# austintheriot/ray-tracer-webgl

Measured on AMD Instinct MI355X. Metric: Mray/s (ray segments/s) at 1920x1080, higher is better.
Workload: dtype f32

## Files before the change

### bindings/rust/ptrace_sys.rs

```rust
use std::os::raw::{c_char, c_int, c_void};

#[repr(C)] #[derive(Clone, Copy, Default)]
pub struct PtSphere {
    pub center: [f32; 3], pub radius: f32,
    pub type_: i32, pub albedo: [f32; 3],
    pub fuzz: f32, pub refraction_index: f32,
    pub uuid: i32, pub _pad: i32,
}

#[repr(C)] #[derive(Clone, Copy, Default)]
pub struct PtParams {
    pub width: u32, pub height: u32,
    pub time: f32, pub samples_per_pixel: i32, pub max_depth: i32,
    pub camera_origin: [f32; 3], pub horizontal: [f32; 3], pub vertical: [f32; 3],
    pub lower_left_corner: [f32; 3], pub u: [f32; 3], pub v: [f32; 3],
    pub lens_radius: f32,
    pub render_count: i32, pub should_average: i32, pub last_frame_weight: f32,
    pub background_mode: i32,
    pub band_rows: u32, pub band_index: u32, pub band_count: u32,
    pub time_step: f32, pub first_pass: u32,
}

#[repr(C)] #[derive(Clone, Copy, Default)]
pub struct PtErrorStats {
// ... 46 lines not shown

#[repr(C)] #[derive(Clone, Copy, Default)]
pub struct PtProbeSH {
    pub sh: [[f32; 3]; 9], pub samples: f32,
}

#[repr(C)] #[derive(Clone, Copy, Default)]
pub struct PtProbeLattice {
    pub origin: [f32; 3], pub nx: u32, pub step: [f32; 3], pub ny: u32, pub nz: u32, pub flags: u32, pub _pad: [u32; 2],
}

#[repr(C)] #[derive(Clone, Copy, Default)]
pub struct PtProbeShadeOptions {
    pub flags: u32, pub normal_bias: f32, pub _pad: [u32; 2],
}

#[repr(C)] #[derive(Clone, Copy)]
pub struct PtMeterOptions {
    pub key: f32, pub key_permille: u32, pub high_permille: u32, pub e_min: f32, pub e_max: f32, pub white_min: f32, pub rate: f32,
    pub x0: u32, pub y0: u32, pub w: u32, pub h: u32, pub _pad: u32,
}
impl Default for PtMeterOptions {
    fn default() -> Self {
        PtMeterOptions { key: 0.18, key_permille: 500, high_permille: 990, e_min: 0.00390625, e_max: 256.0, white_min: 1.0, rate: 1.0,
                         x0: 0, y0: 0, w: 0, h: 0, _pad: 0 }
    }
}

#[repr(C)] #[derive(Clone, Copy, Default)]
pub struct PtExposure {
    pub exposure: f32, pub white: f32, pub y_key: f32, pub y_high: f32, pub lit: u64, pub below: u32, pub meterings: u32,
}

#[repr(C)] #[derive(Clone, Copy, Default)]
pub struct PtToneOptions {
    pub curve: i32, pub gamma: i32, pub exposure: f32, pub white: f32,
}

pub const PT_GLARE_MAX_LEVELS: usize = 8;
#[repr(C)] #[derive(Clone, Copy)]
pub struct PtGlareOptions {
    pub strength: f32, pub threshold: f32, pub levels: u32, pub _pad: u32, pub weight: [f32; PT_GLARE_MAX_LEVELS],
}
impl Default for PtGlareOptions {
    fn default() -> Self {
        PtGlareOptions { strength: 0.15, threshold: 0.0, levels: 6, _pad: 0, weight: [0.35, 0.25, 0.18, 0.12, 0.06, 0.04, 0.0, 0.0] }
    }
}

#[repr(C)] pub struct PtCtx { _private: [u8; 0] }

#[link(name = "ptrace")]
extern "C" {
    pub fn pt_create(out: *mut *mut PtCtx, device: c_int, width: u32, height: u32) -> c_int;
    pub fn pt_create_on_stream(out: *mut *mut PtCtx, device: c_int, width: u32, height: u32, hip_stream: *mut c_void) -> c_int;
    pub fn pt_destroy(ctx: *mut PtCtx) -> c_int;
    pub fn pt_resize(ctx: *mut PtCtx, width: u32, height: u32) -> c_int;
    pub fn pt_set_spheres(ctx: *mut PtCtx, spheres: *const PtSphere, n: u32) -> c_int;
    pub fn pt_set_params(ctx: *mut PtCtx, params: *const PtParams) -> c_int;
    pub fn pt_render(ctx: *mut PtCtx) -> c_int;
    pub fn pt_render_passes(ctx: *mut PtCtx, n_passes: u32) -> c_int;
    pub fn pt_reserve_passes(ctx: *mut PtCtx, max_passes: u32) -> c_int;
    pub fn pt_reset_accum(ctx: *mut PtCtx) -> c_int;
    pub fn pt_synchronize(ctx: *mut PtCtx) -> c_int;
    pub fn pt_resolve(ctx: *mut PtCtx, rgba_out: *mut f32, gamma: c_int) -> c_int;
    pub fn pt_resolve_rgba8(ctx: *mut PtCtx, rgba_out: *mut u8, gamma: c_int) -> c_int;
    pub fn pt_blend_rgba8(ctx: *mut PtCtx, prev: *const u8, out: *mut u8) -> c_int;
    pub fn pt_accum_ptr(ctx: *mut PtCtx, dev_ptr: *mut *mut c_void, bytes: *mut usize) -> c_int;
    pub fn pt_bind_accum(ctx: *mut PtCtx, dev_ptr: *mut c_void, bytes: usize) -> c_int;
    pub fn pt_read_accum(ctx: *mut PtCtx, dst: *mut f32, bytes: usize) -> c_int;
    pub fn pt_load_accum(ctx: *mut PtCtx, src: *const f32, bytes: usize) -> c_int;
    pub fn pt_set_stream(ctx: *mut PtCtx, hip_stream: *mut c_void) -> c_int;
    pub fn pt_set_option(ctx: *mut PtCtx, key: c_int, value: c_int) -> c_int;
    pub fn pt_tune(ctx: *mut PtCtx, n_passes: u32) -> c_int;
    pub fn pt_set_debug_overlay(ctx: *mut PtCtx, enable: c_int, selected_object: i32, cursor_point: *const f32) -> c_int;
    pub fn pt_last_trace_build(ctx: *mut PtCtx) -> c_int;
    pub fn pt_error_ptr(ctx: *mut PtCtx, dev_ptr: *mut *mut c_void, bytes: *mut usize) -> c_int;
    pub fn pt_resolve_error(ctx: *mut PtCtx, rgba_out: *mut f32) -> c_int;
    pub fn pt_error_tiles(ctx: *mut PtCtx, tiles_out: *mut f32, tiles_x: *mut u32, tiles_y: *mut u32) -> c_int;
    pub fn pt_error_stats(ctx: *mut PtCtx, out: *mut PtErrorStats) -> c_int;
    pub fn pt_render_until(ctx: *mut PtCtx, target_rel_error: f32, passes_per_launch: u32, max_passes: u32, out: *mut PtErrorStats) -> c_int;
    pub fn pt_render_adaptive(ctx: *mut PtCtx, target_rel_error: f32, passes_per_round: u32, max_passes: u32, out: *mut PtErrorStats, adaptive_out: *mut PtAdaptiveStats) -> c_int;
    pub fn pt_adaptive_tiles(ctx: *mut PtCtx, base_out: *mut u32, order_out: *mut u32, n_tiles: *mut u32, n_active: *mut u32) -> c_int;
    pub fn pt_resolve_filtered(ctx: *mut PtCtx, rgba_out: *mut f32, radius: u32, kappa: f32, gamma: c_int) -> c_int;
    pub fn pt_resolve_filtered_patch(ctx: *mut PtCtx, rgba_out: *mut f32, radius: u32, patch: u32, kappa: f32, gamma: c_int) -> c_int;
    pub fn pt_render_features(ctx: *mut PtCtx) -> c_int;
    pub fn pt_features_ptr(ctx: *mut PtCtx, plane: c_int, dev_ptr: *mut *mut c_void, bytes: *mut usize) -> c_int;
    pub fn pt_read_features(ctx: *mut PtCtx, plane: c_int, out: *mut c_void) -> c_int;
    pub fn pt_keep_history(ctx: *mut PtCtx) -> c_int;
    pub fn pt_load_history(ctx: *mut PtCtx, prev: *const PtParams, ids: *const c_void, point: *const c_void) -> c_int;
    pub fn pt_reproject(ctx: *mut PtCtx, options: *const PtReprojectOptions) -> c_int;
    pub fn pt_reproject_stats(ctx: *mut PtCtx, out: *mut PtReprojectStats) -> c_int;
    pub fn pt_reproject_constants(prev: *const PtParams, tolerance_px: f32, out16: *mut f32) -> c_int;
    pub fn pt_reproject_estimate(ctx: *mut PtCtx, options: *const PtReprojectOptions) -> c_int;
    pub fn pt_query_rays(ctx: *mut PtCtx, rays: *const PtRay, n: u32, hits: *mut PtRayHit) -> c_int;
    pub fn pt_query_batch(ctx: *mut PtCtx) -> u32;
    pub fn pt_query_radiance(ctx: *mut PtCtx, rays: *const PtRay, n: u32, n_passes: u32, out: *mut PtRayRadiance) -> c_int;
    pub fn pt_gather_irradiance(ctx: *mut PtCtx, points: *const PtGatherPoint, n: u32, directions: u32, n_passes: u32, out: *mut PtIrradiance) -> c_int;
    pub fn pt_bake_probes(ctx: *mut PtCtx, probes: *const PtGatherPoint, n: u32, directions: u32, n_passes: u32, out: *mut PtProbeSH) -> c_int;
    pub fn pt_query_radiance_nee(ctx: *mut PtCtx, rays: *const PtRay, n: u32, n_passes: u32, out: *mut PtRayRadiance) -> c_int;
    pub fn pt_gather_irradiance_nee(ctx: *mut PtCtx, points: *const PtGatherPoint, n: u32, directions: u32, n_passes: u32, out: *mut PtIrradiance) -> c_int;
    pub fn pt_bake_probes_nee(ctx: *mut PtCtx, probes: *const PtGatherPoint, n: u32, directions: u32, n_passes: u32, out: *mut PtProbeSH) -> c_int;
    pub fn pt_bake_lattice(ctx: *mut PtCtx, lattice: *const PtProbeLattice, first: u32, count: u32, directions: u32, n_passes: u32, estimator: c_int, out: *mut PtProbeSH) -> c_int;
    pub fn pt_shade_probes(ctx: *mut PtCtx, lattice: *const PtProbeLattice, probes: *const PtProbeSH, options: *const PtProbeShadeOptions, rgba_out: *mut f32) -> c_int;
    pub fn pt_meter(ctx: *mut PtCtx, src: *const f32, options: *const PtMeterOptions) -> c_int;
    pub fn pt_meter_read(ctx: *mut PtCtx, out: *mut PtExposure, hist256: *mut u32) -> c_int;
    pub fn pt_meter_set(ctx: *mut PtCtx, record: *const PtExposure) -> c_int;
    pub fn pt_exposure_solve(hist256: *const u32, below: u32, options: *const PtMeterOptions, prev_or_null: *const PtExposure, out: *mut PtExposure) -> c_int;
    pub fn pt_resolve_toned(ctx: *mut PtCtx, src: *const f32, options: *const PtToneOptions, rgba_out: *mut f32) -> c_int;
    pub fn pt_resolve_toned_rgba8(ctx: *mut PtCtx, src: *const f32, options: *const PtToneOptions, rgba_out: *mut u8) -> c_int;
    pub fn pt_glare(ctx: *mut PtCtx, src: *const f32, options: *const PtGlareOptions, rgba_out: *mut f32) -> c_int;
    pub fn pt_grid_fit(ctx: *mut PtCtx) -> c_int;
    pub fn pt_refit_grid(ctx: *mut PtCtx, only_if_stale: c_int) -> c_int;
    pub fn pt_clear_textures(ctx: *mut PtCtx) -> c_int;
    pub fn pt_render_frame(ctx: *mut PtCtx, even_odd_count: u32) -> c_int;
    pub fn pt_render_frames(ctx: *mut PtCtx, even_odd_count: u32, max_render_count: u32, n_frames: u32) -> c_int;
    pub fn pt_read_canvas(ctx: *mut PtCtx, rgba_out: *mut u8) -> c_int;
    pub fn pt_read_texture(ctx: *mut PtCtx, index: c_int, rgba_out: *mut u8) -> c_int;
    pub fn pt_write_texture(ctx: *mut PtCtx, index: c_int, rgba_in: *const u8) -> c_int;
    pub fn pt_last_error(ctx: *mut PtCtx) -> *const c_char;
    pub fn pt_abi_version() -> c_int;
    pub fn pt_device_count() -> c_int;
    pub fn pt_local_rows(height: u32, band_rows: u32, band_index: u32, band_count: u32) -> u32;
    pub fn pt_band_row(band_rows: u32, band_index: u32, band_count: u32, local_row: u32) -> u32;
}

pub const PT_OPT_GEOMETRY_PATH: c_int = 1;
pub const PT_OPT_ERROR_ESTIMATE: c_int = 7;
pub const PT_OPT_FEATURES: c_int = 8;
pub const PT_OPT_REPROJECT: c_int = 9;
pub const PT_OPT_RAY_QUERIES: c_int = 10;
pub const PT_OPT_TONEMAP: c_int = 11;
pub const PT_OPT_GLARE: c_int = 12;
pub const PT_TONE_CLAMP: i32 = 0;
pub const PT_TONE_REINHARD: i32 = 1;
pub const PT_TONE_FILMIC: i32 = 2;
pub const PT_LATTICE_SKIP_BURIED: u32 = 1;
pub const PT_PROBE_HALFSPACE: u32 = 1;
pub const PT_RAY_INVALID: i32 = -2;
pub const PT_REPROJECT_TOLERANCE_DEFAULT: f32 = 2.0;
pub const PT_REPROJECT_CAP_DIFFUSE_DEFAULT: f32 = 32.0;
pub const PT_REPROJECT_CAP_OTHER_DEFAULT: f32 = 8.0;
pub const PT_FEAT_ALBEDO: c_int = 0;
pub const PT_FEAT_NORMAL: c_int = 1;
pub const PT_FEAT_POINT: c_int = 2;
pub const PT_FEAT_IDS: c_int = 3;
pub const PT_FEAT_PLANES: c_int = 4;
pub const PT_FILTER_MAX_RADIUS: u32 = 4;
pub const PT_FILTER_KAPPA_DEFAULT: f32 = 2.0;
pub const PT_FILTER_MAX_PATCH: u32 = 1;
pub const PT_FILTER_PATCH_KAPPA_DEFAULT: f32 = 1.5;
pub const PT_OPT_RUSSIAN_ROULETTE: c_int = 5;
pub const PT_OPT_NEXT_EVENT: c_int = 13;
pub const PT_BUILD_NEXT_EVENT: c_int = 16;


impl PtParams {
    pub fn from_state(s: &crate::state::State, now_ms: f64) -> Self {
        let spp = if s.is_paused { s.samples_per_pixel.max(25) } else { s.samples_per_pixel };
        PtParams {
            width: s.width, height: s.height, time: now_ms as f32,
            samples_per_pixel: spp as i32, max_depth: s.max_depth as i32,
            camera_origin: s.camera_origin.to_array(), horizontal: s.horizontal.to_array(),
            vertical: s.vertical.to_array(), lower_left_corner: s.lower_left_corner.to_array(),
            u: s.u.to_array(), v: s.v.to_array(), lens_radius: s.lens_radius as f32,
            render_count: s.render_count as i32, should_average: s.should_average as i32,
            last_frame_weight: s.last_frame_weight, background_mode: 0,
            band_rows: 8, band_index: 0, band_count: 1,
            time_step: 0.0, first_pass: 0,
        }
    }
}

impl From<&crate::glsl::Sphere> for PtSphere {
    fn from(s: &crate::glsl::Sphere) -> Self {
        PtSphere {
            center: s.center.to_array(), radius: s.radius as f32,
            type_: s.material.material_type.value(), albedo: s.material.albedo.to_array(),
            fuzz: s.material.fuzz, refraction_index: s.material.refraction_index,
            uuid: s.uuid, _pad: 0,
        }
    }
}
```

### include/ptrace.h

```cpp
#ifndef PTRACE_H
#define PTRACE_H

#include <stdint.h>
#include <stddef.h>

#ifdef __cplusplus
extern "C" {
#endif

#define PT_ABI_VERSION 5

enum {
  PT_OK = 0,
  PT_ERR_INVALID = -1,
  PT_ERR_NO_DEVICE = -2,
  PT_ERR_HIP = -3,
  PT_ERR_NOT_READY = -4,
  PT_ERR_CAPACITY = -5,
};

enum {
  PT_DIFFUSE = 0,
  PT_METAL = 1,
  PT_GLASS = 2,
  PT_EMISSIVE = 3,
};

enum {
  PT_GEOM_AUTO = 0,
  PT_GEOM_LDS = 1,
  PT_GEOM_SCALAR = 2,
  PT_GEOM_BVH = 3,
  PT_GEOM_GRID = 4,
  PT_GEOM_SMALL = 5,
};
enum {
  PT_OPT_GEOMETRY_PATH = 1,
  PT_OPT_COUNT_WORK = 2,
  PT_OPT_CARRY_LANES = 3,
  PT_OPT_REFILL_MIN = 4,
  PT_OPT_RUSSIAN_ROULETTE = 5,
  PT_OPT_GRID_FIT = 6,
  PT_OPT_ERROR_ESTIMATE = 7,
  PT_OPT_FEATURES = 8,
  PT_OPT_REPROJECT = 9,
  PT_OPT_RAY_QUERIES = 10,
  PT_OPT_TONEMAP = 11,
  PT_OPT_GLARE = 12,
  PT_OPT_NEXT_EVENT = 13,
};

enum {
  PT_BG_SKY = 0,
  PT_BG_BLACK = 1,
};

typedef struct PtSphere {
  float center[3];
  float radius;
  int32_t type;
  float albedo[3];
  float fuzz;
  float refraction_index;
  int32_t uuid;
  int32_t _pad;
} PtSphere;

typedef struct PtParams {
  uint32_t width;
  uint32_t height;
  float time;
  int32_t samples_per_pixel;
  int32_t max_depth;
  float camera_origin[3];
  float horizontal[3];
  float vertical[3];
  float lower_left_corner[3];
  float u[3];
  float v[3];
  float lens_radius;
  int32_t render_count;
  int32_t should_average;
  float last_frame_weight;
  int32_t background_mode;
  uint32_t band_rows;
  uint32_t band_index;
  uint32_t band_count;
  float time_step;
  uint32_t first_pass;
} PtParams;
#define PT_TIME_STEP_DECORRELATED 0.3618034f

typedef struct PtCameraIn {
  uint32_t width, height;
  double camera_origin[3];
  double yaw_degrees;
  double pitch_degrees;
  double vup[3];
  double fov_radians;
  double focus_distance;
  double aperture;
} PtCameraIn;

typedef struct PtLookAtIn {
  uint32_t width, height;
  double look_from[3], look_at[3], vup[3];
  double vfov_radians;
  double focus_distance;
  double aperture;
} PtLookAtIn;

typedef struct PtStats {
  uint64_t segments;
  uint64_t samples;
  uint64_t sphere_tests;
  double render_kernel_ms;
  uint32_t render_launches;
  uint32_t total_spp;
  uint32_t n_spheres;
  uint32_t local_rows;
  uint32_t geometry_path;
  uint32_t geometry_tuned;
  uint32_t bvh_nodes;
  uint32_t bvh_slots;
  uint32_t bvh_outliers;
  uint32_t bvh_depth;
  uint32_t grid_cells[3];
  uint32_t grid_entries;
  uint32_t grid_always;
  uint32_t grid_fit_stale;
  uint64_t work[8];
  float grid_near_factor;
  float grid_need_factor;
  uint64_t far_rays;
  uint32_t grid_kernel_build;
  uint32_t grid_walk_flat;
} PtStats;

typedef struct pt_ctx pt_ctx;

int pt_create(pt_ctx** out, int device, uint32_t width, uint32_t height);
int pt_create_on_stream(pt_ctx** out, int device, uint32_t width, uint32_t height, void* hip_stream);
int pt_destroy(pt_ctx* ctx);
int pt_resize(pt_ctx* ctx, uint32_t width, uint32_t height);

int pt_set_spheres(pt_ctx* ctx, const PtSphere* spheres, uint32_t n);
int pt_set_params(pt_ctx* ctx, const PtParams* params);

int pt_render(pt_ctx* ctx);
int pt_render_passes(pt_ctx* ctx, uint32_t n_passes);
int pt_reserve_passes(pt_ctx* ctx, uint32_t max_passes);
int pt_reset_accum(pt_ctx* ctx);
int pt_synchronize(pt_ctx* ctx);

int pt_resolve(pt_ctx* ctx, float* rgba_out, int gamma);
int pt_resolve_rgba8(pt_ctx* ctx, uint8_t* rgba_out, int gamma);
int pt_accum_ptr(pt_ctx* ctx, void** dev_ptr, size_t* bytes);
int pt_read_accum(pt_ctx* ctx, float* dst, size_t bytes);
int pt_load_accum(pt_ctx* ctx, const float* src, size_t bytes);
int pt_bind_accum(pt_ctx* ctx, void* dev_ptr, size_t bytes);
int pt_set_stream(pt_ctx* ctx, void* hip_stream);
#define PT_STREAM_LEGACY ((void*)1)

typedef struct PtErrorStats {
  double sum_e2;
  double sum_m2;
  double rel_error;
  double rms_error;
  uint64_t pixels;
  uint64_t pixels_counted;
  uint64_t pixels_short;
  uint64_t pixels_nonfinite;
  uint32_t passes_min, passes_max;
  uint32_t passes_rendered;
  uint32_t reached;
} PtErrorStats;
int pt_error_ptr(pt_ctx* ctx, void** dev_ptr, size_t* bytes);
int pt_resolve_error(pt_ctx* ctx, float* rgba_out);
int pt_error_tiles(pt_ctx* ctx, float* tiles_out, uint32_t* tiles_x, uint32_t* tiles_y);
int pt_error_stats(pt_ctx* ctx, PtErrorStats* out);
int pt_render_until(pt_ctx* ctx, float target_rel_error, uint32_t passes_per_launch, uint32_t max_passes, PtErrorStats* out);

typedef struct PtAdaptiveStats {
  uint32_t rounds;
  uint32_t partial_rounds;
  uint32_t tiles;
  uint32_t tiles_active;
  uint64_t tile_passes;
  uint64_t samples;
} PtAdaptiveStats;
int pt_render_adaptive(pt_ctx* ctx, float target_rel_error, uint32_t passes_per_round, uint32_t max_passes, PtErrorStats* out,
                       PtAdaptiveStats* adaptive_out );
int pt_adaptive_tiles(pt_ctx* ctx, uint32_t* base_out, uint32_t* order_out, uint32_t* n_tiles, uint32_t* n_active);

#define PT_FILTER_MAX_RADIUS 4
#define PT_FILTER_KAPPA_DEFAULT 2.0f
int pt_resolve_filtered(pt_ctx* ctx, float* rgba_out, uint32_t radius, float kappa, int gamma);

#define PT_FILTER_MAX_PATCH 1
#define PT_FILTER_PATCH_KAPPA_DEFAULT 1.5f
int pt_resolve_filtered_patch(pt_ctx* ctx, float* rgba_out, uint32_t radius, uint32_t patch, float kappa, int gamma);

// ... 239 lines not shown
```

### ray_tracer_webgl_amd/abi.py

```python
import ctypes as C

import numpy as np

PT_ABI_VERSION = 5

PT_OK = 0
PT_ERR_INVALID = -1
PT_ERR_NO_DEVICE = -2
PT_ERR_HIP = -3
PT_ERR_NOT_READY = -4
PT_ERR_CAPACITY = -5

PT_DIFFUSE = 0
PT_METAL = 1
PT_GLASS = 2
PT_EMISSIVE = 3

PT_BG_SKY = 0
PT_BG_BLACK = 1

PT_GEOM_AUTO, PT_GEOM_LDS, PT_GEOM_SCALAR, PT_GEOM_BVH, PT_GEOM_GRID, PT_GEOM_SMALL = 0, 1, 2, 3, 4, 5
PT_OPT_GEOMETRY_PATH, PT_OPT_COUNT_WORK, PT_OPT_CARRY_LANES, PT_OPT_REFILL_MIN, PT_OPT_RUSSIAN_ROULETTE, PT_OPT_GRID_FIT = 1, 2, 3, 4, 5, 6
PT_OPT_FEATURES = 8
PT_FEAT_ALBEDO, PT_FEAT_NORMAL, PT_FEAT_POINT, PT_FEAT_IDS, PT_FEAT_PLANES = 0, 1, 2, 3, 4
PT_OPT_ERROR_ESTIMATE = 7
PT_OPT_REPROJECT = 9
PT_OPT_RAY_QUERIES = 10
PT_OPT_TONEMAP = 11
PT_TONE_CLAMP, PT_TONE_REINHARD, PT_TONE_FILMIC = 0, 1, 2
PT_OPT_GLARE = 12
PT_GLARE_MAX_LEVELS = 8
PT_OPT_NEXT_EVENT = 13
PT_GLARE_STRENGTH_DEFAULT = 0.15
PT_GLARE_LEVELS_DEFAULT = 6
PT_GLARE_WEIGHTS_DEFAULT = (0.35, 0.25, 0.18, 0.12, 0.06, 0.04, 0.0, 0.0)
PT_METER_KEY_DEFAULT = 0.18
PT_METER_KEY_PERMILLE_DEFAULT = 500
PT_METER_HIGH_PERMILLE_DEFAULT = 990
PT_METER_E_MIN_DEFAULT = 2.0 ** -8
PT_METER_E_MAX_DEFAULT = 2.0 ** 8
PT_RAY_INVALID = -2
PT_REPROJECT_TOLERANCE_DEFAULT = 2.0
PT_REPROJECT_CAP_DIFFUSE_DEFAULT = 32.0
PT_REPROJECT_CAP_OTHER_DEFAULT = 8.0
PT_TIME_STEP_DECORRELATED = 0.3618034
PT_FILTER_MAX_RADIUS = 4
PT_FILTER_KAPPA_DEFAULT = 2.0
PT_FILTER_MAX_PATCH = 1
PT_FILTER_PATCH_KAPPA_DEFAULT = 1.5
NO_SELECTED_OBJECT_ID = 1000
BUILD_PLAIN, BUILD_ROULETTE, BUILD_TWIN, BUILD_DEBUG_OVERLAY, BUILD_FEATURES = 0, 1, 2, 3, 4
BUILD_NEXT_EVENT = 16
PT_STREAM_LEGACY = 1
GEOM_NAMES = {0: "auto", 1: "lds", 2: "scalar", 3: "bvh", 4: "grid", 5: "small"}

f3 = C.c_float * 3
d3 = C.c_double * 3


class PtSphere(C.Structure):
    _fields_ = [
        ("center", f3),
        ("radius", C.c_float),
        ("type", C.c_int32),
        ("albedo", f3),
        ("fuzz", C.c_float),
        ("refraction_index", C.c_float),
        ("uuid", C.c_int32),
        ("_pad", C.c_int32),
    ]


SPHERE_DTYPE = np.dtype(
    [
        ("center", "<f4", 3),
        ("radius", "<f4"),
        ("type", "<i4"),
        ("albedo", "<f4", 3),
        ("fuzz", "<f4"),
        ("refraction_index", "<f4"),
        ("uuid", "<i4"),
        ("_pad", "<i4"),
    ]
)
assert SPHERE_DTYPE.itemsize == C.sizeof(PtSphere) == 48


class PtParams(C.Structure):
    _fields_ = [
        ("width", C.c_uint32),
        ("height", C.c_uint32),
        ("time", C.c_float),
        ("samples_per_pixel", C.c_int32),
        ("max_depth", C.c_int32),
        ("camera_origin", f3),
        ("horizontal", f3),
        ("vertical", f3),
        ("lower_left_corner", f3),
        ("u", f3),
        ("v", f3),
        ("lens_radius", C.c_float),
        ("render_count", C.c_int32),
        ("should_average", C.c_int32),
        ("last_frame_weight", C.c_float),
        ("background_mode", C.c_int32),
        ("band_rows", C.c_uint32),
        ("band_index", C.c_uint32),
        ("band_count", C.c_uint32),
        ("time_step", C.c_float),
        ("first_pass", C.c_uint32),
    ]

    def copy(self):
        out = PtParams()
        C.memmove(C.byref(out), C.byref(self), C.sizeof(PtParams))
        return out


class PtCameraIn(C.Structure):
    _fields_ = [
        ("width", C.c_uint32),
        ("height", C.c_uint32),
        ("camera_origin", d3),
        ("yaw_degrees", C.c_double),
        ("pitch_degrees", C.c_double),
        ("vup", d3),
        ("fov_radians", C.c_double),
        ("focus_distance", C.c_double),
        ("aperture", C.c_double),
    ]


class PtLookAtIn(C.Structure):
    _fields_ = [
        ("width", C.c_uint32),
        ("height", C.c_uint32),
        ("look_from", d3),
        ("look_at", d3),
        ("vup", d3),
        ("vfov_radians", C.c_double),
        ("focus_distance", C.c_double),
        ("aperture", C.c_double),
    ]


class PtStats(C.Structure):
    _fields_ = [
        ("segments", C.c_uint64),
        ("samples", C.c_uint64),
        ("sphere_tests", C.c_uint64),
        ("render_kernel_ms", C.c_double),
        ("render_launches", C.c_uint32),
        ("total_spp", C.c_uint32),
        ("n_spheres", C.c_uint32),
        ("local_rows", C.c_uint32),
        ("geometry_path", C.c_uint32),
        ("geometry_tuned", C.c_uint32),
        ("bvh_nodes", C.c_uint32),
        ("bvh_slots", C.c_uint32),
        ("bvh_outliers", C.c_uint32),
        ("bvh_depth", C.c_uint32),
        ("grid_cells", C.c_uint32 * 3),
        ("grid_entries", C.c_uint32),
        ("grid_always", C.c_uint32),
        ("grid_fit_stale", C.c_uint32),
        ("work", C.c_uint64 * 8),
        ("grid_near_factor", C.c_float),
        ("grid_need_factor", C.c_float),
        ("far_rays", C.c_uint64),
        ("grid_kernel_build", C.c_uint32),
        ("grid_walk_flat", C.c_uint32),
    ]


class PtErrorStats(C.Structure):

    _fields_ = [
        ("sum_e2", C.c_double),
        ("sum_m2", C.c_double),
        ("rel_error", C.c_double),
        ("rms_error", C.c_double),
        ("pixels", C.c_uint64),
        ("pixels_counted", C.c_uint64),
        ("pixels_short", C.c_uint64),
        ("pixels_nonfinite", C.c_uint64),
# ... 326 lines not shown
```

### ray_tracer_webgl_amd/csrc/pt_api.hip

```cpp
#include <hip/hip_runtime.h>

#include <mutex>
#include <chrono>
#include <cmath>
#include <cstdarg>
#include <cstdio>
#include <cstdlib>
#include <cstring>
#include <new>
#include <string>
#include <thread>
#include <utility>
#include <vector>

#include "../../include/ptrace.h"
#include "../../include/ptrace_dev.h"
#include "pt_bvh.hpp"
#include "pt_grid.hpp"
#include "pt_grid_records.hpp"
#include "pt_scene_image.hpp"
#include "pt_extra.h"
#include "pt_kernel_args.h"
#include "pt_geom_plan.hpp"
#include "pt_launch_plan.hpp"
#include "pt_trace_table.hpp"
#include "pt_nee_table.hpp"
#include "pt_rad_nee_table.hpp"
#include "pt_nee.hpp"
#include "pt_tile_order.hpp"
#include "pt_error_plan.hpp"
#include "pt_reproject_plan.hpp"
#include "pt_reproject.hpp"
#include "pt_query.hpp"
#include "pt_radiance.hpp"
#include "pt_tone.hpp"
#include "pt_glare.hpp"
#include "pt_gather.hpp"
#include "pt_probe.hpp"
#include "pt_buffers.hpp"
#include "pt_ctx_state.hpp"

#define PT_API extern "C" __attribute__((visibility("default")))

#include "pt_kernels.hip"

static thread_local std::string g_create_error;

int ptbuf::dev_malloc(void** p, size_t bytes) {
  const hipError_t e = hipMalloc(p, bytes);
  if (e != hipSuccess) (void)hipGetLastError();
  return (int)e;
}
int ptbuf::dev_free(void* p) { return (int)hipFree(p); }
using ptbuf::DevBuf;

struct Launch {
  PtKernelArgs A;
  const void* kfn = nullptr;
  uint32_t grid = 1, block = 256;
  size_t lds = 0;
  int path = 0;
  int trial = -1;
};

struct FramePlan {
  Launch L;
  const uint32_t* ctr = nullptr;
  uint32_t even_odd0 = 0;
  int max_render_count = 0, render_count0 = 0, should_average = 0;
  float last_frame_weight = 0.f;
  hipStream_t stream = nullptr;
  float4* slab = nullptr;
  uint32_t* tex0 = nullptr; uint32_t* tex1 = nullptr; uint32_t* canvas = nullptr;
  uint32_t n_frames = 1;
};

struct SceneList {
  DevBuf<float> geom, r0;
  DevBuf<PtMatRec> mat;
  DevBuf<int32_t> uuid;
  uint32_t n = 0;
  ptscene::Split host;
};
struct SceneSlots {
  bool present = false;
  DevBuf<uint32_t> index;
  DevBuf<PtMatRec> mat;
  DevBuf<int32_t> uuid;
  size_t index_n = 0;
};
struct SceneBvh : SceneSlots { ptbvh::Bvh head; DevBuf<uint32_t> nodes; DevBuf<float> nodes32, slots; };
struct SceneGrid : SceneSlots { ptgrid::Grid head; DevBuf<uint32_t> cells, ring; DevBuf<float> entries; };

constexpr int kProbeFormDefault = 1;

struct pt_ctx {
  int device = 0;
  uint32_t width = 0, height = 0;
  hipStream_t own_stream = nullptr;
  hipStream_t stream = nullptr;
  SceneList list;
  SceneBvh bvh;
  SceneGrid grid;
  ptstate::Flags state;
  ptstate::AccumTally tally;
  PtParams params{};
  uint32_t local_rows = 0;
  ptbuf::FrameSet<float4> frame;
  ptbuf::EstimateSet<float4> est;
  ptbuf::FeatureSet<float4> feat;
  ptbuf::QuerySet<float4> query;
  ptbuf::HistorySet<float4> hist;
  ptbuf::ExposureSet expo;
  ptbuf::GlareSet<float4> glare;
  ptbuf::GatherSet gather;
  ptbuf::ProbeSet probe;
  int probe_form = kProbeFormDefault;
  uint32_t* probe_paths = nullptr;
  uint32_t reserved_passes = 1;
  PathTuner geom;
  hipEvent_t trial_ev[8] = {nullptr, nullptr, nullptr, nullptr, nullptr, nullptr, nullptr, nullptr};
  int grid_fit_mode = 0;
  int count_work = 0;
  DevBuf<uint32_t> d_cell_hist;
  size_t cell_hist_n = 0;
  DevBuf<unsigned long long> d_wave_log;
  size_t wave_log_n = 0;
  uint32_t carry_lanes = 12;
  uint32_t refill_min = 4;
  int rr_min_depth = 0;
  ptbuf::LightSet<ptnee::Light> lights;
  bool dbg_enable = false;
  int32_t dbg_selected = 0;
  float dbg_cursor[3] = {0.f, 0.f, 0.f};
  int last_build = 0;
  TileOrder order;
  DevBuf<uint32_t> d_adapt;
  std::vector<uint32_t> h_adapt_flags;
  uint32_t adapt_tiles = 0, adapt_active = 0;
  DevBuf<uint32_t> d_frame_ctr;
  hipGraphExec_t frame_exec[4] = {nullptr, nullptr, nullptr, nullptr};
  FramePlan frame_plan[4];
  DevBuf<float4> d_frame_slab;
  DevBuf<unsigned long long> d_counters;
  std::vector<std::pair<hipEvent_t, hipEvent_t>> events;
  size_t events_used = 0;
  double kernel_ms = 0.0;
  int num_cus = 256;
  double setup_ms[PT_SETUP_COUNT] = {0};
  std::string error;

  ~pt_ctx() {
    for (auto& ev : events) { (void)hipEventDestroy(ev.first); (void)hipEventDestroy(ev.second); }
    for (hipEvent_t e : trial_ev) if (e) (void)hipEventDestroy(e);
    for (hipGraphExec_t e : frame_exec) if (e) (void)hipGraphExecDestroy(e);
    if (own_stream) (void)hipStreamDestroy(own_stream);
  }
};

namespace {

inline size_t n_pixels(const pt_ctx* c) { return (size_t)c->local_rows * c->width; }
inline uint32_t tiles_x(const pt_ctx* c) { return (c->width + 7) / 8; }
inline uint32_t tiles_y(const pt_ctx* c) { return (c->local_rows + 7) / 8; }
inline uint32_t n_tiles(const pt_ctx* c) { return tiles_x(c) * tiles_y(c); }

inline uint32_t grid_for(uint32_t n, uint32_t block, uint32_t cap) {
  uint32_t g = (n + block - 1) / block;
  if (g < 1) g = 1;
  return g > cap ? cap : g;
}
inline uint32_t pixel_grid(uint32_t n_pix) { return grid_for(n_pix, 256, 2048); }
inline uint32_t tile_grid(uint32_t n) { return grid_for(n, 4, 4096); }

inline hipError_t zero_queue_heads(pt_ctx* c, uint32_t queue_static) {
  if (queue_static == 2u)
    return hipMemsetAsync(c->d_counters.get() + PT_CTR_GROUP_HEADS, 0, 8 * PT_QUEUE_GROUPS_MAX * sizeof(unsigned long long), c->stream);
  if (queue_static == 0u) return hipMemsetAsync(c->d_counters.get() + PT_CTR_HEAD, 0, sizeof(unsigned long long), c->stream);
  return hipSuccess;
}

inline double host_ms() {
  return std::chrono::duration<double, std::milli>(std::chrono::steady_clock::now().time_since_epoch()).count();
}

int fail(pt_ctx* c, int code, const char* fmt, ...) {
  char buf[512];
  va_list ap;
  va_start(ap, fmt);
  vsnprintf(buf, sizeof buf, fmt, ap);
  va_end(ap);
  if (c) c->error = buf; else g_create_error = buf;
  return code;
}

#define PT_HIP(c, call)                                                                     \
  do {                                                                                      \
    hipError_t e_ = static_cast<hipError_t>(call);  \
    if (e_ != hipSuccess)                                                                   \
      return fail((c), PT_ERR_HIP, "%s failed: %s (%s:%d)", #call, hipGetErrorString(e_),   \
                  __FILE__, __LINE__);                                                      \
  } while (0)

constexpr int kFrameLevels = 4;
#ifdef PT_DEV_KNOBS
static uint32_t kFrameGroups[kFrameLevels] = {64u, 16u, 4u, 1u};
struct FrameGroupKnob { FrameGroupKnob() { if (const char* e = getenv("PT_FRAME_GROUP")) { const uint32_t v = (uint32_t)atoi(e); if (v >= 16u && v <= 128u && v % 16u == 0u) kFrameGroups[0] = v; } } } g_frame_group_knob;
#else
constexpr uint32_t kFrameGroups[kFrameLevels] = {64u, 16u, 4u, 1u};
#endif
constexpr size_t kFrameSlabCap = (size_t)1 << 30;

uint32_t count_local_rows(uint32_t height, const PtParams& p) {
  return pt_local_rows(height, p.band_rows, p.band_index, p.band_count);
}

hipError_t fill_identity_order(DevBuf<uint32_t>& order, size_t tiles) {
  std::vector<uint32_t> ident(tiles);
  for (size_t i = 0; i < tiles; i++) ident[i] = (uint32_t)i;
  return hipMemcpy(order.get(), ident.data(), tiles * sizeof(uint32_t), hipMemcpyHostToDevice);
}

ptbuf::Extent extent_of(const pt_ctx* c) { return {n_pixels(c), n_tiles(c), c->reserved_passes}; }

int fit_refused(pt_ctx* c, const char* what, const ptbuf::Fit& f, const ptbuf::Extent& e) {
  if (f.capped) return fail(c, PT_ERR_CAPACITY, "%s: %zu local pixels exceed the kernels' 32-bit texel index", what, e.pix);
  return fail(c, PT_ERR_HIP, "%s: a device allocation for %zu local pixels failed: %s", what, e.pix, hipGetErrorString((hipError_t)f.err));
}

int ensure_buffers(pt_ctx* c) {
  const ptbuf::Extent e = extent_of(c);
  auto zero = [c](auto& buf, size_t n) { return hipMemsetAsync(buf.get(), 0, n * sizeof(*buf.get()), c->stream); };
  {
    auto& s = c->frame;
    const ptbuf::Fit f = s.fit(e);
    if (f.fresh & s.ACCUM) {
      PT_HIP(c, zero(s.own_accum, e.pix));
      c->tally.own_fresh();
    }
    if (f.fresh & s.COST) PT_HIP(c, zero(s.tile_cost, e.tiles));
    if (f.fresh & s.ORDER) {
      PT_HIP(c, fill_identity_order(s.tile_order, e.tiles));
      c->order.reseeded();
      changed(*c, ptstate::TILE_COUNT_CHANGED);
    }
    if (f.fresh & s.TEX0) PT_HIP(c, zero(s.tex[0], e.pix));
    if (f.fresh & s.TEX1) PT_HIP(c, zero(s.tex[1], e.pix));
    if (f.fresh & s.CANVAS) PT_HIP(c, zero(s.canvas, e.pix));
    if (!f.ok()) return fit_refused(c, "the context's buffers", f, e);
  }
  {
    const ptbuf::Fit f = c->est.fit(e, c->hist.on);
    if (f.fresh & c->est.STATE) PT_HIP(c, zero(c->est.state, 2 * e.pix));
    if (!f.ok()) return fit_refused(c, "error estimate", f, e);
  }
  if (const ptbuf::Fit f = c->feat.fit(e); !f.ok()) return fit_refused(c, "feature planes", f, e);
  {
    if (c->query.on && !c->query.fits(e)) PT_HIP(c, hipStreamSynchronize(c->stream));
    const ptbuf::Fit f = c->query.fit(e);
    if (f.fresh & c->query.ORDER) PT_HIP(c, fill_identity_order(c->query.order, e.tiles));
    if (!f.ok()) return fit_refused(c, "query planes", f, e);
  }
  if (const ptbuf::Fit f = c->hist.fit(e); !f.ok()) return fit_refused(c, "history planes", f, e);
  {
    const ptbuf::Fit f = c->expo.fit();
    if (f.fresh & c->expo.STATE) PT_HIP(c, zero(c->expo.state, c->expo.kWords));
    if (!f.ok()) return fit_refused(c, "exposure state", f, e);
  }
  if (const ptbuf::Fit f = c->glare.fit(c->width, c->local_rows); !f.ok()) return fit_refused(c, "glare pyramid", f, e);
  return PT_OK;
}

int frame_buffers_ready(pt_ctx* c, const char* who) {
  const ptbuf::Extent e = extent_of(c);
  if (c->frame.in_place(e) && (!c->est.on || c->est.in_place(e, c->hist.on))) return PT_OK;
  return fail(c, PT_ERR_CAPACITY, "%s: the context's buffers are not allocated for the rows in place (an earlier allocation failed)", who);
}

enum OptInSet { SET_ESTIMATE, SET_FEATURES, SET_QUERIES, SET_REPROJECT, SET_TONEMAP, SET_GLARE, SET_NEXT_EVENT };
int option_off(pt_ctx* c, const char* who, OptInSet set, int code = PT_ERR_NOT_READY) {
  static const char* const what[] = {"the error estimate is off (pt_set_option PT_OPT_ERROR_ESTIMATE)", "the feature planes are off (pt_set_option PT_OPT_FEATURES)",
                                     "ray queries are off (pt_set_option PT_OPT_RAY_QUERIES)", "reprojection is off (pt_set_option PT_OPT_REPROJECT)",
                                     "tone mapping is off (pt_set_option PT_OPT_TONEMAP)", "the glare is off (pt_set_option PT_OPT_GLARE)",
                                     "next-event estimation is off (pt_set_option PT_OPT_NEXT_EVENT)"};
// ... 591 lines not shown
  A.n_slots = g.n_entries;
  A.n_outliers = g.n_always;
  for (int k = 0; k < 3; k++) {
    A.bvh_c0[k] = g.c0[k];
    A.grid_n[k] = g.n[k];
    A.grid_lo[k] = g.lo[k]; A.grid_hi[k] = g.hi[k];
    A.grid_h[k] = g.h[k]; A.grid_inv_h[k] = g.inv_h[k];
    A.grid_lo_n[k] = g.lo_n[k]; A.grid_hi_n[k] = g.hi_n[k];
  }
  A.bvh_s0 = g.s0;
  A.grid_r2_near = g.r2_near;
  return grid_build(c);
}

static hipError_t resident_blocks(const void* kfn, uint32_t block, size_t lds, int built_for, int* out) {
  int n = 0;
  const hipError_t e = hipOccupancyMaxActiveBlocksPerMultiprocessor(&n, kfn, (int)block, lds);
  if (e != hipSuccess) return e;
  const int cap = built_for * 4 / (int)(block / 64u);
  *out = n < cap ? n : cap;
  return hipSuccess;
}

static uint32_t walk_block_threads(const void* kfn, int built_for, size_t scene, size_t lds_max, std::optional<uint32_t> knob) {
  uint32_t block = 0;
  int best_waves = -1;
  for (uint32_t b = 256; b <= 1024; b *= 2) {
    const size_t l = scene + (size_t)PT_PARK_STRIDE * 4 * b;
    if (l > lds_max) continue;
    int n = 0;
    if (resident_blocks(kfn, b, l, built_for, &n) != hipSuccess) {
      (void)hipGetLastError();
      continue;
    }
    const int waves = n * (int)(b / 64);
    if (waves > best_waves) { best_waves = waves; block = b; }
  }
  if (knob && *knob >= 64u && *knob <= 1024u && *knob % 64u == 0u) block = *knob;
  return block ? block : 1024u;
}

static LaunchKnobs read_launch_knobs() {
  LaunchKnobs k;
#ifdef PT_DEV_KNOBS
  auto knob = [](const char* name, auto& field) { if (const char* e = getenv(name)) field = atoi(e); };
  knob("PT_CARRY_LANES", k.carry_lanes), knob("PT_BVH_BLOCK", k.bvh_block), knob("PT_COOP_MAX", k.coop_max);
  knob("PT_PER_CU", k.per_cu), knob("PT_QUEUE_CHUNK", k.queue_chunk), knob("PT_GRID_PERCENT", k.grid_percent);
  knob("PT_QUEUE_STATIC", k.queue_static), knob("PT_COST_FEEDBACK", k.cost_feedback), knob("PT_QUEUE_GROUPED", k.queue_grouped);
  knob("PT_FEWER_X10_1", k.fewer_x10_1), knob("PT_FEWER_X10_2", k.fewer_x10_2);
#endif
  return k;
}

struct LaunchUse {
  bool allow_trials = false;
  enum Feedback { PLANNED, OFF, ON } feedback = PLANNED;
  uint32_t n_first_tiles = 0;
  const uint32_t* table = nullptr;
  Door door = DOOR_NONE;
  bool next_event = false;
  uint32_t query_rays = 0;
  uint32_t first_pass = 0;
  const char* who = "pt_render";
};

static int prepare_launch(pt_ctx* c, uint32_t n_passes, const LaunchUse& use, Launch* L) {
  PtKernelArgs& A = L->A;
  if (int rc = frame_buffers_ready(c, use.who); rc != PT_OK) return rc;
  {
    int rc = fill_uniforms(c, n_passes, A);
    if (rc != PT_OK) return rc;
  }
  if (use.n_first_tiles) {
    A.n_items = use.n_first_tiles * 64u * n_passes;
    A.tile_order = use.table;
  }
  const LaunchKnobs knobs = read_launch_knobs();
  if (knobs.carry_lanes) A.carry_lanes = *knobs.carry_lanes;
  const bool door = use.door != DOOR_NONE, query = use.door == DOOR_QUERY, rad = use.door == DOOR_RADIANCE;
  const bool feat = use.door == DOOR_FEATURES || query;
  if (c->geom.policy == PT_GEOM_AUTO && !door) try_finish_tuning(c);
  const bool rr = !door && c->rr_min_depth > 0, dbg = !door && c->dbg_enable;
  const bool nee = !door && c->lights.on;
  const bool rad_nee = rad && use.next_event;
  if ((nee || rad_nee) && !c->lights.in_place()) return fail(c, PT_ERR_CAPACITY, "%s: PT_OPT_NEXT_EVENT's light table is not in place (a failed allocation: install the scene or turn the option on again)", use.who);
  if (rr && c->count_work) return fail(c, PT_ERR_INVALID, "PT_OPT_COUNT_WORK and PT_OPT_RUSSIAN_ROULETTE exclude each other");
  if (dbg && c->count_work) return fail(c, PT_ERR_INVALID, "PT_OPT_COUNT_WORK and the debug overlay exclude each other");
  if (dbg && !c->state.uuid_valid) return fail(c, PT_ERR_NOT_READY, "debug overlay: the uuid arrays are not in place (pt_set_debug_overlay after a failed upload?)");
  if (feat && !c->state.uuid_valid) return fail(c, PT_ERR_NOT_READY, "%s: the uuid arrays are not in place (%s after a failed upload?)", query ? "ray queries" : "feature planes",
                                             query ? "PT_OPT_RAY_QUERIES" : "PT_OPT_FEATURES");
  const PathChoice choice = c->geom.choose(path_scene(c), use.allow_trials && !door, rr || dbg || door || nee);
  const int path = choice.path;
  if (!door) c->geom.last = path;

  const bool walk = path == PT_GEOM_BVH || path == PT_GEOM_GRID;
  size_t scene = 0;
  Staging st;
  if (walk) {
    st = path == PT_GEOM_BVH ? bind_hierarchy(c, A) : bind_grid(c, A);
    scene = st.bytes;
    A.lds_scene_bytes = (uint32_t)scene;
  } else {
    scene = c->list.n <= PT_MAX_SPHERES_LDS ? (size_t)PT_LDS_ENTRIES(c->list.n) * 16 : 0;
  }
  const int row = trace_row(path, c->list.n, st.kind, c->grid.head.n[1]);
  const int build = door ? door_build(use.door) : trace_build(false, dbg, rr, c->count_work);
  if (feat) {
    A.uuid = c->list.uuid.get();
    A.slot_uuid = path == PT_GEOM_BVH ? c->bvh.uuid.get() : (path == PT_GEOM_GRID ? c->grid.uuid.get() : nullptr);
    A.slab = reinterpret_cast<float*>(query ? c->query.planes.get() : c->feat.planes.get());
    A.spp = 1; A.max_depth = 1; A.rr_min_depth = 0;
    if (query) A.dbg_selected = (int32_t)use.query_rays;
  }
  if (rad) {
    A.uuid = reinterpret_cast<const int32_t*>(c->query.planes.get());
    A.slot_uuid = nullptr;
    A.dbg_selected = (int32_t)use.query_rays;
    A.first_pass = use.first_pass;
    A.rr_min_depth = 0;
  }
  const bool nee_cell = takes_nee_cell(nee, build);
  if (!nee_cell && reads_ring_layout(row, build)) {
    A.grid_cells = c->grid.ring.get();
    A.n_cells = (uint32_t)ptrec::ring_cells(c->grid.head.n[0], c->grid.head.n[2]);
  }
  if (nee_cell) {
    A.uuid = reinterpret_cast<const int32_t*>(c->lights.table.get());
    A.slot_uuid = nullptr;
    A.dbg_selected = (int32_t)c->lights.n;
    A.rr_min_depth = 0;
  }
  const bool rad_nee_cell = takes_rad_nee_cell(rad_nee, build);
  if (rad_nee_cell) {
    const uint32_t n_lights = c->lights.n;
    A.slot_uuid = reinterpret_cast<const int32_t*>(c->lights.table.get());
    memcpy(&A.dbg_cursor[0], &n_lights, sizeof n_lights);
  }
  const TraceCell& tk = rad_nee_cell ? kRadNeeKernels[row] : (nee_cell ? kNeeKernels[row] : kTraceKernels[row][build]);
  const void* kfn = cell_kernel(c->device, tk);
  if (!query && !rad) c->last_build = nee_cell ? (int)BUILD_NEXT_EVENT : build;
  const uint32_t block = walk ? walk_block_threads(kfn, tk.waves, scene, kWalkLdsMax, knobs.bvh_block) : list_block_threads(scene);
  const size_t lds = walk ? scene + (size_t)PT_PARK_STRIDE * 4 * block : scene;
  A.block_threads = block;
  int per_cu = 0;
  PT_HIP(c, resident_blocks(kfn, block, lds, tk.waves, &per_cu));

  const LaunchPlan P = plan_launch({A.n_items, feat ? 1 : c->params.samples_per_pixel, n_passes, block, per_cu, (uint32_t)c->num_cus, walk,
                                    c->list.n, knobs});
  A.queue_chunk = P.queue_chunk; A.queue_static = (uint32_t)P.deal; A.queue_groups = P.queue_groups;
  A.n_waves = P.n_waves; A.coop_max_live = P.coop_max_live; A.refill_ahead = P.refill_ahead;
  A.cost_feedback = use.feedback == LaunchUse::PLANNED ? P.cost_feedback : (use.feedback == LaunchUse::ON ? 1u : 0u);
  if (door) A.cost_feedback = 0u;
  L->kfn = kfn; L->grid = P.grid; L->block = block; L->lds = lds; L->path = path; L->trial = choice.trial;
  return PT_OK;
}

static int launch_trace(pt_ctx* c, const Launch& L) {
  void* kargs[] = {const_cast<PtKernelArgs*>(&L.A)};
  PT_HIP(c, hipLaunchKernel(L.kfn, dim3(L.grid), dim3(L.block), kargs, L.lds, c->stream));
  return PT_OK;
}

static int trace_once(pt_ctx* c, uint32_t n_passes, const LaunchUse& use, TimedSpan* span = nullptr) {
  Launch L;
  if (int rc = prepare_launch(c, n_passes, use, &L); rc != PT_OK) return rc;
  if (span)
    if (int rc = span->take(c); rc != PT_OK) return rc;
  PT_HIP(c, zero_queue_heads(c, L.A.queue_static));
  if (span)
    if (int rc = span->begin(c); rc != PT_OK) return rc;
  if (int rc = launch_trace(c, L); rc != PT_OK) return rc;
  return span ? span->end(c) : PT_OK;
}

PT_API int pt_render_passes(pt_ctx* c, uint32_t n_passes) {
  if (!c) return PT_ERR_INVALID;
  if (int rc = scene_and_uniforms(c, "pt_render"); rc != PT_OK) return rc;
  if (n_passes == 0) return fail(c, PT_ERR_INVALID, "pt_render_passes: n_passes == 0");
  if (n_passes > c->reserved_passes)
    return fail(c, PT_ERR_CAPACITY, "pt_render_passes: %u passes > %u reserved (pt_reserve_passes)",
                n_passes, c->reserved_passes);
  if (c->local_rows == 0) return PT_OK;
  const bool estimate = c->est.on && !c->est.paused;
  if (estimate && c->est.spp != 0 && c->est.spp != c->params.samples_per_pixel)
    return fail(c, PT_ERR_INVALID, "pt_render_passes: %d samples per pixel while the error estimate holds passes of %d: clear first "
                                   "(pt_reset_accum)", c->params.samples_per_pixel, c->est.spp);
  PT_HIP(c, hipSetDevice(c->device));

  Launch L;
  {
    LaunchUse use;
    use.allow_trials = true;
    use.who = "pt_render_passes";
    int rc = prepare_launch(c, n_passes, use, &L);
    if (rc != PT_OK) return rc;
  }
  PtKernelArgs& A = L.A;
  const PtParams& p = c->params;
  const uint32_t grid = L.grid, block = L.block;
  const int path = L.path;
  int trial = L.trial;

  const bool capturing = is_capturing(c);
  if (capturing && c->count_work)
    return fail(c, PT_ERR_INVALID, "pt_render_passes: PT_OPT_COUNT_WORK (measuring twin: allocates its wave log) cannot be captured into a hipGraph");
  if (c->count_work && (path == PT_GEOM_BVH || path == PT_GEOM_GRID || path == PT_GEOM_SMALL)) {
    const size_t n_waves = (size_t)grid * (block / 64);
    if (c->d_wave_log.capacity() < n_waves * PT_WAVE_LOG_WORDS) PT_HIP(c, c->d_wave_log.reserve(n_waves * PT_WAVE_LOG_WORDS));
    PT_HIP(c, hipMemsetAsync(c->d_wave_log.get(), 0, n_waves * PT_WAVE_LOG_WORDS * sizeof(unsigned long long), c->stream));
    c->wave_log_n = n_waves;
    A.wave_log = c->d_wave_log.get();
    if (path == PT_GEOM_GRID && c->count_work >= 2) {
      const size_t n_hist = (size_t)A.n_slots + PT_COH_BINS;
      if (c->d_cell_hist.capacity() < n_hist) PT_HIP(c, c->d_cell_hist.reserve(n_hist));
      PT_HIP(c, hipMemsetAsync(c->d_cell_hist.get(), 0, n_hist * sizeof(uint32_t), c->stream));
      c->cell_hist_n = n_hist;
      A.cell_hist = c->d_cell_hist.get();
    }
  }
  TimedSpan span;
  if (!capturing)
    if (int rc = span.take(c); rc != PT_OK) return rc;

  PT_HIP(c, zero_queue_heads(c, A.queue_static));
  if (c->order.uniform_wants_order_kernel(A.cost_feedback != 0u)) {
    int rc = launch_tile_order(c);
    if (rc != PT_OK) return rc;
    c->order.uniform_order_kernel_enqueued(capturing);
  }
  if (capturing) trial = -1;
  if (trial >= 0) {
    for (int k = 0; k < 2; k++)
      if (!c->trial_ev[2 * trial + k]) PT_HIP(c, hipEventCreate(&c->trial_ev[2 * trial + k]));
    PT_HIP(c, hipEventRecord(c->trial_ev[2 * trial], c->stream));
  }
  if (int rc = span.begin(c); rc != PT_OK) return rc;
  if (int rc = launch_trace(c, L); rc != PT_OK) return rc;
  c->order.uniform_traced(A.cost_feedback != 0u, capturing);
  if (int rc = span.end(c); rc != PT_OK) return rc;
  if (trial >= 0) {
    PT_HIP(c, hipEventRecord(c->trial_ev[2 * trial + 1], c->stream));
    c->geom.enqueued(trial, (double)n_pixels(c) * n_passes * (double)p.samples_per_pixel);
  }

  uint32_t n_pix = (uint32_t)n_pixels(c);
  if (estimate) {
    float4* accum = c->frame.accum;
    float4* est = c->est.state.get();
    const float4* slab = c->frame.slab.get();
    uint32_t passes = n_passes;
    void* kargs[] = {&accum, &est, &slab, &n_pix, &passes};
    PT_HIP(c, hipLaunchKernel(pt_error_kernel(PT_E_FOLD), dim3(pixel_grid(n_pix)), dim3(256), kargs, 0, c->stream));
    c->est.spp = p.samples_per_pixel;
  } else {
    hipLaunchKernelGGL(pt_accumulate_kernel, dim3(pixel_grid(n_pix)), dim3(256), 0, c->stream,
                       c->frame.accum, c->frame.slab.get(), n_pix, n_passes);
    PT_HIP(c, hipGetLastError());
  }

  c->tally.uniform_launch(capturing, n_pix, n_passes, (uint32_t)p.samples_per_pixel);
  return PT_OK;
}

PT_API int pt_render(pt_ctx* c) { return pt_render_passes(c, 1); }

namespace {

int plan_frame(pt_ctx* c, const uint32_t* ctr, uint32_t even_odd0, int max_render_count, uint32_t n_frames, float4* slab, FramePlan* F) {
  memset(static_cast<void*>(F), 0, sizeof *F);
  LaunchUse use;
  use.feedback = LaunchUse::OFF;
  int rc = prepare_launch(c, n_frames, use, &F->L);
  if (rc != PT_OK) return rc;
  F->L.A.frame_ctr = ctr;
  F->ctr = ctr; F->even_odd0 = even_odd0; F->max_render_count = max_render_count;
  F->render_count0 = c->params.render_count; F->should_average = c->params.should_average;
  F->last_frame_weight = c->params.last_frame_weight;
  F->L.A.slab = reinterpret_cast<float*>(slab);
  F->stream = c->stream; F->slab = slab;
  F->tex0 = c->frame.tex[0].get(); F->tex1 = c->frame.tex[1].get(); F->canvas = c->frame.canvas.get();
  F->n_frames = n_frames;
  return PT_OK;
}

int enqueue_frame(pt_ctx* c, FramePlan& F, bool advance) {
  if (int rc = launch_trace(c, F.L); rc != PT_OK) return rc;
  const uint32_t n_pix = (uint32_t)n_pixels(c);
  if (F.n_frames > 1u) {
    hipLaunchKernelGGL(pt_frames_blend_kernel, dim3(pixel_grid(n_pix)), dim3(256), 0, c->stream, F.slab, F.n_frames,
                       c->frame.tex[0].get(), c->frame.tex[1].get(), c->frame.canvas.get(), n_pix, F.ctr, F.render_count0, F.even_odd0, F.max_render_count,
                       F.should_average, F.last_frame_weight);
    PT_HIP(c, hipGetLastError());
  }
  for (uint32_t f = 0; f < (F.n_frames > 1u ? 0u : 1u); f++) {
    hipLaunchKernelGGL(pt_frame_blend_kernel, dim3(pixel_grid(n_pix)), dim3(256), 0, c->stream, F.slab + (size_t)f * n_pix,
                       c->frame.tex[0].get(), c->frame.tex[1].get(), c->frame.canvas.get(), n_pix, F.ctr, f, F.render_count0, F.even_odd0, F.max_render_count,
                       F.should_average, F.last_frame_weight);
    PT_HIP(c, hipGetLastError());
  }
  if (advance) {
    hipLaunchKernelGGL(pt_frame_advance_kernel, dim3(1), dim3(PT_QUEUE_GROUPS_MAX), 0, c->stream, c->d_frame_ctr.get(), c->d_counters.get(), F.n_frames);
    PT_HIP(c, hipGetLastError());
  }
  return PT_OK;
}

int ensure_cost_order(pt_ctx* c, uint32_t n_frames) {
  const TileOrder::FrameStep step = c->order.frames(c->params.samples_per_pixel, c->params, c->state.scene_gen, n_frames, [c] { return is_capturing(c); });
  if (step.zero_costs)
    PT_HIP(c, hipMemsetAsync(c->frame.tile_cost.get(), 0, c->frame.tile_cost.capacity() * sizeof(uint32_t), c->stream));
  if (step.order_kernel) {
    int rc = launch_tile_order(c);
    if (rc != PT_OK) return rc;
    c->order.order_kernel_ran();
  }
  if (!step.probe) return PT_OK;
  Launch L;
  LaunchUse use;
  use.feedback = LaunchUse::ON;
  int rc = prepare_launch(c, 1, use, &L);
  if (rc != PT_OK) return rc;
  L.A.slab = reinterpret_cast<float*>(c->frame.slab.get());
  unsigned long long* seg = c->d_counters.get() + PT_CTR_SEGMENTS;
  PT_HIP(c, hipMemcpyAsync(c->d_counters.get() + PT_CTR_SCRATCH, seg, sizeof *seg, hipMemcpyDeviceToDevice, c->stream));
  PT_HIP(c, zero_queue_heads(c, L.A.queue_static));
  rc = launch_trace(c, L);
  if (rc != PT_OK) return rc;
  rc = launch_tile_order(c);
  if (rc != PT_OK) return rc;
  PT_HIP(c, hipMemcpyAsync(seg, c->d_counters.get() + PT_CTR_SCRATCH, sizeof *seg, hipMemcpyDeviceToDevice, c->stream));
  c->order.probed_for(c->params, c->state.scene_gen);
  return PT_OK;
}

int frame_ready(pt_ctx* c, const char* who) {
  if (!c) return PT_ERR_INVALID;
  if (int rc = scene_and_uniforms(c, who); rc != PT_OK) return rc;
  if (c->count_work) return fail(c, PT_ERR_INVALID, "%s: not with PT_OPT_COUNT_WORK (the measuring twins are not frame kernels)", who);
  return frame_buffers_ready(c, who);
}

}

PT_API int pt_clear_textures(pt_ctx* c) {
  if (!c) return PT_ERR_INVALID;
  if (int rc = frame_buffers_ready(c, "pt_clear_textures"); rc != PT_OK) return rc;
  PT_HIP(c, hipSetDevice(c->device));
  const size_t bytes = n_pixels(c) * sizeof(uint32_t);
  if (bytes == 0) return PT_OK;
  for (int k = 0; k < 2; k++) PT_HIP(c, hipMemsetAsync(c->frame.tex[k].get(), 0, bytes, c->stream));
  PT_HIP(c, hipMemsetAsync(c->frame.canvas.get(), 0, bytes, c->stream));
  return PT_OK;
}

PT_API int pt_render_frame(pt_ctx* c, uint32_t even_odd_count) {
  int rc = frame_ready(c, "pt_render_frame");
  if (rc != PT_OK) return rc;
  if (c->local_rows == 0) return PT_OK;
  PT_HIP(c, hipSetDevice(c->device));
  FramePlan F;
  rc = plan_frame(c, c->d_frame_ctr.get() + 1, even_odd_count, 0x7fffffff, 1, c->frame.slab.get(), &F);
  if (rc != PT_OK) return rc;
  rc = ensure_cost_order(c, 1);
  if (rc != PT_OK) return rc;
  PT_HIP(c, zero_queue_heads(c, F.L.A.queue_static));
  rc = enqueue_frame(c, F, false);
  if (rc != PT_OK) return rc;
  c->tally.frames(1, n_pixels(c), (uint32_t)c->params.samples_per_pixel);
  return PT_OK;
}

PT_API int pt_render_frames(pt_ctx* c, uint32_t even_odd_count, uint32_t max_render_count, uint32_t n_frames) {
  int rc = frame_ready(c, "pt_render_frames");
  if (rc != PT_OK) return rc;
  if (n_frames == 0 || c->local_rows == 0) return PT_OK;
  if (max_render_count > 0x7fffffffu) max_render_count = 0x7fffffffu;
  PT_HIP(c, hipSetDevice(c->device));
// ... 455 lines not shown
  };
  int rc = look();
  while (rc == PT_OK && !out->reached && done < max_passes && n_active != 0) {
    const uint32_t k = passes_per_round < max_passes - done ? passes_per_round : max_passes - done;
    if (n_active == tiles) {
      rc = pt_render_passes(c, k);
    } else {
      rc = partial_round(c, k, tiles, n_active, pixels_active);
    }
    if (rc != PT_OK) break;
    ad.rounds++;
    ad.partial_rounds += n_active != tiles ? 1u : 0u;
    ad.tile_passes += (uint64_t)n_active * k;
    ad.samples += pixels_active * k * (uint64_t)c->params.samples_per_pixel;
    advance_first_pass(c, k);
    done += k;
    rc = look();
  }
  if (adaptive_out) *adaptive_out = ad;
  return rc;
}

PT_API int pt_adaptive_tiles(pt_ctx* c, uint32_t* base_out, uint32_t* order_out, uint32_t* n_tiles, uint32_t* n_active) {
  if (!c) return PT_ERR_INVALID;
  if (!c->state.adapt_valid) return fail(c, PT_ERR_NOT_READY, "pt_adaptive_tiles: no partial round yet (pt_render_adaptive)");
  if (n_tiles) *n_tiles = c->adapt_tiles;
  if (n_active) *n_active = c->adapt_active;
  if (!base_out && !order_out) return PT_OK;
  PT_HIP(c, hipSetDevice(c->device));
  const size_t bytes = (size_t)c->adapt_tiles * sizeof(uint32_t);
  const uint32_t* part = c->d_adapt.get() + c->adapt_tiles;
  if (order_out) PT_HIP(c, hipMemcpyAsync(order_out, part, bytes, hipMemcpyDeviceToHost, c->stream));
  if (base_out) PT_HIP(c, hipMemcpyAsync(base_out, part + c->adapt_tiles, bytes, hipMemcpyDeviceToHost, c->stream));
  PT_HIP(c, hipStreamSynchronize(c->stream));
  return PT_OK;
}

PT_API int pt_get_stats(pt_ctx* c, PtStats* out) {
  if (!c || !out) return PT_ERR_INVALID;
  PT_HIP(c, hipSetDevice(c->device));
  PT_HIP(c, hipStreamSynchronize(c->stream));
  int rc = fold_events(c);
  if (rc != PT_OK) return rc;
  unsigned long long ctr[PT_CTR_COUNT];
  PT_HIP(c, hipMemcpy(ctr, c->d_counters.get(), sizeof ctr, hipMemcpyDeviceToHost));
  memset(out, 0, sizeof *out);
  out->segments = ctr[PT_CTR_SEGMENTS];
  out->samples = c->tally.samples;
  out->sphere_tests = ctr[PT_CTR_SEGMENTS] * (uint64_t)c->list.n;
  out->render_kernel_ms = c->kernel_ms;
  out->render_launches = c->tally.launches;
  out->total_spp = c->tally.total_spp;
  if (c->frame.accum && c->local_rows) {
    float4 px0;
    PT_HIP(c, hipMemcpy(&px0, c->frame.accum, sizeof px0, hipMemcpyDeviceToHost));
    if (px0.w >= 0.0f && px0.w < 4294967040.0f) out->total_spp = (uint32_t)px0.w;
  }
  out->n_spheres = c->list.n;
  try_finish_tuning(c);
  out->local_rows = c->local_rows;
  out->geometry_path = (uint32_t)c->geom.last;
  out->geometry_tuned = c->geom.tuned ? 1u : 0u;
  for (int k = 0; k < 8; k++) out->work[k] = ctr[PT_CTR_WORK + k];
  out->far_rays = ctr[PT_CTR_FAR_RAYS];
  if (c->grid.present) {
    for (int k = 0; k < 3; k++) out->grid_cells[k] = c->grid.head.n[k];
    out->grid_entries = c->grid.head.n_entries;
    out->grid_always = c->grid.head.n_always;
    out->grid_near_factor = c->grid.head.near_factor;
    out->grid_need_factor = (float)need_factor(c);
    out->grid_fit_stale = (uint32_t)fit_state(c);
    out->grid_kernel_build = (uint32_t)grid_build(c).kind;
    out->grid_walk_flat = grid_walk_flat((int)out->grid_kernel_build, c->grid.head.n[1]) ? 1u : 0u;
  }
  if (c->bvh.present) {
    out->bvh_nodes = c->bvh.head.n_nodes;
    out->bvh_slots = c->bvh.head.n_slots;
    out->bvh_outliers = c->bvh.head.n_outliers;
    out->bvh_depth = c->bvh.head.depth;
  }
  return PT_OK;
}

template <class Set, class Off, class Extra>
static int set_buffer_option(pt_ctx* c, int value, const char* name, Set& set, Off off, const void* kernel, Extra extra) {
  if (value != 0 && value != 1) return fail(c, PT_ERR_INVALID, "pt_set_option: %s %d", name, value);
  PT_HIP(c, hipSetDevice(c->device));
  PT_HIP(c, hipStreamSynchronize(c->stream));
  if (!value) { off(); return PT_OK; }
  if (set.on) return PT_OK;
  hipFuncAttributes attr;
  PT_HIP(c, hipFuncGetAttributes(&attr, kernel));
  set.on = true;
  int rc = ensure_buffers(c);
  if (rc == PT_OK) rc = extra();
  if (rc != PT_OK) off();
  return rc;
}

PT_API int pt_set_option(pt_ctx* c, int key, int value) {
  if (!c) return PT_ERR_INVALID;
  if (key == PT_OPT_GEOMETRY_PATH) {
    if (value != PT_GEOM_AUTO && value != PT_GEOM_LDS && value != PT_GEOM_SCALAR && value != PT_GEOM_BVH &&
        value != PT_GEOM_GRID && value != PT_GEOM_SMALL)
      return fail(c, PT_ERR_INVALID, "pt_set_option: bad geometry path %d", value);
    c->geom.policy = value;
    return PT_OK;
  }
  if (key == PT_OPT_COUNT_WORK) {
    if (value > 0 && c->lights.on)
      return fail(c, PT_ERR_INVALID, "pt_set_option: PT_OPT_COUNT_WORK and PT_OPT_NEXT_EVENT exclude each other (turn next-event estimation off first: "
                                     "pt_set_option(ctx, PT_OPT_NEXT_EVENT, 0))");
    c->count_work = value < 0 ? 0 : (value > 2 ? 2 : value);
    return PT_OK;
  }
  if (key == PT_OPT_REFILL_MIN) {
    if (value < 1 || value > 64) return fail(c, PT_ERR_INVALID, "pt_set_option: refill min %d", value);
    c->refill_min = (uint32_t)value;
    return PT_OK;
  }
  if (key == PT_OPT_RUSSIAN_ROULETTE) {
    if (value < 0 || value > 1000000) return fail(c, PT_ERR_INVALID, "pt_set_option: roulette depth %d", value);
    if (value > 0 && c->dbg_enable)
      return fail(c, PT_ERR_INVALID, "pt_set_option: PT_OPT_RUSSIAN_ROULETTE and the debug overlay exclude each other (turn the overlay off first: "
                                     "pt_set_debug_overlay(ctx, 0, ...))");
    if (value > 0 && c->lights.on)
      return fail(c, PT_ERR_INVALID, "pt_set_option: PT_OPT_RUSSIAN_ROULETTE and PT_OPT_NEXT_EVENT exclude each other (turn next-event estimation off first: "
                                     "pt_set_option(ctx, PT_OPT_NEXT_EVENT, 0))");
    c->rr_min_depth = value;
    return PT_OK;
  }
  if (key == PT_OPT_NEXT_EVENT) {
    if (value != 0 && value != 1) return fail(c, PT_ERR_INVALID, "pt_set_option: next-event estimation %d", value);
    if (value && c->rr_min_depth > 0)
      return fail(c, PT_ERR_INVALID, "pt_set_option: PT_OPT_NEXT_EVENT and PT_OPT_RUSSIAN_ROULETTE exclude each other (turn roulette off first: "
                                     "pt_set_option(ctx, PT_OPT_RUSSIAN_ROULETTE, 0))");
    if (value && c->dbg_enable)
      return fail(c, PT_ERR_INVALID, "pt_set_option: PT_OPT_NEXT_EVENT and the debug overlay exclude each other (turn the overlay off first: "
                                     "pt_set_debug_overlay(ctx, 0, ...))");
    if (value && c->count_work)
      return fail(c, PT_ERR_INVALID, "pt_set_option: PT_OPT_NEXT_EVENT and PT_OPT_COUNT_WORK exclude each other (turn the measuring twins off first: "
                                     "pt_set_option(ctx, PT_OPT_COUNT_WORK, 0))");
    PT_HIP(c, hipSetDevice(c->device));
    PT_HIP(c, hipStreamSynchronize(c->stream));
    if (!value) { c->lights.release(); return PT_OK; }
    if (c->lights.on) return PT_OK;
    hipFuncAttributes attr;
    PT_HIP(c, hipFuncGetAttributes(&attr, pt_nee_kernel(PT_VARIANT_ID(pt_trace_kernel_scalar))));
    c->lights.on = true;
    if (c->state.have_spheres) {
      int rc = upload_lights(c, c->list.host, c->list.n);
      if (rc != PT_OK) { c->lights.release(); return rc; }
    }
    return PT_OK;
  }
  if (key == PT_OPT_CARRY_LANES) {
    if (value < 0 || value > 64) return fail(c, PT_ERR_INVALID, "pt_set_option: carry lanes %d", value);
    c->carry_lanes = (uint32_t)value;
    return PT_OK;
  }
  if (key == PT_OPT_GRID_FIT) {
    if (value != 0 && value != 1) return fail(c, PT_ERR_INVALID, "pt_set_option: grid fit mode %d", value);
    c->grid_fit_mode = value;
    return PT_OK;
  }
  auto reproject_off = [c] { c->hist.release(); c->est.stage.release(); };
  auto uuids = [c] { return !c->state.uuid_valid && c->state.have_spheres ? upload_uuids(c, c->list.host.uuid) : PT_OK; };
  if (key == PT_OPT_ERROR_ESTIMATE)
    return set_buffer_option(c, value, "error estimate", c->est, [c] { c->est.release(); }, pt_error_kernel(PT_E_FOLD), [c] { return clear_error(c); });
  if (key == PT_OPT_FEATURES)
    return set_buffer_option(c, value, "feature planes", c->feat, [&] { c->feat.release(); c->probe.release_stage(); reproject_off(); },
                             pt_feature_kernel(PT_VARIANT_ID(pt_trace_kernel_scalar)), uuids);
  if (key == PT_OPT_RAY_QUERIES)
    return set_buffer_option(c, value, "ray queries", c->query, [c] { c->query.release(); c->gather.release(); c->probe.release_points(); }, pt_query_kernel(PT_VARIANT_ID(pt_trace_kernel_scalar)), uuids);
  if (key == PT_OPT_REPROJECT) {
    if (value == 1 && !c->feat.on) return fail(c, PT_ERR_INVALID, "pt_set_option: PT_OPT_REPROJECT needs PT_OPT_FEATURES on (it reads the feature planes)");
    return set_buffer_option(c, value, "reprojection", c->hist, reproject_off, pt_reproject_kernel_handle(), [] { return PT_OK; });
  }
  if (key == PT_OPT_TONEMAP)
    return set_buffer_option(c, value, "tone mapping", c->expo, [c] { c->expo.release(); }, pt_display_kernel(PT_D_METER), [] { return PT_OK; });
  if (key == PT_OPT_GLARE)
    return set_buffer_option(c, value, "glare", c->glare, [c] { c->glare.release(); }, pt_glare_kernel(PT_G_DOWN), [] { return PT_OK; });
  return fail(c, PT_ERR_INVALID, "pt_set_option: unknown key %d", key);
}

PT_API int pt_set_debug_overlay(pt_ctx* c, int enable, int32_t selected_object, const float cursor_point[3]) {
  if (!c) return PT_ERR_INVALID;
  if (enable && !cursor_point) return fail(c, PT_ERR_INVALID, "pt_set_debug_overlay: cursor_point is NULL");
  if (enable && c->rr_min_depth > 0)
    return fail(c, PT_ERR_INVALID, "pt_set_debug_overlay: the debug overlay and PT_OPT_RUSSIAN_ROULETTE exclude each other (turn roulette off first: "
                                   "pt_set_option(ctx, PT_OPT_RUSSIAN_ROULETTE, 0))");
  if (enable && c->lights.on)
    return fail(c, PT_ERR_INVALID, "pt_set_debug_overlay: the debug overlay and PT_OPT_NEXT_EVENT exclude each other (turn next-event estimation off first: "
                                   "pt_set_option(ctx, PT_OPT_NEXT_EVENT, 0))");
  if (!enable) {
    c->dbg_enable = false;
    return PT_OK;
  }
  if (!c->state.uuid_valid && c->state.have_spheres) {
    int rc = upload_uuids(c, c->list.host.uuid);
    if (rc != PT_OK) return rc;
  }
  c->dbg_enable = true;
  c->dbg_selected = selected_object;
  for (int k = 0; k < 3; k++) c->dbg_cursor[k] = cursor_point[k];
  return PT_OK;
}

PT_API int pt_last_trace_build(pt_ctx* c) {
  if (!c) return PT_ERR_INVALID;
  return c->last_build;
}

PT_API int pt_render_features(pt_ctx* c) {
  if (!c) return PT_ERR_INVALID;
  if (c->count_work) return fail(c, PT_ERR_INVALID, "pt_render_features: not with PT_OPT_COUNT_WORK (the measuring twins have no feature build)");
  PT_TRY(scene_and_uniforms(c, "pt_render_features"));
  if (!c->feat.on) return option_off(c, "pt_render_features", SET_FEATURES);
  PT_HIP(c, hipSetDevice(c->device));
  if (is_capturing(c)) return fail(c, PT_ERR_INVALID, "pt_render_features: not inside a stream capture");
  if (!c->feat.in_place(extent_of(c))) return fail(c, PT_ERR_CAPACITY, "pt_render_features: the planes are not allocated for the rows in place (an earlier allocation failed)");
  if (c->local_rows == 0) { c->feat.valid = true; return PT_OK; }
  LaunchUse use;
  use.door = DOOR_FEATURES;
  use.who = "pt_render_features";
  if (int rc = trace_once(c, 1, use); rc != PT_OK) return rc;
  c->feat.valid = true;
  return PT_OK;
}

PT_API int pt_features_ptr(pt_ctx* c, int plane, void** dev_ptr, size_t* bytes) {
  if (!c || !dev_ptr) return fail(c, PT_ERR_INVALID, "pt_features_ptr: NULL argument");
  if (plane < 0 || plane >= PT_FEAT_PLANES) return fail(c, PT_ERR_INVALID, "pt_features_ptr: plane %d out of range", plane);
  if (!c->feat.on) return option_off(c, "pt_features_ptr", SET_FEATURES);
  if (!c->feat.in_place(extent_of(c))) return fail(c, PT_ERR_CAPACITY, "pt_features_ptr: the planes are not allocated for the rows in place (an earlier allocation failed)");
  *dev_ptr = c->feat.planes.get() + (size_t)plane * n_pixels(c);
  if (bytes) *bytes = n_pixels(c) * sizeof(float4);
  return PT_OK;
}

PT_API int pt_read_features(pt_ctx* c, int plane, void* out) {
  if (!c || !out) return fail(c, PT_ERR_INVALID, "pt_read_features: NULL argument");
  if (plane < 0 || plane >= PT_FEAT_PLANES) return fail(c, PT_ERR_INVALID, "pt_read_features: plane %d out of range", plane);
  if (c->count_work) return fail(c, PT_ERR_INVALID, "pt_read_features: not with PT_OPT_COUNT_WORK");
  if (!c->feat.on) return option_off(c, "pt_read_features", SET_FEATURES);
  if (!c->feat.valid)
    return fail(c, PT_ERR_NOT_READY, "pt_read_features: no pt_render_features since the scene, the uniforms or the size last changed");
  PT_HIP(c, hipSetDevice(c->device));
  if (is_capturing(c)) return fail(c, PT_ERR_INVALID, "pt_read_features: not inside a stream capture (a read-out synchronises)");
  const size_t need = n_pixels(c) * sizeof(float4);
  if (need) PT_HIP(c, hipMemcpyAsync(out, c->feat.planes.get() + (size_t)plane * n_pixels(c), need, hipMemcpyDefault, c->stream));
  PT_HIP(c, hipStreamSynchronize(c->stream));
  return PT_OK;
}

static bool device_pointer(const void* p) {
  hipPointerAttribute_t attr;
  if (hipPointerGetAttributes(&attr, p) != hipSuccess) {
    (void)hipGetLastError();
    return false;
  }
  return attr.type == hipMemoryTypeDevice || attr.type == hipMemoryTypeManaged;
}

PT_API uint32_t pt_query_batch(pt_ctx* c) {
  if (!c || !c->query.on || !c->state.have_spheres || !c->state.have_params || c->local_rows == 0 || !c->query.in_place(extent_of(c))) return 0u;
  return (uint32_t)n_pixels(c);
}

static int query_ready(pt_ctx* c, const char* who, const char* build, const void* rays, const void* out) {
  if (!rays || !out) return fail(c, PT_ERR_INVALID, "%s: NULL argument", who);
  if (c->count_work) return fail(c, PT_ERR_INVALID, "%s: not with PT_OPT_COUNT_WORK (the measuring twins have no %s build)", who, build);
  if (!c->query.on) return option_off(c, who, SET_QUERIES);
  PT_TRY(scene_and_uniforms(c, who));
  PT_HIP(c, hipSetDevice(c->device));
  PT_TRY(not_capturing(c, who));
  if (c->local_rows == 0) return fail(c, PT_ERR_NOT_READY, "%s: this band owns no rows, so it has no work items to decode rays against", who);
  if (!c->query.in_place(extent_of(c))) return fail(c, PT_ERR_CAPACITY, "%s: the planes are not allocated for the rows in place (an earlier allocation failed)", who);
  return frame_buffers_ready(c, who);
}

static int stage_rays(pt_ctx* c, const PtRay* rays, bool on_device, uint32_t m, std::vector<ptq::F4>& h_in) {
  ptq::F4* planes = reinterpret_cast<ptq::F4*>(c->query.planes.get());
  uint32_t plane = (uint32_t)n_pixels(c);
  if (on_device) {
    void* kargs[] = {&rays, &m, &planes, &plane};
    PT_HIP(c, hipLaunchKernel(pt_query_pack_kernel_handle(), dim3((m + 255u) / 256u), dim3(256), kargs, 0, c->stream));
    return PT_OK;
  }
  h_in.resize(2 * (size_t)m);
  for (uint32_t i = 0; i < m; i++) ptq::pack_ray(rays[i], &h_in[i], &h_in[(size_t)m + i]);
  PT_HIP(c, hipMemcpyAsync(planes + (size_t)PT_FEAT_POINT * plane, h_in.data(), (size_t)m * sizeof(ptq::F4), hipMemcpyHostToDevice, c->stream));
  PT_HIP(c, hipMemcpyAsync(planes + (size_t)PT_FEAT_NORMAL * plane, h_in.data() + m, (size_t)m * sizeof(ptq::F4), hipMemcpyHostToDevice, c->stream));
  return PT_OK;
}

static int estimator_ready(pt_ctx* c, const char* who, bool next_event) {
  if (!next_event) return PT_OK;
  if (!c->lights.on) return option_off(c, who, SET_NEXT_EVENT);
  if (!c->lights.in_place()) return fail(c, PT_ERR_CAPACITY, "%s: PT_OPT_NEXT_EVENT's light table is not in place (a failed allocation: install the scene or turn the option on again)", who);
  return PT_OK;
}

static LaunchUse batch_use(const pt_ctx* c, Door door, uint32_t m) {
  LaunchUse use;
  use.door = door;
// ... 704 lines not shown
```

### ray_tracer_webgl_amd/csrc/pt_buffers.hpp

```cpp
#pragma once
#include <cstddef>
#include <cstdint>
#include <utility>

#include "../../include/ptrace.h"
#include "pt_gather.hpp"
#include "pt_glare.hpp"

namespace ptbuf {

int dev_malloc(void** p, size_t bytes);
int dev_free(void* p);

template <class T>
struct DevBuf {
  DevBuf() = default;
  DevBuf(const DevBuf&) = delete;
  DevBuf& operator=(const DevBuf&) = delete;
  DevBuf(DevBuf&& o) noexcept : p_(o.p_), cap_(o.cap_) { o.p_ = nullptr; o.cap_ = 0; }
  DevBuf& operator=(DevBuf&& o) noexcept { std::swap(p_, o.p_); std::swap(cap_, o.cap_); return *this; }
  ~DevBuf() { if (p_) (void)dev_free(p_); }
  int reserve(size_t n) {
    int e = 0;
    if (p_) e = dev_free(p_);
// ... 138 lines not shown

  bool fits(const Extent& e) const { return planes.capacity() == plane_texels(e.pix) && order.capacity() == e.tiles; }
  Fit fit(const Extent& e) {
    Fit f;
    if (!on || fits(e)) return f;
    if (!planes_indexable(e.pix)) { f.capped = true; return f; }
    planes.release();
    if (refit(f, order, e.tiles, ORDER)) refit(f, planes, plane_texels(e.pix), PLANES);
    return f;
  }
  bool in_place(const Extent& e) const { return on && planes.holds(plane_texels(e.pix)) && order.holds(e.tiles); }
  void release() {
    on = false;
    planes.release(); order.release();
  }
};

template <class Texel>
struct HistorySet {
  enum : uint32_t { PLANES = 1, TALLY = 2 };
  bool on = false;
  bool valid = false;
  bool ran = false;
  PtParams params{};
  DevBuf<Texel> planes;
  DevBuf<unsigned long long> tally;

  Fit fit(const Extent& e) {
    Fit f;
    if (!on) return f;
    if (planes.capacity() != 2 * e.pix) {
      valid = false;
      if (!refit(f, planes, 2 * e.pix, PLANES)) return f;
    }
    if (tally.capacity() < 3) refit(f, tally, 3, TALLY);
    return f;
  }
  bool in_place(const Extent& e) const { return on && planes.holds(2 * e.pix) && tally.holds_at_least(3); }
  void release() {
    on = valid = ran = false;
    planes.release(); tally.release();
  }
};

struct ExposureSet {
  enum : uint32_t { STATE = 1 };
  static constexpr size_t kTallies = 258, kWords = kTallies + sizeof(PtExposure) / sizeof(uint32_t);
  bool on = false;
  bool valid = false;
  DevBuf<uint32_t> state;

  Fit fit() {
    Fit f;
    if (!on || state.holds(kWords)) return f;
    valid = false;
    refit(f, state, kWords, STATE);
    return f;
  }
  bool in_place() const { return on && state.holds(kWords); }
  void release() {
    on = valid = false;
    state.release();
  }
};

template <class Texel>
struct GlareSet {
  enum : uint32_t { PYRAMID = 1 };
  bool on = false;
  DevBuf<Texel> pyramid;

  static size_t texels(uint32_t width, uint32_t rows) {
    const size_t n = ptglare::pyramid_texels(width, rows, PT_GLARE_MAX_LEVELS);
    return n ? n : 1;
  }
  Fit fit(uint32_t width, uint32_t rows) {
    Fit f;
    if (!on || pyramid.holds(texels(width, rows))) return f;
    refit(f, pyramid, texels(width, rows), PYRAMID);
    return f;
  }
  bool in_place(uint32_t width, uint32_t rows) const { return on && pyramid.holds(texels(width, rows)); }
  void release() {
    on = false;
    pyramid.release();
  }
};

struct GatherSet {
  enum : uint32_t { WORK = 1 };
  static constexpr size_t kSlot = (size_t)ptgather::kLanes * ptgather::kMaxAcc, kCarry = 2 * kSlot, kPoint = 8, kRecord = 28;
  DevBuf<float> work;

  static size_t items(const Extent& e) { return e.pix / ptgather::kMinDirections + 2; }
  static size_t floats(const Extent& e) { return kCarry + (kPoint + kRecord) * items(e); }
  Fit fit(const Extent& e) {
    Fit f;
    if (work.holds_at_least(floats(e))) return f;
    refit(f, work, floats(e), WORK);
    return f;
  }
  bool in_place(const Extent& e) const { return work.holds_at_least(floats(e)); }
  float* carry(uint32_t slot) const { return work.get() + (slot & 1u) * kSlot; }
  float* points() const { return work.get() + kCarry; }
  float* records(const Extent& e) const { return work.get() + kCarry + kPoint * items(e); }
  void release() { work.release(); }
};

struct ProbeSet {
  enum : uint32_t { POINTS = 1, STAGE = 2 };
  static constexpr size_t kPoint = 8, kRecord = 28;
  DevBuf<float> points, stage;

  Fit fit_points(size_t nodes) {
    Fit f;
    if (!points.holds_at_least(kPoint * (nodes ? nodes : 1))) refit(f, points, kPoint * (nodes ? nodes : 1), POINTS);
    return f;
  }
  Fit fit_stage(size_t nodes) {
    Fit f;
    if (!stage.holds_at_least(kRecord * (nodes ? nodes : 1))) refit(f, stage, kRecord * (nodes ? nodes : 1), STAGE);
    return f;
  }
  bool points_in_place(size_t nodes) const { return points.holds_at_least(kPoint * (nodes ? nodes : 1)); }
  bool stage_in_place(size_t nodes) const { return stage.holds_at_least(kRecord * (nodes ? nodes : 1)); }
  void release_points() { points.release(); }
  void release_stage() { stage.release(); }
};

template <class Record>
struct LightSet {
  enum : uint32_t { TABLE = 1 };
  bool on = false;
  uint32_t n = 0;
  DevBuf<Record> table;

  Fit fit(uint32_t n_lights) {
    Fit f;
    n = 0;
    if (!on) return f;
    const size_t want = n_lights ? n_lights : 1u;
    if (table.capacity() < want && !refit(f, table, want, TABLE)) return f;
    n = n_lights;
    return f;
  }
  bool in_place() const { return on && table.holds_at_least(n ? n : 1u); }
  void release() {
    on = false;
    n = 0;
    table.release();
  }
};

}
```

### ray_tracer_webgl_amd/csrc/pt_kernel_args.h

```cpp
#pragma once
#include <stdint.h>

struct PtMatRec {
  float albedo[3];
  float fuzz;
  float refraction_index;
  int32_t type;
  float radius;
  float inv_ri;
};
static_assert(sizeof(PtMatRec) == 32, "PtMatRec must be 32 bytes");
struct PtDiv {
  uint32_t m, s1, s2;
};
static inline PtDiv pt_div_make(uint32_t d) {
  PtDiv r;
  uint32_t l = 0;
  while (l < 32 && (1ull << l) < (unsigned long long)d) l++;
  r.m = (uint32_t)(((1ull << 32) * ((1ull << l) - d)) / d + 1ull);
  r.s1 = l < 1 ? l : 1;
  r.s2 = l > 0 ? l - 1 : 0;
  return r;
}

struct PtKernelArgs {
  float origin[3], horizontal[3], vertical[3], llc[3], cam_u[3], cam_v[3];
  float lens_radius;
  float time0, time_step;
  uint32_t first_pass;
  int32_t spp;
  int32_t max_depth;
  int32_t background_mode;
  uint32_t width, height;
  uint32_t local_rows;
  uint32_t band_rows, band_index, band_count;
  uint32_t n_passes;
  uint32_t n_spheres;
  uint32_t scene_regular;
  uint32_t tiles_x, tiles_y;
  uint32_t n_items;
  const float* geom;
  const PtMatRec* mat;
  float* slab;
  unsigned long long* counters;
  const uint32_t* tile_order;
  uint32_t* tile_cost;
  const uint32_t* bvh_nodes;
  const float* bvh_nodes32;
  const float* bvh_slots;
  const uint32_t* bvh_slot_index;
  const PtMatRec* slot_mat;
  uint32_t n_nodes, n_tree_slots, n_slots, n_outliers;
  float bvh_c0[3], bvh_s0;
  const uint32_t* grid_cells;
  uint32_t n_cells;
  uint32_t grid_n[3];
  float grid_lo[3], grid_hi[3], grid_h[3], grid_inv_h[3];
  float grid_r2_near;
  float grid_lo_n[3], grid_hi_n[3];
  uint32_t lds_scene_bytes;
  unsigned long long* wave_log;
  uint32_t refill_min;
  uint32_t carry_lanes;
  float bvh_kinv;
  uint32_t block_threads;
  uint32_t queue_chunk;
  float fw, fh;
  PtDiv div_per_tile, div_tiles_x, div_band_rows;
  uint32_t coop_max_live;
  int32_t rr_min_depth;
  uint32_t lens_off;
  uint32_t queue_groups;
  uint32_t queue_static;
  uint32_t n_waves;
  uint32_t cost_feedback;
  uint32_t* cell_hist;
  const uint32_t* frame_ctr;
  const float* mat_r0;
  const int32_t* uuid;
  const int32_t* slot_uuid;
  float dbg_cursor[3];
  int32_t dbg_selected;
  uint32_t refill_ahead;
};

#ifndef PT_WAVES_WALK
#define PT_WAVES_WALK 6
#endif
#ifndef PT_WAVES_LIST
#define PT_WAVES_LIST 7
#endif
#define PT_WAVES_LIST_LDS 6
#ifndef PT_WAVES_SMALL
#define PT_WAVES_SMALL 7
#endif
#define PT_WAVES_TWIN_CELLS 4
#define PT_BUILT_FOR(n) __attribute__((amdgpu_waves_per_eu(n, n)))
#ifndef PT_LEAF_GROUP_GMEM
#define PT_LEAF_GROUP_GMEM 4
#endif

enum { PT_WAVE_LOG_WORDS = 4 };
enum { PT_COH_BINS = 66, PT_HIST_WAVE_STRIDE = 8 };
enum { PT_REG_REFILL_DECODE = 0, PT_REG_REFILL_RESERVE, PT_REG_CAMERA_RAY, PT_REG_SHADE_HIT_RECORD, PT_REG_SHADE_SKY, PT_REG_SHADE_DIFFUSE,
       PT_REG_SHADE_METAL, PT_REG_SHADE_GLASS, PT_REG_SHADE_GLASS_REFRACT, PT_REG_SHADE_CONTINUES, PT_REG_SHADE_FINISHED, PT_REG_SHADE_ITEM_STORE,
       PT_REG_WALK_ENTRY, PT_REG_WALK_ENTER_CELL, PT_REG_WALK_FAR_RAY, PT_REG_SHADE_ANY,
       PT_REG_REFILL_PROMOTE , PT_N_REGIONS };
enum { PT_CTR_HEAD = 0, PT_CTR_SEGMENTS = 1, PT_CTR_SAMPLES = 2, PT_CTR_FAR_RAYS = 3 , PT_CTR_REGIONS_MORE = 4 , PT_CTR_SCRATCH = 7 , PT_CTR_WORK = 8, PT_CTR_LITERAL = 16, PT_CTR_PHASES = 24, PT_N_PHASES = 8, PT_CTR_REGIONS = 32, PT_CTR_TIMEBINS = 64, PT_CTR_COUNT = 128,
       PT_QUEUE_GROUPS_MAX = 256, PT_CTR_GROUP_HEADS = 128 ,
       PT_CTR_ALLOC = PT_CTR_GROUP_HEADS + 8 * PT_QUEUE_GROUPS_MAX };

#define PT_LDS_ENTRIES(n) ((((n) + 7u) & ~7u) + 4u)
#define PT_MAX_SPHERES_SMALL 16u
#define PT_MAX_SPHERES_LDS 10232u
#define PT_PARK_DWORDS 14u
#ifndef PT_PARK_STRIDE
#define PT_PARK_STRIDE 15u
#endif
#define PT_BVH_LDS_BYTES32(n_nodes, n_slots) ((((size_t)(n_nodes) + 1u) * 2u + (size_t)(n_slots)) * 16u)
#define PT_BVH_LDS_BYTES16(n_nodes) (((size_t)(n_nodes) + 1u) * 16u)
#define PT_GRID_LDS_CELLS(n_cells) ((((size_t)(n_cells) + 3u) / 4u) * 16u)
#define PT_MAX_SPHERES 65528u

enum {
  PT_PROBE_HASH = 0,
  PT_PROBE_SINCOS = 1,
  PT_PROBE_CBRT = 2,
  PT_PROBE_UNIT_SPHERE = 3,
  PT_PROBE_DIVSQRT = 4,
  PT_PROBE_BASE_HASH = 5,
  PT_PROBE_FAST_ARITH = 6,
};
```

### ray_tracer_webgl_amd/csrc/pt_kernels.hip

```cpp
#include "pt_trace_body.hpp"

PT_MAIN_KERNELS(PT_TRACE_KERNEL)

extern "C" const void* pt_main_kernel(int id) {
  switch (id) {
    PT_MAIN_KERNELS(PT_TRACE_KERNEL_CASE)
    default: return nullptr;
  }
}

extern "C" __global__ __launch_bounds__(1024) void pt_tile_order_kernel(uint32_t* cost, uint32_t* order,
                                                                        uint32_t n_tiles) {
  __shared__ uint32_t s_hist[1024];
  __shared__ uint32_t s_scan[1024];
  __shared__ uint32_t s_max;
  const uint32_t t = threadIdx.x;
  if (t == 0) s_max = 0;
  s_hist[t] = 0;
  __syncthreads();
  uint32_t m = 0;
  for (uint32_t i = t; i < n_tiles; i += 1024) m = cost[i] > m ? cost[i] : m;
  atomicMax(&s_max, m);
  __syncthreads();
  const uint32_t mx = s_max;
  if (mx == 0) {
    for (uint32_t i = t; i < n_tiles; i += 1024) order[i] = i;
    return;
  }
  const float scale = 1023.0f / (float)mx;
  for (uint32_t i = t; i < n_tiles; i += 1024) {
    uint32_t b = 1023u - (uint32_t)((float)cost[i] * scale);
    atomicAdd(&s_hist[b > 1023u ? 0u : b], 1u);
  }
  __syncthreads();
  s_scan[t] = s_hist[t];
  __syncthreads();
  for (uint32_t off = 1; off < 1024; off <<= 1) {
    uint32_t v = t >= off ? s_scan[t - off] : 0u;
    __syncthreads();
    s_scan[t] += v;
    __syncthreads();
  }
  s_hist[t] = s_scan[t] - s_hist[t];
  __syncthreads();
  for (uint32_t i = t; i < n_tiles; i += 1024) {
    uint32_t b = 1023u - (uint32_t)((float)cost[i] * scale);
    uint32_t pos = atomicAdd(&s_hist[b > 1023u ? 0u : b], 1u);
    order[pos] = i;
  }
  __syncthreads();
  for (uint32_t i = t; i < n_tiles; i += 1024) cost[i] = 0;
}

extern "C" __global__ __launch_bounds__(256) void pt_accumulate_kernel(float4* accum,
                                                                       const float4* slab,
                                                                       uint32_t n_pix,
                                                                       uint32_t n_passes) {
  uint32_t stride = gridDim.x * blockDim.x;
  for (uint32_t i = blockIdx.x * blockDim.x + threadIdx.x; i < n_pix; i += stride) {
    float4 acc = accum[i];
    for (uint32_t p = 0; p < n_passes; p++) {
      float4 s = slab[(size_t)p * n_pix + i];
      acc.x += s.x; acc.y += s.y; acc.z += s.z; acc.w += s.w;
    }
    accum[i] = acc;
  }
}

__device__ __forceinline__ uint32_t unorm8(float v) {
  if (!(v > 0.0f)) return 0u;
  if (v >= 1.0f) return 255u;
  return (uint32_t)(v * 255.0f + 0.5f);
}

__device__ __forceinline__ float pixel_scale(float w) { return w > 0.0f ? 1.0f / w : 0.0f; }

struct BlendRule {
  float rc, lfw, total, y_total, y255;
  bool averaging;
  bool total_ok;
};
__device__ __forceinline__ BlendRule blend_rule(int render_count, int should_average, float last_frame_weight) {
  BlendRule B;
  B.rc = (float)render_count;
  B.lfw = last_frame_weight;
  B.total = B.rc + last_frame_weight;
  B.total_ok = ptk::div_den_ok(B.total);
  B.y_total = ptk::rcp_newton(B.total_ok ? B.total : 1.0f);
  B.y255 = ptk::rcp_newton(255.0f);
  B.averaging = should_average && render_count > 1;
  return B;
}
__device__ __forceinline__ uint32_t blend_texel(const float4 v, const uint32_t pv, const BlendRule& B) {
  using namespace ptk;
  const float scale = pixel_scale(v.w);
  const float x0 = v.x * scale, x1 = v.y * scale, x2 = v.z * scale;
  float px[3] = {sqrt_core(x0), sqrt_core(x1), sqrt_core(x2)};
  const uint32_t lo = f2u(0x1p-96f), span = 0x7f800000u - f2u(0x1p-96f);
  bool odd = (f2u(x0) != 0u && f2u(x0) - lo > span) || (f2u(x1) != 0u && f2u(x1) - lo > span) || (f2u(x2) != 0u && f2u(x2) - lo > span);
  uint32_t o = 255u << 24;
  const bool merge = B.averaging && (pv >> 24) != 0u;
  float m[3] = {px[0], px[1], px[2]};
  if (B.averaging) {
    const float n_lo = 0x1p-103f;
#pragma unroll
    for (int c = 0; c < 3; c++) {
      const float pr = div_core((float)((pv >> (8 * c)) & 255u), 255.0f, B.y255);
      const float num = fma_(px[c], B.lfw, pr * B.rc);
      const float q = div_core(num, B.total, B.y_total);
      odd = odd || (merge && !(B.total_ok && (f2u(num) == 0u || f2u(num) - f2u(n_lo) < f2u(0x1p76f) - f2u(n_lo))));
      m[c] = merge ? q : px[c];
    }
  }
  if (__builtin_expect(pt_ballot(odd) != 0ull, 0)) {
    if (odd) {
      m[0] = px[0] = __builtin_sqrtf(x0); m[1] = px[1] = __builtin_sqrtf(x1); m[2] = px[2] = __builtin_sqrtf(x2);
      if (merge) {
#pragma unroll
        for (int c = 0; c < 3; c++) {
          const float pr = (float)((pv >> (8 * c)) & 255u) / 255.0f;
          m[c] = fma_(px[c], B.lfw, pr * B.rc) / B.total;
        }
      }
    }
  }
  o |= unorm8(m[0]) | (unorm8(m[1]) << 8) | (unorm8(m[2]) << 16);
  return o;
}

extern "C" __global__ __launch_bounds__(256) void pt_resolve_kernel(const float4* accum, float4* out,
                                                                    uint32_t n_pix, int gamma) {
  uint32_t stride = gridDim.x * blockDim.x;
  for (uint32_t i = blockIdx.x * blockDim.x + threadIdx.x; i < n_pix; i += stride) {
    float4 v = accum[i];
    const float scale = pixel_scale(v.w);
    float r = v.x * scale, g = v.y * scale, b = v.z * scale;
    if (gamma) { r = __builtin_sqrtf(r); g = __builtin_sqrtf(g); b = __builtin_sqrtf(b); }
    out[i] = make_float4(r, g, b, 1.0f);
  }
}

extern "C" __global__ __launch_bounds__(256) void pt_resolve_rgba8_kernel(const float4* accum,
                                                                          uint32_t* out, uint32_t n_pix,
                                                                          int gamma) {
  uint32_t stride = gridDim.x * blockDim.x;
  for (uint32_t i = blockIdx.x * blockDim.x + threadIdx.x; i < n_pix; i += stride) {
    float4 v = accum[i];
    const float scale = pixel_scale(v.w);
    float r = v.x * scale, g = v.y * scale, b = v.z * scale;
    if (gamma) { r = __builtin_sqrtf(r); g = __builtin_sqrtf(g); b = __builtin_sqrtf(b); }
    out[i] = unorm8(r) | (unorm8(g) << 8) | (unorm8(b) << 16) | (255u << 24);
  }
}

extern "C" __global__ __launch_bounds__(256) void pt_blend_rgba8_kernel(
    const float4* accum, const uint32_t* prev, uint32_t* out, uint32_t n_pix,
    int render_count, int should_average, float last_frame_weight) {
  uint32_t stride = gridDim.x * blockDim.x;
  const BlendRule B = blend_rule(render_count, should_average, last_frame_weight);
  for (uint32_t i = blockIdx.x * blockDim.x + threadIdx.x; i < n_pix; i += stride) {
    const uint32_t o = blend_texel(accum[i], prev[i], B);
    out[i] = o;
  }
}

extern "C" __global__ __launch_bounds__(256) void pt_frame_blend_kernel(
    const float4* slab, uint32_t* tex0, uint32_t* tex1, uint32_t* canvas, uint32_t n_pix, const uint32_t* ctr, uint32_t k_off,
    int render_count0, uint32_t even_odd0, int max_render_count, int should_average, float last_frame_weight) {
  const uint32_t k = ctr[0] + k_off;
  const long long rc_ll = (long long)render_count0 + (long long)k;
  const int render_count = rc_ll < (long long)max_render_count ? (int)rc_ll : max_render_count;
  const uint32_t even_odd = even_odd0 + k;
  const uint32_t* prev = ((even_odd + 1u) & 1u) ? tex1 : tex0;
  uint32_t* out_tex = (even_odd & 1u) ? tex1 : tex0;
  uint32_t stride = gridDim.x * blockDim.x;
  const BlendRule B = blend_rule(render_count, should_average, last_frame_weight);
  for (uint32_t i = blockIdx.x * blockDim.x + threadIdx.x; i < n_pix; i += stride) {
    const uint32_t o = blend_texel(slab[i], prev[i], B);
    canvas[i] = o;
    if (should_average) out_tex[i] = o;
  }
}

extern "C" __global__ __launch_bounds__(256) void pt_frames_blend_kernel(
    const float4* slab, uint32_t n_frames, uint32_t* tex0, uint32_t* tex1, uint32_t* canvas, uint32_t n_pix, const uint32_t* ctr,
    int render_count0, uint32_t even_odd0, int max_render_count, int should_average, float last_frame_weight) {
  const uint32_t k0 = ctr[0];
  uint32_t stride = gridDim.x * blockDim.x;
  for (uint32_t i = blockIdx.x * blockDim.x + threadIdx.x; i < n_pix; i += stride) {
    uint32_t pv = 0u, o = 0u;
    auto frame = [&](uint32_t f, const float4 v) {
      const uint32_t k = k0 + f;
      const long long rc_ll = (long long)render_count0 + (long long)k;
      const int render_count = rc_ll < (long long)max_render_count ? (int)rc_ll : max_render_count;
      const BlendRule B = blend_rule(render_count, should_average, last_frame_weight);
      const uint32_t even_odd = even_odd0 + k;
      if (f == 0u || !should_average) pv = (((even_odd + 1u) & 1u) ? tex1 : tex0)[i];
      else pv = o;
      o = blend_texel(v, pv, B);
      if (should_average && f + 2u >= n_frames) ((even_odd & 1u) ? tex1 : tex0)[i] = o;
    };
    uint32_t f = 0;
    for (; f + 8u <= n_frames; f += 8u) {
      float4 v[8];
// ... 82 lines not shown
```

### ray_tracer_webgl_amd/csrc/pt_refill.hpp

```cpp
#pragma once
#include "pt_scene.hpp"
#include "pt_query.hpp"

namespace ptk {

struct PixelDiv {
  bool wh_ok;
  float y_fw, y_fh;
};
__device__ __forceinline__ PixelDiv pixel_div() {
  karg_t& K = *kargs();
  PixelDiv pd;
  pd.wh_ok = div_den_ok(K.fw) && div_den_ok(K.fh);
  pd.y_fw = u2f((uint32_t)__builtin_amdgcn_readfirstlane((int)f2u(rcp_newton(K.fw))));
  pd.y_fh = u2f((uint32_t)__builtin_amdgcn_readfirstlane((int)f2u(rcp_newton(K.fh))));
  return pd;
}

template <bool FEAT = false, bool QRY = false, bool RAD = false>
__device__ __forceinline__ void start_sample(Path& p, const PixelDiv& pd) {
  karg_t& K = *kargs();
  if constexpr (RAD) {
    const uint32_t j = f2u(p.st_s), plane = K.local_rows * K.width;
    const float4* rays = reinterpret_cast<const float4*>(K.uuid);
    const float4 qo = rays[2u * plane + j], qd = rays[plane + j];
    const V3 o = mk(qo.x, qo.y, qo.z), d = mk(qd.x, qd.y, qd.z);
    p.o = o; p.d = d; p.a = dot3(d, d); p.col = mk(1.0f, 1.0f, 1.0f); p.depth = 0;
    return;
  }
  if constexpr (QRY) {
    const uint32_t i = p.slab_index, plane = K.local_rows * K.width;
    const float4* planes = reinterpret_cast<const float4*>(K.slab);
    const float4 qo = planes[2u * plane + i], qd = planes[plane + i];
    const V3 o = mk(qo.x, qo.y, qo.z), d = mk(qd.x, qd.y, qd.z);
    p.o = o; p.d = d; p.a = dot3(d, d); p.col = mk(1.0f, 1.0f, 1.0f); p.depth = 0;
    return;
  }
  if constexpr (FEAT) {
    const float s = p.st_s, t = p.st_t;
    const V3 dd = mk(fma_(t, K.vertical[0], fma_(s, K.horizontal[0], K.llc[0])),
                     fma_(t, K.vertical[1], fma_(s, K.horizontal[1], K.llc[1])),
                     fma_(t, K.vertical[2], fma_(s, K.horizontal[2], K.llc[2])));
    const V3 cam_o = mk(K.origin[0], K.origin[1], K.origin[2]);
    const V3 d = mk(dd.x - cam_o.x, dd.y - cam_o.y, dd.z - cam_o.z);
    p.o = cam_o; p.d = d; p.a = dot3(d, d); p.col = mk(1.0f, 1.0f, 1.0f); p.depth = 0;
    return;
  }
  float seed = p.seed;
  const float st_s = p.st_s, st_t = p.st_t;
  const bool wh_ok = pd.wh_ok;
  const float y_fw = pd.y_fw, y_fh = pd.y_fh;
  V3 o, d; float a; V3 col; int depth;
  float r0, r1;
  hash2(seed, r0, r1);
  float jx, jy;
  if (wh_ok) { jx = div_core(r0, K.fw, y_fw); jy = div_core(r1, K.fh, y_fh); }
  else { jx = r0 / K.fw; jy = r1 / K.fh; }
  float s = st_s + jx;
  float t = st_t + jy;
  V3 dd = mk(fma_(t, K.vertical[0], fma_(s, K.horizontal[0], K.llc[0])),
             fma_(t, K.vertical[1], fma_(s, K.horizontal[1], K.llc[1])),
             fma_(t, K.vertical[2], fma_(s, K.horizontal[2], K.llc[2])));
  const V3 cam_o = mk(K.origin[0], K.origin[1], K.origin[2]);
  const V3 tt = mk(dd.x - cam_o.x, dd.y - cam_o.y, dd.z - cam_o.z);
  float seed_l = seed;
  seed = (seed + 0.1f) + 0.1f;
  seed = (seed + 0.1f) + 0.1f;
  bool lens = K.lens_off == 0u;
  if (!lens) {
    const uint32_t nz = 0x80000000u;
    lens = pt_ballot(f2u(tt.x) == nz || f2u(tt.y) == nz || f2u(tt.z) == nz) != 0ull;
  }
  if (lens) {
    float ua = hash1(seed_l);
    float sa, ca;
    sincos2pi(ua, sa, ca);
    float rr = sqrt_rn(hash1(seed_l));
    float rdx = K.lens_radius * (rr * ca);
    float rdy = K.lens_radius * (rr * sa);
    V3 off = mk(fma_(K.cam_v[0], rdy, K.cam_u[0] * rdx), fma_(K.cam_v[1], rdy, K.cam_u[1] * rdx),
                fma_(K.cam_v[2], rdy, K.cam_u[2] * rdx));
    d = mk(tt.x - off.x, tt.y - off.y, tt.z - off.z);
    o = mk(cam_o.x + off.x, cam_o.y + off.y, cam_o.z + off.z);
  } else {
    d = tt;
    o = cam_o;
  }
  a = dot3(d, d);
  col = mk(1.0f, 1.0f, 1.0f);
  depth = 0;
  p.seed = seed; p.o = o; p.d = d; p.a = a; p.col = col; p.depth = depth;
}

__device__ __forceinline__ bool query_admit(uint32_t i) {
  karg_t& K = *kargs();
  if (i >= (uint32_t)K.dbg_selected) return false;
  const uint32_t plane = K.local_rows * K.width;
  float4* planes = reinterpret_cast<float4*>(K.slab);
  const float4 qo = planes[2u * plane + i], qd = planes[plane + i];
  if (ptq::ray_valid(qo.x, qo.y, qo.z, qd.x, qd.y, qd.z)) return true;
  ptq::F4 t_alb, t_n, t_hp; ptq::I4 t_ids;
  ptq::invalid_texels(&t_alb, &t_n, &t_hp, &t_ids);
  planes[i] = make_float4(t_alb.x, t_alb.y, t_alb.z, t_alb.w);
  planes[plane + i] = make_float4(t_n.x, t_n.y, t_n.z, t_n.w);
  planes[2u * plane + i] = make_float4(t_hp.x, t_hp.y, t_hp.z, t_hp.w);
  reinterpret_cast<int4*>(planes)[3u * plane + i] = make_int4(t_ids.x, t_ids.y, t_ids.z, t_ids.w);
  return false;
}

__device__ __forceinline__ bool radiance_admit(uint32_t j) {
  karg_t& K = *kargs();
  if (j >= (uint32_t)K.dbg_selected) return false;
  const uint32_t plane = K.local_rows * K.width;
  const float4* rays = reinterpret_cast<const float4*>(K.uuid);
  const float4 qo = rays[2u * plane + j], qd = rays[plane + j];
  return ptq::ray_valid(qo.x, qo.y, qo.z, qd.x, qd.y, qd.z);
}

template <bool COUNT, bool QRY = false, bool RAD = false>
__device__ __forceinline__ void refill(const PtKernelArgs& A, Path& p, Queue& q, const PixelDiv& pd, Tally<COUNT>& tally) {
  karg_t& K = *kargs();
  const bool alive = p.alive;
  bool dry = q.dry;
  uint32_t nx_slab = p.nx_slab, nx_tile = p.nx_tile;
  float nx_seed = p.nx_seed, nx_s = p.nx_s, nx_t = p.nx_t;
  uint32_t pool_next = q.pool_next, pool_end = q.pool_end;
  uint32_t pool_tp0 = q.pool_tp0, pool_split = q.pool_split, pool_tile0 = q.pool_tile0, pool_tile1 = q.pool_tile1;
  uint32_t q_round = q.round;
  const bool wh_ok = pd.wh_ok;
  const float y_fw = pd.y_fw, y_fh = pd.y_fh;
  for (;;) {
    const bool slot_empty = nx_slab == ptdeal::kSlotEmpty;
    if (pt_ballot(ptdeal::starving(alive, slot_empty, dry)) == 0ull) break;
    bool need = ptdeal::wants_item(alive, slot_empty, dry, K.refill_ahead != 0u);
    const unsigned long long mask = pt_ballot(need);
    if (ptdeal::pool_used_up(pool_next, pool_end)) {
      tally.flag(PT_REG_REFILL_RESERVE);
      unsigned long long base = 0;
      if (K.queue_static == 2u) {
        const uint32_t wave = blockIdx.x * (blockDim.x >> 6) + (threadIdx.x >> 6);
        const uint32_t group = ptdeal::group_of(wave, K.queue_groups);
        unsigned long long r = 0;
        if (lane_id() == 0u) r = atomicAdd(&A.counters[PT_CTR_GROUP_HEADS + 8u * group], 1ull);
        const uint32_t r_lo = (uint32_t)__builtin_amdgcn_readfirstlane((int)(uint32_t)r);
        base = ptdeal::grouped_base(r_lo, K.queue_groups, group, A.queue_chunk);
      } else if (K.queue_static != 0u) {
        const uint32_t wave = blockIdx.x * (blockDim.x >> 6) + (threadIdx.x >> 6);
        base = ptdeal::static_base(q_round, K.n_waves, wave, A.queue_chunk);
        q_round++;
      } else {
        if (lane_id() == 0u) base = atomicAdd(&A.counters[PT_CTR_HEAD], (unsigned long long)A.queue_chunk);
      }
      base = ((unsigned long long)(uint32_t)__builtin_amdgcn_readfirstlane((int)(uint32_t)(base >> 32)) << 32) |
             (unsigned long long)(uint32_t)__builtin_amdgcn_readfirstlane((int)(uint32_t)base);
      if (ptdeal::reservation_dry(base, A.n_items)) {
        tally.queue_dry();
        dry = true;
        need = false;
      } else {
        pool_next = (uint32_t)base;
        pool_end = ptdeal::reservation_end(base, A.queue_chunk, A.n_items);
        pool_tp0 = div_by(pool_next, K.div_per_tile.m, K.div_per_tile.s1, K.div_per_tile.s2);
        pool_split = (pool_tp0 + 1u) * (64u * K.n_passes);
        const uint32_t n_tiles_w = K.tiles_x * K.tiles_y;
        pool_tile0 = (uint32_t)__builtin_amdgcn_readfirstlane((int)K.tile_order[pool_tp0]);
        pool_tile1 = (uint32_t)__builtin_amdgcn_readfirstlane((int)K.tile_order[pool_tp0 + 1u < n_tiles_w ? pool_tp0 + 1u : pool_tp0]);
      }
    }
    const uint32_t avail = pool_end - pool_next;
    const uint32_t rank = ptdeal::rank_of(mask, lane_id());
    const uint32_t pool_base = pool_next;
    pool_next += ptdeal::taken(mask, avail);
    if (ptdeal::gets_item(need, rank, avail)) {
      tally.flag(PT_REG_REFILL_DECODE);
      uint32_t item = ptdeal::item_of(pool_base, rank);
      uint32_t per_tile = 64u * K.n_passes;
      uint32_t tile_pos, tile;
      if (K.queue_chunk <= per_tile) {
        const bool second = item >= pool_split;
        tile_pos = pool_tp0 + (second ? 1u : 0u);
        const uint32_t t0 = pool_tile0, t1 = pool_tile1;
        tile = second ? t1 : t0;
      } else {
        tile_pos = div_by(item, K.div_per_tile.m, K.div_per_tile.s1, K.div_per_tile.s2);
        tile = K.tile_order[tile_pos];
      }
      uint32_t rem_i = item - tile_pos * per_tile;
      uint32_t pass = rem_i >> 6, l = rem_i & 63u;
      uint32_t ty = div_by(tile, K.div_tiles_x.m, K.div_tiles_x.s1, K.div_tiles_x.s2), tx = tile - ty * K.tiles_x;
      uint32_t px = tx * 8u + (l & 7u), ly = ty * 8u + (l >> 3);
      bool inside = px < K.width && ly < K.local_rows;
      if constexpr (QRY) { if (inside) inside = query_admit((pass * K.local_rows + ly) * K.width + px); }
      if constexpr (RAD) { if (inside) inside = radiance_admit(ly * K.width + px); }
      if (inside) {
        uint32_t y = ly;
        if (K.band_count > 1u) {
          uint32_t b = div_by(ly, K.div_band_rows.m, K.div_band_rows.s1, K.div_band_rows.s2), r = ly - b * K.band_rows;
          y = (b * K.band_count + K.band_index) * K.band_rows + r;
        }
        const float fx2 = (float)(2u * px + 1u), fy2 = (float)(2u * y + 1u);
        float vx, vy;
        if (wh_ok) { vx = div_core(fx2, K.fw, y_fw) - 1.0f; vy = div_core(fy2, K.fh, y_fh) - 1.0f; }
        else { vx = fx2 / K.fw - 1.0f; vy = fy2 / K.fh - 1.0f; }
        const uint32_t frame_k = *(const uint32_t __attribute__((address_space(4)))*)K.frame_ctr;
        float u_time = K.time0 + (float)(K.first_pass + pass + frame_k) * K.time_step;
        nx_seed = (float)base_hash(f2u(vx), f2u(vy)) * (1.0f / 4294967296.0f) + u_time;
        nx_s = (vx + 1.0f) * 0.5f;
        nx_t = (vy + 1.0f) * 0.5f;
        if constexpr (RAD) nx_s = u2f(ly * K.width + px);
        nx_slab = (pass * K.local_rows + ly) * K.width + px;
        nx_tile = (pass == 0u && K.cost_feedback != 0u) ? tile : 0xffffffffu;
      }
    }
  }
  p.nx_slab = nx_slab; p.nx_tile = nx_tile; p.nx_seed = nx_seed; p.nx_s = nx_s; p.nx_t = nx_t;
  q.pool_next = pool_next; q.pool_end = pool_end;
  q.pool_tp0 = pool_tp0; q.pool_split = pool_split; q.pool_tile0 = pool_tile0; q.pool_tile1 = pool_tile1;
  q.round = q_round; q.dry = dry;
}

template <bool COUNT>
__device__ __forceinline__ void promote(Path& p, Tally<COUNT>& tally) {
  if (ptdeal::promotes(p.alive, p.nx_slab == ptdeal::kSlotEmpty)) {
    tally.flag(PT_REG_REFILL_PROMOTE);
    p.seed = p.nx_seed; p.st_s = p.nx_s; p.st_t = p.nx_t;
    p.slab_index = p.nx_slab; p.item_tile = p.nx_tile; p.item_segs = 0;
    p.sum = mk(0.f, 0.f, 0.f);
    p.sample = 0;
    p.new_path = true;
    p.alive = true;
    p.nx_slab = ptdeal::kSlotEmpty;
  }
}

}
```

### ray_tracer_webgl_amd/csrc/pt_scene.hpp

```cpp
#pragma once
#include "pt_arith.hpp"
#include "pt_deal.hpp"
#include "pt_kernel_args.h"

namespace ptk {
using namespace ptd;

extern __shared__ float4 pt_lds[];

typedef float f4v __attribute__((ext_vector_type(4)));
typedef const f4v __attribute__((address_space(4))) const_f4v;
typedef const PtKernelArgs __attribute__((address_space(4))) karg_t;

__device__ __forceinline__ karg_t* kargs() { return (karg_t*)__builtin_amdgcn_kernarg_segment_ptr(); }

__device__ __forceinline__ uint32_t lane_id() { return threadIdx.x & 63u; }

__device__ __forceinline__ uint32_t div_by(uint32_t n, uint32_t m, uint32_t s1, uint32_t s2) {
  const uint32_t t = __umulhi(m, n);
  return (t + ((n - t) >> s1)) >> s2;
}

struct Path {
  bool alive = false;
  bool new_path = false;
  uint32_t slab_index = 0;
  uint32_t item_tile = 0xffffffffu, item_segs = 0;
  int sample = 0, depth = 0;
  float seed = 0.f, st_s = 0.f, st_t = 0.f;
  V3 o = mk(0, 0, 0), d = mk(0, 0, 0);
  float a = 0.f;
  V3 col = mk(1, 1, 1), sum = mk(0, 0, 0);
  uint32_t nx_slab = ptdeal::kSlotEmpty, nx_tile = 0xffffffffu;
  float nx_seed = 0.f, nx_s = 0.f, nx_t = 0.f;
};

template <bool NEE>
struct NeeState {};
template <>
struct NeeState<true> {
  uint32_t bits = 0u;
  float wgt = 0.f;
  V3 nd = mk(0, 0, 0);
  __device__ __forceinline__ bool pending() const { return (bits & 1u) != 0u; }
  __device__ __forceinline__ bool sampled() const { return (bits & 2u) != 0u; }
  __device__ __forceinline__ int light() const { return (int)(bits >> 2); }
  __device__ __forceinline__ void set_sampled(bool on) { bits = on ? 2u : 0u; }
  __device__ __forceinline__ void set_pending(int k) { bits = 3u | ((uint32_t)k << 2); }
  __device__ __forceinline__ void clear_pending() { bits = 2u; }
};

template <bool NEE> struct NeeArgOf { typedef NeeState<false> type; };
template <> struct NeeArgOf<true> { typedef NeeState<true>& type; };

template <bool RAD>
__device__ __forceinline__ const float4* nee_light_table(karg_t* K) {
  if constexpr (RAD) return reinterpret_cast<const float4*>(K->slot_uuid);
  else return reinterpret_cast<const float4*>(K->uuid);
}
template <bool RAD>
__device__ __forceinline__ int nee_light_count(karg_t* K) {
  if constexpr (RAD) return __float_as_int(K->dbg_cursor[0]);
  else return K->dbg_selected;
}

struct Queue {
  uint32_t pool_next = 0, pool_end = 0;
  uint32_t pool_tp0 = 0, pool_split = 0, pool_tile0 = 0, pool_tile1 = 0;
  uint32_t round = 0;
  bool dry = false;
};

struct Hit {
  float closest = PT_MAX_T;
  int hit = -1;
  uint32_t lit_from = 0xffffffffu;
};

struct Carry {
  bool carried = false;
  float closest_w = PT_MAX_T;
  uint32_t hit_pos = 0xffffffffu;
};
struct BvhWalk {
  uint32_t cur = 0, l0 = 0, l1 = 0, l2 = 0, l3 = 0, l_cnt = 0;
  uint32_t q0 = 0, q1 = 0, q2 = 0, q3 = 0, q_cnt = 0;
};
struct GridWalk {
  float tmx = 0.f, tmy = 0.f, tmz = 0.f, t_exit = 0.f;
  uint32_t cell = 0, rem = 0, pend = 0;
};

template <bool SCAN_LDS_, bool HAVE_LDS_, int WALK_, int TAIL_ = -1, bool FLAT_Y_ = false>
struct Scene {
  static constexpr bool SCAN_LDS = SCAN_LDS_, HAVE_LDS = HAVE_LDS_;
  static constexpr int WALK = WALK_;
  static constexpr bool BVH = WALK >= 1 && WALK <= 3;
  static constexpr bool GRID = WALK >= 4 && WALK <= 6;
  static constexpr bool FLAT_Y = FLAT_Y_;
  static_assert(!FLAT_Y_ || WALK_ == 4, "the one-layer walk exists for the LDS-staged grid build");
  static constexpr bool SMALL = WALK == 7;
  static constexpr int SMALL_TAIL = TAIL_;
  static_assert(TAIL_ >= -1 && TAIL_ <= 3 && (TAIL_ < 0 || WALK_ == 7), "a list remainder belongs to the small-list kernel");
  static constexpr bool TREE = BVH || GRID;
  static constexpr int BVH_MODE = BVH ? WALK : 0;
  static constexpr bool NODES_LDS = WALK == 1 || WALK == 2;
  static constexpr bool CELLS_LDS = WALK == 4 || WALK == 5;
  static_assert(HAVE_LDS || !SCAN_LDS, "an LDS scan needs the LDS copy");
  static_assert(!TREE || (!SCAN_LDS && !HAVE_LDS), "the walk kernels read list-order data from global memory");

  static __device__ __forceinline__ void stage(const PtKernelArgs& A) {
    const float4* __restrict__ g_geom = reinterpret_cast<const float4*>(A.geom);
    const uint4* __restrict__ g_nodes = reinterpret_cast<const uint4*>(A.bvh_nodes);
    const float4* __restrict__ g_nodes32 = reinterpret_cast<const float4*>(A.bvh_nodes32);
    const float4* __restrict__ g_slots = reinterpret_cast<const float4*>(A.bvh_slots);
    if constexpr (HAVE_LDS && !TREE) {
      const uint32_t n_padded = PT_LDS_ENTRIES(A.n_spheres);
      for (uint32_t i = threadIdx.x; i < n_padded; i += blockDim.x) pt_lds[i] = g_geom[i];
      __syncthreads();
    }
    if constexpr (WALK == 1) {
      const uint32_t n_a = 2u * (A.n_nodes + 1u);
      typedef float4 __attribute__((address_space(3))) lds_f4s;
      const uint32_t lds_base = (uint32_t)(uintptr_t)(lds_f4s*)pt_lds;
      for (uint32_t i = threadIdx.x; i < n_a; i += blockDim.x) {
        float4 v = g_nodes32[i];
        if ((i & 1u) == 0u) v.w = u2f(f2u(v.w) + lds_base);
        pt_lds[i] = v;
      }
      for (uint32_t i = threadIdx.x; i < A.n_slots; i += blockDim.x) pt_lds[n_a + i] = g_slots[i];
      __syncthreads();
    }
    if constexpr (WALK == 2) {
      const uint32_t n_a = A.n_nodes + 1u;
      uint4* s_nodes = reinterpret_cast<uint4*>(pt_lds);
      for (uint32_t i = threadIdx.x; i < n_a; i += blockDim.x) s_nodes[i] = g_nodes[i];
      __syncthreads();
    }
    if constexpr (CELLS_LDS) {
      const uint32_t n_c4 = (A.n_cells + 3u) >> 2;
      const uint4* g_c4 = reinterpret_cast<const uint4*>(A.grid_cells);
      uint4* s_c4 = reinterpret_cast<uint4*>(pt_lds);
      for (uint32_t i = threadIdx.x; i < n_c4; i += blockDim.x) s_c4[i] = g_c4[i];
      if constexpr (WALK == 4)
        for (uint32_t i = threadIdx.x; i < A.n_slots; i += blockDim.x) pt_lds[n_c4 + i] = g_slots[i];
      __syncthreads();
    }
  }

  static __device__ __forceinline__ float4 geom_scan(const PtKernelArgs& A, uint32_t i) {
    if constexpr (SCAN_LDS) {
      return pt_lds[i];
    } else {
      const f4v v = ((const_f4v*)A.geom)[i];
      return make_float4(v.x, v.y, v.z, v.w);
    }
  }
  static __device__ __forceinline__ float4 geom_at(const PtKernelArgs& A, uint32_t i) {
    if constexpr (HAVE_LDS && !TREE) {
      return pt_lds[i];
    } else {
      return reinterpret_cast<const float4*>(A.geom)[i];
    }
  }
  static __device__ __forceinline__ uint4 node_at(const PtKernelArgs& A, uint32_t i) {
    if constexpr (NODES_LDS) return reinterpret_cast<const uint4*>(pt_lds)[i];
    else return reinterpret_cast<const uint4*>(A.bvh_nodes)[i];
  }
  static __device__ __forceinline__ float4 slot_at(const PtKernelArgs& A, uint32_t i) {
    if constexpr (WALK == 1) return pt_lds[2u * (A.n_nodes + 1u) + i];
    else if constexpr (WALK == 4) return pt_lds[((A.n_cells + 3u) >> 2) + i];
    else return reinterpret_cast<const float4*>(A.bvh_slots)[i];
  }
  static __device__ __forceinline__ uint32_t cell_at(const PtKernelArgs& A, uint32_t i) {
    if constexpr (CELLS_LDS) return reinterpret_cast<const uint32_t*>(pt_lds)[i];
    else return A.grid_cells[i];
  }
  static __device__ __forceinline__ const_f4v* c_slots(const PtKernelArgs& A) { return (const_f4v*)A.bvh_slots; }
};

typedef volatile uint32_t __attribute__((address_space(3))) lds_u32;
__device__ __forceinline__ lds_u32* park_of(const PtKernelArgs& A) {
  return (lds_u32*)reinterpret_cast<uint32_t*>(pt_lds) + (A.lds_scene_bytes >> 2) + PT_PARK_STRIDE * threadIdx.x;
}
__device__ __forceinline__ void park_store(const PtKernelArgs& A, const Path& p) {
  lds_u32* ps = park_of(A);
  ps[0] = f2u(p.sum.x); ps[1] = f2u(p.sum.y); ps[2] = f2u(p.sum.z);
  ps[3] = f2u(p.col.x); ps[4] = f2u(p.col.y); ps[5] = f2u(p.col.z);
  ps[6] = f2u(p.seed);
  ps[7] = f2u(p.st_s); ps[8] = f2u(p.st_t);
  ps[12] = (uint32_t)p.sample; ps[13] = (uint32_t)p.depth;
  ps[9] = p.slab_index; ps[10] = p.item_tile; ps[11] = p.item_segs;
}
__device__ __forceinline__ void park_load(const PtKernelArgs& A, Path& p) {
  lds_u32* ps = park_of(A);
  p.sum = mk(u2f(ps[0]), u2f(ps[1]), u2f(ps[2]));
  p.col = mk(u2f(ps[3]), u2f(ps[4]), u2f(ps[5]));
  p.seed = u2f(ps[6]);
  p.st_s = u2f(ps[7]); p.st_t = u2f(ps[8]);
  p.sample = (int)ps[12]; p.depth = (int)ps[13];
  p.slab_index = ps[9]; p.item_tile = ps[10]; p.item_segs = ps[11];
}

static_assert(PT_PARK_STRIDE > PT_PARK_DWORDS, "the parking area has a spare dword per lane");
__device__ __forceinline__ void park_store(const PtKernelArgs& A, const NeeState<true>& ne) { park_of(A)[PT_PARK_DWORDS] = f2u(ne.wgt); }
__device__ __forceinline__ void park_load(const PtKernelArgs& A, NeeState<true>& ne) { ne.wgt = u2f(park_of(A)[PT_PARK_DWORDS]); }

template <bool COUNT>
struct Tally {
  unsigned long long t_wave_start = 0, t_wave_dry = 0;
  uint32_t lane_flags = 0, reg_acc = 0;
  uint32_t hw_id = 0, xcc_id = 0;
  uint32_t tb_bin = 0xffffffffu, tb_acc = 0;
  uint32_t n_walk_it = 0, n_walk_ln = 0, n_leaf_it = 0, n_leaf_ln = 0, n_exact_it = 0, n_exact_ln = 0, n_steps = 0,
           n_carried = 0;
  uint32_t n_walk_first = 0;
  uint32_t n_exact_always_it = 0, n_exact_always_ln = 0;
  bool in_always = false;
  unsigned long long ph_t[PT_N_PHASES] = {0, 0, 0, 0, 0, 0, 0, 0}, ph_mark = 0;

  __device__ __forceinline__ void start() {
    if constexpr (COUNT) {
      t_wave_start = __builtin_amdgcn_s_memrealtime();
// ... 124 lines not shown
```

### ray_tracer_webgl_amd/csrc/pt_shade.hpp

```cpp
#pragma once
#include "pt_nee.hpp"
#include "pt_scene.hpp"

namespace ptk {

template <typename S, bool RR, bool COUNT, bool DBG = false, bool FEAT = false, bool QRY = false, bool NEE = false, bool RAD = false>
__device__ __forceinline__ void shade_segment(const PtKernelArgs& A, Path& p, const Hit& h, const Carry& cw, Tally<COUNT>& tally, typename NeeArgOf<NEE>::type ne) {
  static_assert(!NEE || (!RR && !DBG && !FEAT && !COUNT), "next-event estimation excludes roulette, the overlay, the doors and the twins");
  tally.flag(PT_REG_SHADE_ANY);
  bool alive = p.alive, new_path = p.new_path;
  const uint32_t slab_index = p.slab_index; const uint32_t item_tile = p.item_tile; uint32_t item_segs = p.item_segs;
  int sample = p.sample, depth = p.depth; float seed = p.seed;
  V3 o = p.o, d = p.d; float a = p.a; V3 col = p.col, sum = p.sum;
  const float closest = h.closest; const int hit = h.hit; const uint32_t hit_pos = cw.hit_pos;
  (void)hit_pos;
  item_segs++;
  if constexpr (NEE) {
    if (ne.pending()) {
      int index = hit;
      if constexpr (S::TREE) {
        if (hit >= 0 && hit_pos != 0xffffffffu) index = (int)A.bvh_slot_index[hit_pos];
      }
      karg_t* K = kargs();
      const float4 l1 = nee_light_table<RAD>(K)[2 * ne.light() + 1];
      if (hit >= 0 && index == __float_as_int(l1.w)) {
        float s3[3] = {sum.x, sum.y, sum.z};
        const float t3[3] = {col.x, col.y, col.z}, a3[3] = {l1.x, l1.y, l1.z};
        ptnee::add(s3, t3, a3, ne.wgt);
        p.sum = mk(s3[0], s3[1], s3[2]);
      }
      ne.clear_pending();
      p.d = ne.nd; p.a = dot3(ne.nd, ne.nd);
      p.item_segs = item_segs;
      return;
    }
  }
  bool finished = false;
  bool nee_skip = false;
  (void)nee_skip;
  int mtype = -1;
  V3 hp = mk(0.f, 0.f, 0.f), n = hp, alb = hp; bool front = false; float fuzz = 0.f, ri = 1.f, inv_ri = 1.f;
  if (hit >= 0) {
    tally.flag(PT_REG_SHADE_HIT_RECORD);
    float4 g;
    if constexpr (S::TREE) {
      if (hit_pos != 0xffffffffu) g = S::slot_at(A, hit_pos);
      else g = S::geom_at(A, (uint32_t)hit);
    } else {
      g = S::geom_at(A, (uint32_t)hit);
    }
    const float4* mp = reinterpret_cast<const float4*>(A.mat + hit);
    if constexpr (S::TREE) {
      if (hit_pos != 0xffffffffu) mp = reinterpret_cast<const float4*>(A.slot_mat + hit_pos);
    }
    float4 m0 = mp[0];
    float4 m1 = mp[1];
    mtype = __float_as_int(m1.y);
    float radius = m1.z;
    fuzz = m0.w; ri = m1.x; inv_ri = m1.w;
    hp = mk(fma_(d.x, closest, o.x), fma_(d.y, closest, o.y), fma_(d.z, closest, o.z));
    const float nx = hp.x - g.x, ny = hp.y - g.y, nz = hp.z - g.z;
    V3 on;
    const float n_lo = __builtin_fminf(__builtin_fminf(__builtin_fabsf(nx), __builtin_fabsf(ny)), __builtin_fabsf(nz));
    const float n_hi = __builtin_fmaxf(__builtin_fmaxf(__builtin_fabsf(nx), __builtin_fabsf(ny)), __builtin_fabsf(nz));
    const uint32_t r_guard = div_den_ok(radius) ? f2u(0x1p76f) - f2u(0x1p-103f) : 0u;
    const bool n_odd = f2u(n_lo) - f2u(0x1p-103f) >= r_guard || f2u(n_hi) - f2u(0x1p-103f) >= r_guard;
    const float yr = rcp_newton(radius);
    on = mk(div_core(nx, radius, yr), div_core(ny, radius, yr), div_core(nz, radius, yr));
    if (__builtin_expect(pt_ballot(n_odd) != 0ull, 0)) {
      if (n_odd) on = mk(nx / radius, ny / radius, nz / radius);
    }
    front = dot3(d, on) < 0.0f;
    n = front ? on : mk(-on.x, -on.y, -on.z);
    alb = mk(m0.x, m0.y, m0.z);
    if constexpr (NEE) {
      if (ne.sampled() && mtype == 3) {
        const float x3[3] = {o.x, o.y, o.z}, c3[3] = {g.x, g.y, g.z};
        float w3[3], d2;
        const bool reached = ptnee::reach(x3, c3, g.w, w3, d2);
        nee_skip = reached && radius != 0.0f && ptnee::is_finite(m0.x) && ptnee::is_finite(m0.y) && ptnee::is_finite(m0.z);
      }
    }
    if constexpr (DBG) {
      karg_t* K = kargs();
      const V3 v = mk(hp.x - K->dbg_cursor[0], hp.y - K->dbg_cursor[1], hp.z - K->dbg_cursor[2]);
      const bool on_cursor = sqrt_rn(dot3(v, v)) < 0.1f;
      const int32_t* up = K->uuid + hit;
      if constexpr (S::TREE) {
        if (hit_pos != 0xffffffffu) up = K->slot_uuid + hit_pos;
      }
      const bool on_outline = *up == K->dbg_selected && dot3(n, d) > -0.05f;
      if (on_cursor || on_outline) {
        sum.x += on_cursor ? 0.0f : 1.0f; sum.y += 0.0f; sum.z += on_cursor ? 1.0f : 0.0f;
        mtype = 4;
      }
    }
  }
  if constexpr (FEAT) {
    karg_t* K = kargs();
    float4* planes = reinterpret_cast<float4*>(A.slab);
    const uint32_t plane = K->local_rows * K->width;
    float4 t_alb = make_float4(0.f, 0.f, 0.f, 0.f), t_n = t_alb, t_hp = t_alb;
    int4 t_ids = make_int4(-1, -1, -1, 0);
    if (hit >= 0) {
      int index = hit;
      const int32_t* up = K->uuid + hit;
      if constexpr (S::TREE) {
        if (hit_pos != 0xffffffffu) { index = (int)A.bvh_slot_index[hit_pos]; up = K->slot_uuid + hit_pos; }
      }
      t_alb = make_float4(alb.x, alb.y, alb.z, closest);
      t_n = make_float4(n.x, n.y, n.z, 0.f);
      t_hp = make_float4(hp.x, hp.y, hp.z, 0.f);
      t_ids = make_int4(index, *up, mtype, front ? 1 : 0);
    } else if (A.background_mode == 0) {
      const float uy = d.y * inv_sqrt_rn(a);
      const float t = 0.5f * (uy + 1.0f);
      const float omt = 1.0f - t;
      t_alb = make_float4(0.0f + col.x * fma_(0.5f, t, omt), 0.0f + col.y * fma_(0.7f, t, omt), 0.0f + col.z * fma_(1.0f, t, omt), 0.f);
    }
    planes[slab_index] = t_alb;
    planes[plane + slab_index] = t_n;
    planes[2u * plane + slab_index] = t_hp;
    reinterpret_cast<int4*>(planes)[3u * plane + slab_index] = t_ids;
    p.alive = false; p.new_path = false; p.item_segs = item_segs;
    return;
  }
  const bool sky = hit < 0 && A.background_mode == 0;
  const float inv = inv_sqrt_rn(a);
  float seed_drawn = seed;
  const uint32_t draw = seed_step_hash(seed_drawn);
  seed = (uint32_t)mtype <= 2u ? seed_drawn : seed;
  if (hit < 0) {
    if (sky) {
      tally.flag(PT_REG_SHADE_SKY);
      float uy = d.y * inv;
      float t = 0.5f * (uy + 1.0f);
      float omt = 1.0f - t;
      sum.x += col.x * fma_(0.5f, t, omt);
      sum.y += col.y * fma_(0.7f, t, omt);
      sum.z += col.z * fma_(1.0f, t, omt);
    }
    finished = true;
  } else {
    const V3 p = hp;
    if (mtype == 0 || mtype == 1) {
      V3 rs = random_in_unit_sphere_from(draw);
      V3 nd;
      bool ok = true;
      if (mtype == 0) {
        tally.flag(PT_REG_SHADE_DIFFUSE);
        V3 ruv = normalize3(rs);
        nd = mk(n.x + ruv.x, n.y + ruv.y, n.z + ruv.z);
      } else {
        tally.flag(PT_REG_SHADE_METAL);
        V3 refl = reflect3(d, n);
        nd = mk(fma_(fuzz, rs.x, refl.x), fma_(fuzz, rs.y, refl.y), fma_(fuzz, rs.z, refl.z));
        ok = dot3(n, nd) > 0.0f;
      }
      if (ok) {
        o = p; d = nd;
        col.x *= alb.x; col.y *= alb.y; col.z *= alb.z;
      } else {
        finished = true;
      }
    } else if (mtype == 2) {
      tally.flag(PT_REG_SHADE_GLASS);
      float ratio = front ? inv_ri : ri;
      V3 ud = mk(d.x * inv, d.y * inv, d.z * inv);
      float cdot = dot3(mk(-ud.x, -ud.y, -ud.z), n);
      float cos_theta = (1.0f < cdot) ? 1.0f : cdot;
      float sin_theta = sqrt_rn(fma_(-cos_theta, cos_theta, 1.0f));
      bool cannot_refract = ratio * sin_theta > 1.0f;
      float refl_amount;
      if constexpr (S::SMALL) {
        const float r0 = A.mat_r0[2u * (uint32_t)hit + (front ? 0u : 1u)];
        const float x = 1.0f - cos_theta, x2 = x * x, x5 = (x2 * x2) * x;
        refl_amount = fma_(1.0f - r0, x5, r0);
      } else {
        refl_amount = reflectance(cos_theta, ratio);
      }
      float rnd = (float)draw * (1.0f / 4294967296.0f);
      V3 nd;
      if (cannot_refract || refl_amount > rnd) {
        nd = reflect3(ud, n);
      } else {
        tally.flag(PT_REG_SHADE_GLASS_REFRACT);
        float dni = dot3(n, ud);
        float k = fma_(-(ratio * ratio), fma_(-dni, dni, 1.0f), 1.0f);
        if (k < 0.0f) {
          nd = mk(0.f, 0.f, 0.f);
        } else {
          float t = fma_(ratio, dni, sqrt_rn(k));
          nd = mk(fma_(-t, n.x, ratio * ud.x), fma_(-t, n.y, ratio * ud.y),
                  fma_(-t, n.z, ratio * ud.z));
        }
      }
      o = p; d = nd;
      col.x *= alb.x; col.y *= alb.y; col.z *= alb.z;
    } else if (mtype == 3) {
      if constexpr (NEE) {
        if (!nee_skip) { sum.x += col.x * alb.x; sum.y += col.y * alb.y; sum.z += col.z * alb.z; }
      } else {
        sum.x += col.x * alb.x; sum.y += col.y * alb.y; sum.z += col.z * alb.z;
      }
      finished = true;
    } else {
      finished = true;
    }
    if (!finished) {
      tally.flag(PT_REG_SHADE_CONTINUES);
      a = dot3(d, d);
      depth++;
      if (depth >= A.max_depth) {
        sum.x += col.x; sum.y += col.y; sum.z += col.z;
        finished = true;
      }
      if constexpr (RR) if (!finished && depth >= A.rr_min_depth) {
        const float q = __builtin_fminf(__builtin_fmaxf(__builtin_fmaxf(col.x, col.y), col.z), 1.0f);
        const float xi = hash1(seed);
        if (!(xi < q)) {
          finished = true;
        } else {
          const float inv = 1.0f / q;
          col.x *= inv; col.y *= inv; col.z *= inv;
        }
      }
      if constexpr (NEE) {
        karg_t* K = kargs();
        const int n_lights = nee_light_count<RAD>(K);
        const bool smp = !finished && mtype == 0 && n_lights > 0;
        ne.set_sampled(smp);
        if (smp) {
          float u0, u1, u2;
          hash3(seed, u0, u1, u2);
          const int k = ptnee::choose(u0, n_lights);
          const float4 l0 = nee_light_table<RAD>(K)[2 * k];
          const float x3[3] = {o.x, o.y, o.z}, c3[3] = {l0.x, l0.y, l0.z};
          float w3[3], d2;
          if (ptnee::reach(x3, c3, l0.w, w3, d2)) {
            float sp, cp, om3[3], om;
            sincos2pi(u2, sp, cp);
            ptnee::sample(w3, d2, l0.w, u1, sp, cp, om3, om);
            const float n3[3] = {n.x, n.y, n.z};
            const float cos_s = ptnee::cos_at(n3, om3);
            if (cos_s > 0.0f) {
              ne.set_pending(k); ne.wgt = ptnee::weight(n_lights, om, cos_s);
              ne.nd = d;
              d = mk(om3[0], om3[1], om3[2]);
              a = dot3(d, d);
            }
          }
        }
      }
    }
  }
  if constexpr (NEE) { if (finished) ne.set_sampled(false); }

  if (finished) {
    tally.flag(PT_REG_SHADE_FINISHED);
    sample++;
    if (sample >= A.spp) {
      tally.flag(PT_REG_SHADE_ITEM_STORE);
      float4 outv = make_float4(sum.x, sum.y, sum.z, (float)A.spp);
      reinterpret_cast<float4*>(A.slab)[slab_index] = outv;
      if (item_tile != 0xffffffffu) atomicMax(&A.tile_cost[item_tile], item_segs);
      alive = false;
    } else {
      new_path = true;
    }
  }
  p.alive = alive; p.new_path = new_path; p.item_segs = item_segs;
  p.sample = sample; p.depth = depth; p.seed = seed;
  p.o = o; p.d = d; p.a = a; p.col = col; p.sum = sum;
}

}
```

### ray_tracer_webgl_amd/csrc/pt_trace_body.hpp

```cpp
#pragma once
#include <hip/hip_runtime.h>
#include <stdint.h>

#include "pt_kernel_args.h"
#include "pt_extra.h"
#include "pt_arith.hpp"
#include "pt_scene.hpp"
#include "pt_refill.hpp"
#include "pt_list.hpp"
#include "pt_bvh_walk.hpp"
#include "pt_grid_walk.hpp"
#include "pt_shade.hpp"

using namespace ptd;

namespace ptb {
struct Defaults {
  static constexpr bool SCAN_LDS = false, HAVE_LDS = false, COUNT = false, RR = false, FLAT_Y = false, DBG = false, FEAT = false, QRY = false, RAD = false, NEE = false;
  static constexpr int WALK = 0, TAIL = -1;
};
struct ListLds : Defaults { static constexpr bool SCAN_LDS = true, HAVE_LDS = true; };
struct Scalar : Defaults { static constexpr bool HAVE_LDS = true; };
struct ScalarNolds : Defaults {};
template <int T> struct Small : Defaults { static constexpr bool HAVE_LDS = true; static constexpr int WALK = 7, TAIL = T; };
struct Bvh : Defaults { static constexpr int WALK = 1; };
struct BvhNodes : Defaults { static constexpr int WALK = 2; };
struct BvhGmem : Defaults { static constexpr int WALK = 3; };
struct GridLayers : Defaults { static constexpr int WALK = 4; };
struct Grid : GridLayers { static constexpr bool FLAT_Y = true; };
struct GridCells : Defaults { static constexpr int WALK = 5; };
struct GridGmem : Defaults { static constexpr int WALK = 6; };
template <class Row> struct Count : Row { static constexpr bool COUNT = true; };
template <class Row> struct Rr : Row { static constexpr bool RR = true; };
template <class Row> struct Dbg : Row { static constexpr bool DBG = true; };
template <class Row> struct Feat : Row { static constexpr bool FEAT = true; };
template <class Row> struct Qry : Row { static constexpr bool FEAT = true, QRY = true; };
template <class Row> struct Rad : Row { static constexpr bool RAD = true; };
template <class Row> struct Nee : Row { static constexpr bool NEE = true; };
template <class Row> using RadNee = Nee<Rad<Row>>;
}

#define PT_TRACE_KERNEL(sym, waves, Build) \
  extern "C" __global__ __launch_bounds__(1024) PT_BUILT_FOR(waves) void sym(const PtKernelArgs A) { using namespace ptb; pt_trace_body<Build>(A); }
#define PT_TRACE_KERNEL_CASE(sym, waves, Build) case PT_KERNEL_ID(sym): return reinterpret_cast<const void*>(sym);
#define PT_TRACE_VARIANT(stem, waves, Row, suffix, Adaptor) PT_TRACE_KERNEL(stem##suffix, waves, Adaptor<Row>)
#define PT_TRACE_VARIANT_CASE(stem, waves, Row, suffix, Adaptor) case PT_VARIANT_ID(stem): return reinterpret_cast<const void*>(stem##suffix);
#define PT_VARIANT_ACCESSOR(name, suffix, Adaptor)             \
  extern "C" const void* name(int id) {                        \
    switch (id) {                                              \
      PT_VARIANT_ROWS(PT_TRACE_VARIANT_CASE, suffix, Adaptor)  \
      default: return nullptr;                                 \
    }                                                          \
  }

template <class B>
__device__ __forceinline__ void pt_trace_body(const PtKernelArgs& A) {
  using namespace ptk;
  constexpr bool SCAN_LDS = B::SCAN_LDS, HAVE_LDS = B::HAVE_LDS, COUNT = B::COUNT, RR = B::RR, FLAT_Y = B::FLAT_Y, DBG = B::DBG, FEAT = B::FEAT, QRY = B::QRY, RAD = B::RAD, NEE = B::NEE;
  constexpr int WALK = B::WALK, TAIL = B::TAIL;
  using S = Scene<SCAN_LDS, HAVE_LDS, WALK, TAIL, FLAT_Y>;
  S::stage(A);

  Path p;
  Queue q;
  Carry cw;
  BvhWalk bw;
  GridWalk gw;
  Tally<COUNT> tally;
  const PixelDiv pd = pixel_div();
  uint32_t seg_count = 0;
  tally.start();
  NeeState<NEE> ne;

  for (;;) {
    refill<COUNT, QRY, RAD>(A, p, q, pd, tally);
    promote<COUNT>(p, tally);
    tally.phase(0);
    if (p.alive && p.new_path) {
      tally.flag(PT_REG_CAMERA_RAY);
      start_sample<FEAT, QRY, RAD>(p, pd);
      p.new_path = false;
    }
    tally.phase(1);
    const unsigned long long live = pt_ballot(p.alive);
    if (live == 0ull) break;
    tally.step();

    Hit h;
    if constexpr (S::TREE) h.closest = cw.carried ? cw.closest_w : PT_MAX_T;
    if (!cw.carried) cw.hit_pos = 0xffffffffu;
    const bool fast = regular_ray(A, p);
    const int n_live = (int)__popcll(live);
    if constexpr (S::TREE) park_store(A, p);
    if constexpr (S::TREE && NEE) park_store(A, ne);
    constexpr bool kTail = !S::TREE && !S::SMALL;
    const bool coop = kTail && (n_live <= (int)A.coop_max_live) && (pt_ballot(p.alive && !fast) == 0ull) &&
                      (pt_ballot(cw.carried) == 0ull);
    if (coop) {
      tail_mode<S>(A, p, live, h);
    } else {
      h.lit_from = fast ? 0xffffffffu : 0u;
      const bool scan_lane = p.alive && fast;
      if constexpr (S::BVH) bvh_walk<S, COUNT>(A, p, scan_lane, n_live, cw, bw, h, tally);
      else if constexpr (S::GRID) grid_walk<S, COUNT>(A, p, scan_lane, n_live, cw, gw, h, tally);
      else if constexpr (S::SMALL) small_scan<S>(A, p, scan_lane, h);
      else list_scan<S>(A, p, scan_lane, h);
      tally.literal(A, p.alive && !fast, scan_lane && h.lit_from < A.n_spheres, p.slab_index);
      if constexpr (S::GRID && S::WALK != 4) {
        const bool handed_over = scan_lane && h.lit_from == 0u;
        const unsigned long long m_h = pt_ballot(handed_over);
        if (m_h != 0ull) {
          tail_mode<S>(A, p, m_h, h);
          if (handed_over) h.lit_from = 0xffffffffu;
        }
      }
      literal_loop<S>(A, p, h);
    }
    if constexpr (S::TREE) {
      if (coop) cw.carried = false;
      cw.closest_w = h.closest;
      park_load(A, p);
      if constexpr (NEE) park_load(A, ne);
    }
    tally.phase(6);

    const bool shade = p.alive && !cw.carried;
    seg_count += (uint32_t)__popcll(pt_ballot(shade));
    tally.timebin(A, shade);
    if (shade) shade_segment<S, RR, COUNT, DBG, FEAT, QRY, NEE, RAD>(A, p, h, cw, tally, ne);
    tally.collect();
    tally.phase(7);
  }

  if (lane_id() == 0) atomicAdd(&A.counters[PT_CTR_SEGMENTS], (unsigned long long)seg_count);
  tally.flush(A);
}
```

### ray_tracer_webgl_amd/tracer.py

```python
import ctypes as C

import numpy as np

from . import abi
from ._lib import load


class PtError(RuntimeError):
    def __init__(self, code, message):
        super().__init__("libptrace error %d: %s" % (code, message))
        self.code = code


class PathTracer:
    def __init__(self, width, height, device=0, use_torch=False):
        self.lib = load()
        self.width, self.height = int(width), int(height)
        self.device = int(device)
        self._ctx = C.c_void_p()
        self.use_torch = bool(use_torch)
        stream_handle = None
        if self.use_torch:
            import torch

            self._torch = torch
            try:
                stream = torch.cuda.current_stream(self.device)
            except RuntimeError as e:
                raise PtError(abi.PT_ERR_NO_DEVICE, "PyTorch cannot see the GPU libptrace is using (%s): two HIP runtimes in one "
                              "process?  `import torch` before anything of ray_tracer_webgl_amd" % e) from e
            stream_handle = C.c_void_p(stream.cuda_stream or abi.PT_STREAM_LEGACY)
            rc = self.lib.pt_create_on_stream(C.byref(self._ctx), self.device, self.width, self.height, stream_handle)
        else:
            rc = self.lib.pt_create(C.byref(self._ctx), self.device, self.width, self.height)
        if rc != abi.PT_OK:
            msg = self.lib.pt_last_error(None)
            self._ctx = C.c_void_p()
            raise PtError(rc, msg.decode() if msg else "pt_create failed")
        self.params = None
        self.local_rows = self.height
        self.accum_tensor = None
        self._keep = None

    def _check(self, rc):
        if rc != abi.PT_OK:
            msg = self.lib.pt_last_error(self._ctx)
            raise PtError(rc, msg.decode() if msg else "")
        return rc

    def close(self):
        if self._ctx:
            self.lib.pt_destroy(self._ctx)
            self._ctx = C.c_void_p()

    def __del__(self):
        try:
            self.close()
        except Exception:
            pass

    def __enter__(self):
        return self

    def __exit__(self, *exc):
        self.close()

    def set_spheres(self, spheres):
        ptr, n, keep = abi.spheres_as_ctypes(spheres)
        self._check(self.lib.pt_set_spheres(self._ctx, ptr, n))
        self.n_spheres = n

    def set_params(self, params):
        self.params = params.copy()
        rows = abi.local_rows(self.height, params.band_rows, params.band_index, params.band_count)
        if self.use_torch and self.accum_tensor is not None and self.accum_tensor.shape[0] != max(rows, 1):
            self._check(self.lib.pt_bind_accum(self._ctx, None, 0))
            self.accum_tensor = None
        self._check(self.lib.pt_set_params(self._ctx, C.byref(self.params)))
        self.local_rows = rows
        if self.use_torch:
            self._bind_torch_accum()

    def _bind_torch_accum(self):
        torch = self._torch
        shape = (max(self.local_rows, 1), self.width, 4)
        if self.accum_tensor is None or tuple(self.accum_tensor.shape) != shape:
            self.accum_tensor = torch.zeros(shape, dtype=torch.float32, device="cuda:%d" % self.device)
            nbytes = self.accum_tensor.numel() * 4
            self._check(self.lib.pt_bind_accum(self._ctx, C.c_void_p(self.accum_tensor.data_ptr()), nbytes))

    def set_geometry_path(self, path):
        self._check(self.lib.pt_set_option(self._ctx, abi.PT_OPT_GEOMETRY_PATH, int(path)))

    def set_count_work(self, on=True):
        self._check(self.lib.pt_set_option(self._ctx, abi.PT_OPT_COUNT_WORK, int(on)))

    def set_carry_lanes(self, n):
        self._check(self.lib.pt_set_option(self._ctx, abi.PT_OPT_CARRY_LANES, int(n)))

    def set_refill_min(self, n):
        self._check(self.lib.pt_set_option(self._ctx, abi.PT_OPT_REFILL_MIN, int(n)))

    def set_russian_roulette(self, min_depth):
        self._check(self.lib.pt_set_option(self._ctx, abi.PT_OPT_RUSSIAN_ROULETTE, int(min_depth)))

    def next_event(self, on=True):
        self._check(self.lib.pt_set_option(self._ctx, abi.PT_OPT_NEXT_EVENT, 1 if on else 0))

    def set_debug_overlay(self, enable, selected_object=abi.NO_SELECTED_OBJECT_ID, cursor_point=(0.0, 0.0, 0.0)):
        cur = (C.c_float * 3)(*[float(x) for x in cursor_point])
        self._check(self.lib.pt_set_debug_overlay(self._ctx, 1 if enable else 0, int(selected_object), cur))

    def last_trace_build(self):
        rc = self.lib.pt_last_trace_build(self._ctx)
        if rc < 0:
            raise PtError(rc, "pt_last_trace_build failed")
        return rc

    def set_grid_fit(self, unmeasured):
        self._check(self.lib.pt_set_option(self._ctx, abi.PT_OPT_GRID_FIT, 1 if unmeasured else 0))

    def tune(self, n_passes):
        self._check(self.lib.pt_tune(self._ctx, int(n_passes)))
        if self.accum_tensor is not None:
            self.accum_tensor.zero_()

    def refit_grid(self, only_if_stale=False):
        self._check(self.lib.pt_refit_grid(self._ctx, 1 if only_if_stale else 0))

    def grid_fit(self):
        rc = self.lib.pt_grid_fit(self._ctx)
        if rc < 0:
            raise PtError(rc, "pt_grid_fit failed")
        return rc

    def reserve_passes(self, n):
        self._check(self.lib.pt_reserve_passes(self._ctx, int(n)))

    def render(self):
        self._check(self.lib.pt_render(self._ctx))

    def render_passes(self, n):
        self._check(self.lib.pt_render_passes(self._ctx, int(n)))

    def reset(self):
        self._check(self.lib.pt_reset_accum(self._ctx))
        if self.accum_tensor is not None:
            self.accum_tensor.zero_()

    def synchronize(self):
        self._check(self.lib.pt_synchronize(self._ctx))

    def wait(self, timeout_s):
        fn = self.lib.pt_debug_wait
        fn.restype, fn.argtypes = C.c_int, [C.c_void_p, C.c_uint]
        rc = fn(self._ctx, int(timeout_s * 1000))
        if rc < 0:
            raise PtError(rc, "pt_debug_wait failed")
        return rc == 0

    def clear_textures(self):
        self._check(self.lib.pt_clear_textures(self._ctx))

    def render_frame(self, even_odd_count):
        self._check(self.lib.pt_render_frame(self._ctx, int(even_odd_count) & 0xFFFFFFFF))

    def render_frames(self, even_odd_count, max_render_count, n_frames):
        self._check(self.lib.pt_render_frames(self._ctx, int(even_odd_count) & 0xFFFFFFFF, int(max_render_count), int(n_frames)))

    def read_canvas(self):
        out = np.empty((self.local_rows, self.width, 4), dtype=np.uint8)
        if out.size:
            self._check(self.lib.pt_read_canvas(self._ctx, out.ctypes.data_as(C.c_void_p)))
        return out

    def read_texture(self, index):
        out = np.empty((self.local_rows, self.width, 4), dtype=np.uint8)
        if out.size:
            self._check(self.lib.pt_read_texture(self._ctx, int(index), out.ctypes.data_as(C.c_void_p)))
        return out

    def write_texture(self, index, rgba8):
        a = np.ascontiguousarray(rgba8, dtype=np.uint8)
        if a.shape != (self.local_rows, self.width, 4):
            raise ValueError("texture is %s, this context holds %s" % (a.shape, (self.local_rows, self.width, 4)))
        self._check(self.lib.pt_write_texture(self._ctx, int(index), a.ctypes.data_as(C.c_void_p)))

    def resolve(self, gamma=True):
        out = np.empty((self.local_rows, self.width, 4), dtype=np.float32)
        if out.size:
            self._check(self.lib.pt_resolve(self._ctx, out.ctypes.data_as(C.c_void_p), 1 if gamma else 0))
        return out

    def resolve_rgba8(self, gamma=True):
        out = np.empty((self.local_rows, self.width, 4), dtype=np.uint8)
        if out.size:
            self._check(self.lib.pt_resolve_rgba8(self._ctx, out.ctypes.data_as(C.c_void_p), 1 if gamma else 0))
        return out

    def blend_rgba8(self, prev):
        prev = np.ascontiguousarray(prev, dtype=np.uint8)
        out = np.empty_like(prev)
        self._check(self.lib.pt_blend_rgba8(self._ctx, prev.ctypes.data_as(C.c_void_p), out.ctypes.data_as(C.c_void_p)))
        return out

    def accum(self):
        self.synchronize()
        if self.accum_tensor is not None:
            self._torch.cuda.current_stream(self.device).synchronize()
            return self.accum_tensor[: self.local_rows].cpu().numpy()
        out = np.empty((self.local_rows, self.width, 4), dtype=np.float32)
        if out.size:
            self._check(self.lib.pt_read_accum(self._ctx, out.ctypes.data_as(C.c_void_p), out.nbytes))
        return out

    def load_accum(self, accum):
        a = np.ascontiguousarray(accum, dtype=np.float32)
        if a.shape != (self.local_rows, self.width, 4):
            raise ValueError("accumulation checkpoint is %s, this context holds %s"
                             % (a.shape, (self.local_rows, self.width, 4)))
        self._check(self.lib.pt_load_accum(self._ctx, a.ctypes.data_as(C.c_void_p), a.nbytes))

    def error_estimate(self, on=True):
        self._check(self.lib.pt_set_option(self._ctx, abi.PT_OPT_ERROR_ESTIMATE, 1 if on else 0))

    def error_state(self):
        ptr, nbytes = C.c_void_p(), C.c_size_t()
        self._check(self.lib.pt_error_ptr(self._ctx, C.byref(ptr), C.byref(nbytes)))
        self.synchronize()
        out = np.empty((self.local_rows, self.width, 2, 4), dtype=np.float32)
        assert out.nbytes == nbytes.value
        if out.size:
            _memcpy(out.ctypes.data_as(C.c_void_p), ptr, out.nbytes, _D2H)
        return out

    def load_error_state(self, state):
        a = np.ascontiguousarray(state, dtype=np.float32)
        if a.shape != (self.local_rows, self.width, 2, 4):
            raise ValueError("error state is %s, this context holds %s" % (a.shape, (self.local_rows, self.width, 2, 4)))
        ptr, nbytes = C.c_void_p(), C.c_size_t()
        self._check(self.lib.pt_error_ptr(self._ctx, C.byref(ptr), C.byref(nbytes)))
        self.synchronize()
        if a.size:
            _memcpy(ptr, a.ctypes.data_as(C.c_void_p), a.nbytes, _H2D)

    def error_image(self):
        out = np.empty((self.local_rows, self.width, 4), dtype=np.float32)
        if out.size:
            self._check(self.lib.pt_resolve_error(self._ctx, out.ctypes.data_as(C.c_void_p)))
        return out

    def filtered_image(self, radius=2, kappa=abi.PT_FILTER_KAPPA_DEFAULT, gamma=True):
        out = np.empty((self.local_rows, self.width, 4), dtype=np.float32)
        if out.size:
            self._check(self.lib.pt_resolve_filtered(self._ctx, out.ctypes.data_as(C.c_void_p), int(radius), float(kappa), 1 if gamma else 0))
        return out

    def patch_filtered_image(self, radius=2, patch=abi.PT_FILTER_MAX_PATCH, kappa=abi.PT_FILTER_PATCH_KAPPA_DEFAULT, gamma=True):
        out = np.empty((self.local_rows, self.width, 4), dtype=np.float32)
        if out.size:
# ... 398 lines not shown
```

Before: 61390.

## Skip intersection for waves whose tiles provably miss all spheres

Adds a tile classification kernel that conservatively proves, in double precision, that every primary ray of an 8x8 tile (including lens and pixel jitter) misses all spheres. It stores the result as a bitmask that is cached and keyed on the scene and camera. The refill path tags work items from empty tiles, and when every live lane of a wave is in such a tile, the geometry walk is skipped and the rays go straight to sky shading. This removes traversal cost for background regions, at the price of an extra launch whenever the camera or scene changes, more bit-packing in the tile IDs, and new template variants.

```diff
diff --git a/bindings/rust/ptrace_sys.rs b/bindings/rust/ptrace_sys.rs
--- a/bindings/rust/ptrace_sys.rs
+++ b/bindings/rust/ptrace_sys.rs
@@ -222,6 +222,7 @@
 pub const PT_FILTER_PATCH_KAPPA_DEFAULT: f32 = 1.5;
 pub const PT_OPT_RUSSIAN_ROULETTE: c_int = 5;
 pub const PT_OPT_NEXT_EVENT: c_int = 13;
+pub const PT_OPT_TILE_BYPASS: c_int = 0;
 pub const PT_BUILD_NEXT_EVENT: c_int = 16;
 
 
diff --git a/include/ptrace.h b/include/ptrace.h
--- a/include/ptrace.h
+++ b/include/ptrace.h
@@ -48,6 +48,7 @@
   PT_OPT_TONEMAP = 11,
   PT_OPT_GLARE = 12,
   PT_OPT_NEXT_EVENT = 13,
+  PT_OPT_TILE_BYPASS = 0,
 };
 
 enum {
diff --git a/ray_tracer_webgl_amd/abi.py b/ray_tracer_webgl_amd/abi.py
--- a/ray_tracer_webgl_amd/abi.py
+++ b/ray_tracer_webgl_amd/abi.py
@@ -31,6 +31,7 @@
 PT_OPT_GLARE = 12
 PT_GLARE_MAX_LEVELS = 8
 PT_OPT_NEXT_EVENT = 13
+PT_OPT_TILE_BYPASS = 0
 PT_GLARE_STRENGTH_DEFAULT = 0.15
 PT_GLARE_LEVELS_DEFAULT = 6
 PT_GLARE_WEIGHTS_DEFAULT = (0.35, 0.25, 0.18, 0.12, 0.06, 0.04, 0.0, 0.0)
diff --git a/ray_tracer_webgl_amd/csrc/pt_api.hip b/ray_tracer_webgl_amd/csrc/pt_api.hip
--- a/ray_tracer_webgl_amd/csrc/pt_api.hip
+++ b/ray_tracer_webgl_amd/csrc/pt_api.hip
@@ -61,6 +61,15 @@
   size_t lds = 0;
   int path = 0;
   int trial = -1;
+  bool bypass = false;
+};
+
+struct TileMaskKey {
+  uint64_t scene_gen;
+  const float* geom;
+  uint32_t n_spheres, scene_regular;
+  float camera[19];
+  uint32_t width, height, local_rows, band_rows, band_index, band_count, tiles_x, tiles_y;
 };
 
 struct FramePlan {
@@ -130,6 +139,7 @@
   uint32_t refill_min = 4;
   int rr_min_depth = 0;
   ptbuf::LightSet<ptnee::Light> lights;
+  ptbuf::TileClassSet<TileMaskKey> tile_class;
   bool dbg_enable = false;
   int32_t dbg_selected = 0;
   float dbg_cursor[3] = {0.f, 0.f, 0.f};
@@ -1027,6 +1037,43 @@
   A.cost_feedback = use.feedback == LaunchUse::PLANNED ? P.cost_feedback : (use.feedback == LaunchUse::ON ? 1u : 0u);
   if (door) A.cost_feedback = 0u;
   L->kfn = kfn; L->grid = P.grid; L->block = block; L->lds = lds; L->path = path; L->trial = choice.trial;
+  const bool reads_tile_mask = (build == BUILD_PLAIN || build == BUILD_TWIN) && path != PT_GEOM_SMALL &&
+                               !(path == PT_GEOM_GRID && st.kind != 1);
+  L->bypass = !door && !nee_cell && use.n_first_tiles == 0u && reads_tile_mask;
+  return PT_OK;
+}
+
+static TileMaskKey tile_mask_key(const pt_ctx* c, const PtKernelArgs& A) {
+  TileMaskKey k;
+  memset(static_cast<void*>(&k), 0, sizeof k);
+  k.scene_gen = c->state.scene_gen;
+  k.geom = A.geom; k.n_spheres = A.n_spheres; k.scene_regular = A.scene_regular;
+  const float* parts[6] = {A.origin, A.llc, A.horizontal, A.vertical, A.cam_u, A.cam_v};
+  for (int i = 0; i < 6; i++) memcpy(&k.camera[3 * i], parts[i], 3 * sizeof(float));
+  k.camera[18] = A.lens_radius;
+  k.width = A.width; k.height = A.height; k.local_rows = A.local_rows;
+  k.band_rows = A.band_rows; k.band_index = A.band_index; k.band_count = A.band_count;
+  k.tiles_x = A.tiles_x; k.tiles_y = A.tiles_y;
+  return k;
+}
+
+static int tile_mask_for(pt_ctx* c, Launch& L, bool capturing) {
+  auto& s = c->tile_class;
+  if (!L.bypass || !s.on || capturing) return PT_OK;
+  const ptbuf::Extent e = extent_of(c);
+  if (!s.in_place(e)) (void)s.fit(e);
+  if (!s.in_place(e)) return PT_OK;
+  const TileMaskKey key = tile_mask_key(c, L.A);
+  if (!s.valid || memcmp(&key, &s.key, sizeof key) != 0) {
+    s.valid = false;
+    const uint32_t tiles = L.A.tiles_x * L.A.tiles_y;
+    hipLaunchKernelGGL(pt_tile_class_kernel, dim3(grid_for(tiles, 256, 0xffffffffu)), dim3(256), 0, c->stream, L.A, s.mask.get(),
+                       (uint32_t)s.mask.capacity());
+    PT_HIP(c, hipGetLastError());
+    s.key = key;
+    s.valid = true;
+  }
+  L.A.tile_empty = s.mask.get();
   return PT_OK;
 }
 
@@ -1098,6 +1145,7 @@
     if (int rc = span.take(c); rc != PT_OK) return rc;
 
   PT_HIP(c, zero_queue_heads(c, A.queue_static));
+  if (int rc = tile_mask_for(c, L, capturing); rc != PT_OK) return rc;
   if (c->order.uniform_wants_order_kernel(A.cost_feedback != 0u)) {
     int rc = launch_tile_order(c);
     if (rc != PT_OK) return rc;
@@ -1859,6 +1907,16 @@
       int rc = upload_lights(c, c->list.host, c->list.n);
       if (rc != PT_OK) { c->lights.release(); return rc; }
     }
+    return PT_OK;
+  }
+  if (key == PT_OPT_TILE_BYPASS) {
+    if (value != 0 && value != 1) return fail(c, PT_ERR_INVALID, "pt_set_option: tile bypass %d", value);
+    if (!value && c->tile_class.on) {
+      PT_HIP(c, hipSetDevice(c->device));
+      PT_HIP(c, hipStreamSynchronize(c->stream));
+      c->tile_class.release();
+    }
+    c->tile_class.on = value != 0;
     return PT_OK;
   }
   if (key == PT_OPT_CARRY_LANES) {
diff --git a/ray_tracer_webgl_amd/csrc/pt_buffers.hpp b/ray_tracer_webgl_amd/csrc/pt_buffers.hpp
--- a/ray_tracer_webgl_amd/csrc/pt_buffers.hpp
+++ b/ray_tracer_webgl_amd/csrc/pt_buffers.hpp
@@ -314,4 +314,27 @@
   }
 };
 
+template <class Key>
+struct TileClassSet {
+  enum : uint32_t { MASK = 1 };
+  bool on = true;
+  bool valid = false;
+  Key key{};
+  DevBuf<uint32_t> mask;
+
+  static size_t words(const Extent& e) { return 2 * ((e.tiles + 63) / 64); }
+  Fit fit(const Extent& e) {
+    Fit f;
+    if (!on || mask.holds(words(e))) return f;
+    valid = false;
+    refit(f, mask, words(e), MASK);
+    return f;
+  }
+  bool in_place(const Extent& e) const { return on && mask.holds(words(e)); }
+  void release() {
+    valid = false;
+    mask.release();
+  }
+};
+
 }
diff --git a/ray_tracer_webgl_amd/csrc/pt_kernel_args.h b/ray_tracer_webgl_amd/csrc/pt_kernel_args.h
--- a/ray_tracer_webgl_amd/csrc/pt_kernel_args.h
+++ b/ray_tracer_webgl_amd/csrc/pt_kernel_args.h
@@ -82,6 +82,7 @@
   float dbg_cursor[3];
   int32_t dbg_selected;
   uint32_t refill_ahead;
+  const uint32_t* tile_empty;
 };
 
 #ifndef PT_WAVES_WALK
diff --git a/ray_tracer_webgl_amd/csrc/pt_kernels.hip b/ray_tracer_webgl_amd/csrc/pt_kernels.hip
--- a/ray_tracer_webgl_amd/csrc/pt_kernels.hip
+++ b/ray_tracer_webgl_amd/csrc/pt_kernels.hip
@@ -1,4 +1,5 @@
 #include "pt_trace_body.hpp"
+#include "pt_tile_class.hpp"
 
 PT_MAIN_KERNELS(PT_TRACE_KERNEL)
 
@@ -50,6 +51,37 @@
   }
   __syncthreads();
   for (uint32_t i = t; i < n_tiles; i += 1024) cost[i] = 0;
+}
+
+extern "C" __global__ __launch_bounds__(256) void pt_tile_class_kernel(const PtKernelArgs A, uint32_t* mask, uint32_t mask_words) {
+  const uint32_t tile = blockIdx.x * 256u + threadIdx.x;
+  const uint32_t n_tiles = A.tiles_x * A.tiles_y;
+  bool empty = false;
+  if (tile < n_tiles) {
+    pttile::Camera cam;
+    for (int k = 0; k < 3; k++) {
+      cam.origin[k] = (double)A.origin[k]; cam.llc[k] = (double)A.llc[k];
+      cam.horizontal[k] = (double)A.horizontal[k]; cam.vertical[k] = (double)A.vertical[k];
+      cam.cam_u[k] = (double)A.cam_u[k]; cam.cam_v[k] = (double)A.cam_v[k];
+    }
+    cam.lens_radius = (double)A.lens_radius; cam.fw = (double)A.fw; cam.fh = (double)A.fh;
+    const uint32_t ty = tile / A.tiles_x, tx = tile - ty * A.tiles_x;
+    const uint32_t x0 = tx * 8u, x1 = (x0 + 7u < A.width ? x0 + 7u : A.width - 1u);
+    const uint32_t ly0 = ty * 8u, ly1 = (ly0 + 7u < A.local_rows ? ly0 + 7u : A.local_rows - 1u);
+    uint32_t y0 = ly0, y1 = ly1;
+    if (A.band_count > 1u) {
+      const uint32_t b0 = ly0 / A.band_rows, b1 = ly1 / A.band_rows;
+      y0 = (b0 * A.band_count + A.band_index) * A.band_rows + (ly0 - b0 * A.band_rows);
+      y1 = (b1 * A.band_count + A.band_index) * A.band_rows + (ly1 - b1 * A.band_rows);
+    }
+    empty = pttile::tile_empty(cam, x0, x1, y0, y1, A.geom, A.n_spheres, A.scene_regular != 0u);
+  }
+  const unsigned long long m = pt_ballot(empty);
+  const uint32_t word = 2u * (tile >> 6);
+  if ((threadIdx.x & 63u) == 0u && word + 1u < mask_words) {
+    mask[word] = (uint32_t)m;
+    mask[word + 1u] = (uint32_t)(m >> 32);
+  }
 }
 
 extern "C" __global__ __launch_bounds__(256) void pt_accumulate_kernel(float4* accum,
diff --git a/ray_tracer_webgl_amd/csrc/pt_refill.hpp b/ray_tracer_webgl_amd/csrc/pt_refill.hpp
--- a/ray_tracer_webgl_amd/csrc/pt_refill.hpp
+++ b/ray_tracer_webgl_amd/csrc/pt_refill.hpp
@@ -117,7 +117,10 @@
   return ptq::ray_valid(qo.x, qo.y, qo.z, qd.x, qd.y, qd.z);
 }
 
-template <bool COUNT, bool QRY = false, bool RAD = false>
+__device__ __forceinline__ uint32_t tile_empty_bit(const uint32_t* mask, uint32_t tile) {
+  return mask ? (mask[tile >> 5] >> (tile & 31u)) << 31 : 0u;
+}
+template <bool COUNT, bool QRY = false, bool RAD = false, bool BYPASS = false>
 __device__ __forceinline__ void refill(const PtKernelArgs& A, Path& p, Queue& q, const PixelDiv& pd, Tally<COUNT>& tally) {
   karg_t& K = *kargs();
   const bool alive = p.alive;
@@ -127,6 +130,7 @@
   uint32_t pool_next = q.pool_next, pool_end = q.pool_end;
   uint32_t pool_tp0 = q.pool_tp0, pool_split = q.pool_split, pool_tile0 = q.pool_tile0, pool_tile1 = q.pool_tile1;
   uint32_t q_round = q.round;
+  uint32_t sky_seen = q.sky_seen;
   const bool wh_ok = pd.wh_ok;
   const float y_fw = pd.y_fw, y_fh = pd.y_fh;
   for (;;) {
@@ -165,6 +169,11 @@
         const uint32_t n_tiles_w = K.tiles_x * K.tiles_y;
         pool_tile0 = (uint32_t)__builtin_amdgcn_readfirstlane((int)K.tile_order[pool_tp0]);
         pool_tile1 = (uint32_t)__builtin_amdgcn_readfirstlane((int)K.tile_order[pool_tp0 + 1u < n_tiles_w ? pool_tp0 + 1u : pool_tp0]);
+        if constexpr (BYPASS) {
+          pool_tile0 |= (uint32_t)__builtin_amdgcn_readfirstlane((int)tile_empty_bit(K.tile_empty, pool_tile0));
+          pool_tile1 |= (uint32_t)__builtin_amdgcn_readfirstlane((int)tile_empty_bit(K.tile_empty, pool_tile1));
+          sky_seen |= K.queue_chunk <= 64u * K.n_passes ? (pool_tile0 | pool_tile1) >> 31 : (K.tile_empty != nullptr ? 1u : 0u);
+        }
       }
     }
     const uint32_t avail = pool_end - pool_next;
@@ -176,14 +185,17 @@
       uint32_t item = ptdeal::item_of(pool_base, rank);
       uint32_t per_tile = 64u * K.n_passes;
       uint32_t tile_pos, tile;
+      uint32_t empty_bit = 0u;
       if (K.queue_chunk <= per_tile) {
         const bool second = item >= pool_split;
         tile_pos = pool_tp0 + (second ? 1u : 0u);
         const uint32_t t0 = pool_tile0, t1 = pool_tile1;
         tile = second ? t1 : t0;
+        if constexpr (BYPASS) { empty_bit = tile & kTileEmptyBit; tile &= ~kTileEmptyBit; }
       } else {
         tile_pos = div_by(item, K.div_per_tile.m, K.div_per_tile.s1, K.div_per_tile.s2);
         tile = K.tile_order[tile_pos];
+        if constexpr (BYPASS) empty_bit = tile_empty_bit(K.tile_empty, tile);
       }
       uint32_t rem_i = item - tile_pos * per_tile;
       uint32_t pass = rem_i >> 6, l = rem_i & 63u;
@@ -209,14 +221,15 @@
         nx_t = (vy + 1.0f) * 0.5f;
         if constexpr (RAD) nx_s = u2f(ly * K.width + px);
         nx_slab = (pass * K.local_rows + ly) * K.width + px;
-        nx_tile = (pass == 0u && K.cost_feedback != 0u) ? tile : 0xffffffffu;
+        if constexpr (BYPASS) nx_tile = ((pass == 0u && K.cost_feedback != 0u) ? tile : kNoCostTile) | empty_bit;
+        else nx_tile = (pass == 0u && K.cost_feedback != 0u) ? tile : 0xffffffffu;
       }
     }
   }
   p.nx_slab = nx_slab; p.nx_tile = nx_tile; p.nx_seed = nx_seed; p.nx_s = nx_s; p.nx_t = nx_t;
   q.pool_next = pool_next; q.pool_end = pool_end;
   q.pool_tp0 = pool_tp0; q.pool_split = pool_split; q.pool_tile0 = pool_tile0; q.pool_tile1 = pool_tile1;
-  q.round = q_round; q.dry = dry;
+  q.round = q_round; q.dry = dry; q.sky_seen = sky_seen;
 }
 
 template <bool COUNT>
diff --git a/ray_tracer_webgl_amd/csrc/pt_scene.hpp b/ray_tracer_webgl_amd/csrc/pt_scene.hpp
--- a/ray_tracer_webgl_amd/csrc/pt_scene.hpp
+++ b/ray_tracer_webgl_amd/csrc/pt_scene.hpp
@@ -34,6 +34,8 @@
   uint32_t nx_slab = ptdeal::kSlotEmpty, nx_tile = 0xffffffffu;
   float nx_seed = 0.f, nx_s = 0.f, nx_t = 0.f;
 };
+
+constexpr uint32_t kTileEmptyBit = 0x80000000u, kNoCostTile = 0x7fffffffu;
 
 template <bool NEE>
 struct NeeState {};
@@ -69,6 +71,7 @@
   uint32_t pool_tp0 = 0, pool_split = 0, pool_tile0 = 0, pool_tile1 = 0;
   uint32_t round = 0;
   bool dry = false;
+  uint32_t sky_seen = 0;
 };
 
 struct Hit {
diff --git a/ray_tracer_webgl_amd/csrc/pt_shade.hpp b/ray_tracer_webgl_amd/csrc/pt_shade.hpp
--- a/ray_tracer_webgl_amd/csrc/pt_shade.hpp
+++ b/ray_tracer_webgl_amd/csrc/pt_shade.hpp
@@ -4,7 +4,7 @@
 
 namespace ptk {
 
-template <typename S, bool RR, bool COUNT, bool DBG = false, bool FEAT = false, bool QRY = false, bool NEE = false, bool RAD = false>
+template <typename S, bool RR, bool COUNT, bool DBG = false, bool FEAT = false, bool QRY = false, bool NEE = false, bool RAD = false, bool BYPASS = false>
 __device__ __forceinline__ void shade_segment(const PtKernelArgs& A, Path& p, const Hit& h, const Carry& cw, Tally<COUNT>& tally, typename NeeArgOf<NEE>::type ne) {
   static_assert(!NEE || (!RR && !DBG && !FEAT && !COUNT), "next-event estimation excludes roulette, the overlay, the doors and the twins");
   tally.flag(PT_REG_SHADE_ANY);
@@ -263,7 +263,12 @@
       tally.flag(PT_REG_SHADE_ITEM_STORE);
       float4 outv = make_float4(sum.x, sum.y, sum.z, (float)A.spp);
       reinterpret_cast<float4*>(A.slab)[slab_index] = outv;
-      if (item_tile != 0xffffffffu) atomicMax(&A.tile_cost[item_tile], item_segs);
+      if constexpr (BYPASS) {
+        const uint32_t cost_tile = item_tile & kNoCostTile;
+        if (cost_tile != kNoCostTile) atomicMax(&A.tile_cost[cost_tile], item_segs);
+      } else {
+        if (item_tile != 0xffffffffu) atomicMax(&A.tile_cost[item_tile], item_segs);
+      }
       alive = false;
     } else {
       new_path = true;
diff --git a/ray_tracer_webgl_amd/csrc/pt_tile_class.hpp b/ray_tracer_webgl_amd/csrc/pt_tile_class.hpp
--- /dev/null
+++ b/ray_tracer_webgl_amd/csrc/pt_tile_class.hpp
@@ -0,0 +1,113 @@
+#pragma once
+#include <math.h>
+#include <stdint.h>
+
+#if defined(__HIPCC__) || defined(__CUDACC__)
+#define PT_TC_FN __host__ __device__ inline
+#else
+#define PT_TC_FN inline
+#endif
+
+namespace pttile {
+
+constexpr double kU = 5.9604644775390625e-08;
+constexpr double kSafety = 4.0;
+constexpr double kRound = 64.0;
+constexpr double kPatchSlack = 0.25;
+constexpr double kRel = 1e-9;
+constexpr double kLens = 1.01;
+
+struct Camera {
+  double origin[3], llc[3], horizontal[3], vertical[3], cam_u[3], cam_v[3];
+  double lens_radius, fw, fh;
+};
+
+struct Bundle {
+  bool ok;
+  double dc[3];
+  double dc2;
+  double rho_l, rho_f;
+};
+
+PT_TC_FN bool finite_(double x) { return x - x == 0.0; }
+PT_TC_FN double abs3(const double* v) { return fabs(v[0]) + fabs(v[1]) + fabs(v[2]); }
+
+PT_TC_FN Bundle bundle_of(const Camera& c, uint32_t x0, uint32_t x1, uint32_t y0, uint32_t y1, bool scene_regular) {
+  Bundle B;
+  B.ok = false;
+  B.dc[0] = B.dc[1] = B.dc[2] = 0.0; B.dc2 = 0.0; B.rho_l = 0.0; B.rho_f = 0.0;
+  bool fin = finite_(c.lens_radius) && finite_(c.fw) && finite_(c.fh);
+  for (int k = 0; k < 3; k++)
+    fin = fin && finite_(c.origin[k]) && finite_(c.llc[k]) && finite_(c.horizontal[k]) && finite_(c.vertical[k]) &&
+          finite_(c.cam_u[k]) && finite_(c.cam_v[k]);
+  if (!fin || !scene_regular || !(c.fw >= 1.0) || !(c.fh >= 1.0) || !(c.fw <= 65536.0) || !(c.fh <= 65536.0) || x1 < x0 || y1 < y0) return B;
+  const double s_lo = ((double)x0 + 0.5 - kPatchSlack) / c.fw, s_hi = ((double)x1 + 1.5 + kPatchSlack) / c.fw;
+  const double t_lo = ((double)y0 + 0.5 - kPatchSlack) / c.fh, t_hi = ((double)y1 + 1.5 + kPatchSlack) / c.fh;
+  const double sc = 0.5 * (s_lo + s_hi), tc = 0.5 * (t_lo + t_hi), sh = 0.5 * (s_hi - s_lo), th = 0.5 * (t_hi - t_lo);
+  const double s_abs = fabs(s_lo) > fabs(s_hi) ? fabs(s_lo) : fabs(s_hi), t_abs = fabs(t_lo) > fabs(t_hi) ? fabs(t_lo) : fabs(t_hi);
+  const double lens = fabs(c.lens_radius);
+  const double uu = c.cam_u[0] * c.cam_u[0] + c.cam_u[1] * c.cam_u[1] + c.cam_u[2] * c.cam_u[2];
+  const double vv = c.cam_v[0] * c.cam_v[0] + c.cam_v[1] * c.cam_v[1] + c.cam_v[2] * c.cam_v[2];
+  const double uv = c.cam_u[0] * c.cam_v[0] + c.cam_u[1] * c.cam_v[1] + c.cam_u[2] * c.cam_v[2];
+  const double lmax = 0.5 * (uu + vv) + sqrt(0.25 * (uu - vv) * (uu - vv) + uv * uv);
+  const double rho_l0 = kLens * lens * sqrt(lmax);
+  const double rho_f0 = sh * sqrt(c.horizontal[0] * c.horizontal[0] + c.horizontal[1] * c.horizontal[1] + c.horizontal[2] * c.horizontal[2]) +
+                        th * sqrt(c.vertical[0] * c.vertical[0] + c.vertical[1] * c.vertical[1] + c.vertical[2] * c.vertical[2]);
+  const double M = abs3(c.origin) + abs3(c.llc) + s_abs * abs3(c.horizontal) + t_abs * abs3(c.vertical) + rho_l0;
+  const double eps = kRound * kU * M;
+  double dc2 = 0.0, o_inf = 0.0;
+  for (int k = 0; k < 3; k++) {
+    B.dc[k] = (c.llc[k] + sc * c.horizontal[k] + tc * c.vertical[k]) - c.origin[k];
+    dc2 += B.dc[k] * B.dc[k];
+    o_inf = fabs(c.origin[k]) > o_inf ? fabs(c.origin[k]) : o_inf;
+  }
+  B.dc2 = dc2;
+  B.rho_l = rho_l0 * (1.0 + kRel) + eps;
+  B.rho_f = rho_f0 * (1.0 + kRel) + eps;
+  const double dn = sqrt(dc2), b = B.rho_l + B.rho_f;
+  if (!finite_(dn) || !finite_(b) || !finite_(M)) return B;
+  if (!(dn - b > 1e-5) || !(dn + b < 900.0) || !(o_inf + B.rho_l < 1e14)) return B;
+  B.ok = true;
+  return B;
+}
+
+PT_TC_FN bool clear_on(double w2, double wd, double wd_abs, double dc2, double a, double b, double l0, bool to_infinity) {
+  const double A2 = dc2 - b * b - kRel * (dc2 + b * b);
+  const double B1 = wd - a * b - kRel * (wd_abs + fabs(a * b));
+  const double C0 = w2 - a * a - kRel * (w2 + a * a);
+  if (!((A2 * l0 + 2.0 * B1) * l0 + C0 > 0.0)) return false;
+  if (to_infinity) {
+    if (!(A2 > 0.0)) return false;
+  } else {
+    if (!(A2 + 2.0 * B1 + C0 > 0.0)) return false;
+    if (!(A2 > 0.0)) return true;
+  }
+  const double vertex = -B1 / A2;
+  if (vertex <= l0 || (!to_infinity && vertex >= 1.0)) return true;
+  return C0 - B1 * B1 / A2 > 0.0;
+}
+
+PT_TC_FN bool sphere_excluded(const Camera& c, const Bundle& B, double cx, double cy, double cz, double r2) {
+  if (!B.ok || !finite_(cx) || !finite_(cy) || !finite_(cz) || !finite_(r2) || r2 < 0.0) return false;
+  const double r = sqrt(r2);
+  const double w[3] = {c.origin[0] - cx, c.origin[1] - cy, c.origin[2] - cz};
+  const double w2 = w[0] * w[0] + w[1] * w[1] + w[2] * w[2];
+  const double D = sqrt(w2) + B.rho_l;
+  const double delta = sqrt(r2 + 32.0 * kU * D * D) - r + 10.0 * kU * r;
+  const double R = r + kSafety * delta;
+  const double wd = w[0] * B.dc[0] + w[1] * B.dc[1] + w[2] * B.dc[2];
+  const double wd_abs = fabs(w[0] * B.dc[0]) + fabs(w[1] * B.dc[1]) + fabs(w[2] * B.dc[2]);
+  return clear_on(w2, wd, wd_abs, B.dc2, R + B.rho_l, B.rho_f - B.rho_l, 0.0, false) &&
+         clear_on(w2, wd, wd_abs, B.dc2, R - B.rho_l, B.rho_f + B.rho_l, 1.0, true);
+}
+
+PT_TC_FN bool tile_empty(const Camera& c, uint32_t x0, uint32_t x1, uint32_t y0, uint32_t y1, const float* geom, uint32_t n,
+                         bool scene_regular) {
+  const Bundle B = bundle_of(c, x0, x1, y0, y1, scene_regular);
+  if (!B.ok) return false;
+  for (uint32_t i = 0; i < n; i++)
+    if (!sphere_excluded(c, B, (double)geom[4 * i], (double)geom[4 * i + 1], (double)geom[4 * i + 2], (double)geom[4 * i + 3])) return false;
+  return true;
+}
+
+}
diff --git a/ray_tracer_webgl_amd/csrc/pt_trace_body.hpp b/ray_tracer_webgl_amd/csrc/pt_trace_body.hpp
--- a/ray_tracer_webgl_amd/csrc/pt_trace_body.hpp
+++ b/ray_tracer_webgl_amd/csrc/pt_trace_body.hpp
@@ -58,6 +58,7 @@
   using namespace ptk;
   constexpr bool SCAN_LDS = B::SCAN_LDS, HAVE_LDS = B::HAVE_LDS, COUNT = B::COUNT, RR = B::RR, FLAT_Y = B::FLAT_Y, DBG = B::DBG, FEAT = B::FEAT, QRY = B::QRY, RAD = B::RAD, NEE = B::NEE;
   constexpr int WALK = B::WALK, TAIL = B::TAIL;
+  constexpr bool BYPASS = !RR && !DBG && !FEAT && !QRY && !RAD && !NEE && WALK != 5 && WALK != 6 && WALK != 7;
   using S = Scene<SCAN_LDS, HAVE_LDS, WALK, TAIL, FLAT_Y>;
   S::stage(A);
 
@@ -73,7 +74,7 @@
   NeeState<NEE> ne;
 
   for (;;) {
-    refill<COUNT, QRY, RAD>(A, p, q, pd, tally);
+    refill<COUNT, QRY, RAD, BYPASS>(A, p, q, pd, tally);
     promote<COUNT>(p, tally);
     tally.phase(0);
     if (p.alive && p.new_path) {
@@ -87,47 +88,59 @@
     tally.step();
 
     Hit h;
-    if constexpr (S::TREE) h.closest = cw.carried ? cw.closest_w : PT_MAX_T;
-    if (!cw.carried) cw.hit_pos = 0xffffffffu;
-    const bool fast = regular_ray(A, p);
-    const int n_live = (int)__popcll(live);
-    if constexpr (S::TREE) park_store(A, p);
-    if constexpr (S::TREE && NEE) park_store(A, ne);
-    constexpr bool kTail = !S::TREE && !S::SMALL;
-    const bool coop = kTail && (n_live <= (int)A.coop_max_live) && (pt_ballot(p.alive && !fast) == 0ull) &&
-                      (pt_ballot(cw.carried) == 0ull);
-    if (coop) {
-      tail_mode<S>(A, p, live, h);
+    bool sky_step = false;
+    if constexpr (BYPASS) {
+      if (q.sky_seen != 0u) {
+        const unsigned long long in_sky = pt_ballot((int32_t)p.item_tile < 0);
+        sky_step = ((live & ~in_sky) | pt_ballot(cw.carried)) == 0ull;
+      }
+    }
+    if (sky_step) {
+      cw.hit_pos = 0xffffffffu;
+      if constexpr (S::TREE) cw.closest_w = PT_MAX_T;
     } else {
-      h.lit_from = fast ? 0xffffffffu : 0u;
-      const bool scan_lane = p.alive && fast;
-      if constexpr (S::BVH) bvh_walk<S, COUNT>(A, p, scan_lane, n_live, cw, bw, h, tally);
-      else if constexpr (S::GRID) grid_walk<S, COUNT>(A, p, scan_lane, n_live, cw, gw, h, tally);
-      else if constexpr (S::SMALL) small_scan<S>(A, p, scan_lane, h);
-      else list_scan<S>(A, p, scan_lane, h);
-      tally.literal(A, p.alive && !fast, scan_lane && h.lit_from < A.n_spheres, p.slab_index);
-      if constexpr (S::GRID && S::WALK != 4) {
-        const bool handed_over = scan_lane && h.lit_from == 0u;
-        const unsigned long long m_h = pt_ballot(handed_over);
-        if (m_h != 0ull) {
-          tail_mode<S>(A, p, m_h, h);
-          if (handed_over) h.lit_from = 0xffffffffu;
+      if constexpr (S::TREE) h.closest = cw.carried ? cw.closest_w : PT_MAX_T;
+      if (!cw.carried) cw.hit_pos = 0xffffffffu;
+      const bool fast = regular_ray(A, p);
+      const int n_live = (int)__popcll(live);
+      if constexpr (S::TREE) park_store(A, p);
+      if constexpr (S::TREE && NEE) park_store(A, ne);
+      constexpr bool kTail = !S::TREE && !S::SMALL;
+      const bool coop = kTail && (n_live <= (int)A.coop_max_live) && (pt_ballot(p.alive && !fast) == 0ull) &&
+                        (pt_ballot(cw.carried) == 0ull);
+      if (coop) {
+        tail_mode<S>(A, p, live, h);
+      } else {
+        h.lit_from = fast ? 0xffffffffu : 0u;
+        const bool scan_lane = p.alive && fast;
+        if constexpr (S::BVH) bvh_walk<S, COUNT>(A, p, scan_lane, n_live, cw, bw, h, tally);
+        else if constexpr (S::GRID) grid_walk<S, COUNT>(A, p, scan_lane, n_live, cw, gw, h, tally);
+        else if constexpr (S::SMALL) small_scan<S>(A, p, scan_lane, h);
+        else list_scan<S>(A, p, scan_lane, h);
+        tally.literal(A, p.alive && !fast, scan_lane && h.lit_from < A.n_spheres, p.slab_index);
+        if constexpr (S::GRID && S::WALK != 4) {
+          const bool handed_over = scan_lane && h.lit_from == 0u;
+          const unsigned long long m_h = pt_ballot(handed_over);
+          if (m_h != 0ull) {
+            tail_mode<S>(A, p, m_h, h);
+            if (handed_over) h.lit_from = 0xffffffffu;
+          }
         }
+        literal_loop<S>(A, p, h);
       }
-      literal_loop<S>(A, p, h);
-    }
-    if constexpr (S::TREE) {
-      if (coop) cw.carried = false;
-      cw.closest_w = h.closest;
-      park_load(A, p);
-      if constexpr (NEE) park_load(A, ne);
+      if constexpr (S::TREE) {
+        if (coop) cw.carried = false;
+        cw.closest_w = h.closest;
+        park_load(A, p);
+        if constexpr (NEE) park_load(A, ne);
+      }
     }
     tally.phase(6);
 
     const bool shade = p.alive && !cw.carried;
     seg_count += (uint32_t)__popcll(pt_ballot(shade));
     tally.timebin(A, shade);
-    if (shade) shade_segment<S, RR, COUNT, DBG, FEAT, QRY, NEE, RAD>(A, p, h, cw, tally, ne);
+    if (shade) shade_segment<S, RR, COUNT, DBG, FEAT, QRY, NEE, RAD, BYPASS>(A, p, h, cw, tally, ne);
     tally.collect();
     tally.phase(7);
   }
diff --git a/ray_tracer_webgl_amd/tracer.py b/ray_tracer_webgl_amd/tracer.py
--- a/ray_tracer_webgl_amd/tracer.py
+++ b/ray_tracer_webgl_amd/tracer.py
@@ -106,6 +106,9 @@
 
     def next_event(self, on=True):
         self._check(self.lib.pt_set_option(self._ctx, abi.PT_OPT_NEXT_EVENT, 1 if on else 0))
+
+    def set_tile_bypass(self, on=True):
+        self._check(self.lib.pt_set_option(self._ctx, abi.PT_OPT_TILE_BYPASS, 1 if on else 0))
 
     def set_debug_overlay(self, enable, selected_object=abi.NO_SELECTED_OBJECT_ID, cursor_point=(0.0, 0.0, 0.0)):
         cur = (C.c_float * 3)(*[float(x) for x in cursor_point])
```

Result: no change. 61580 (median of 6 runs) (+0.3%).
